# by256/icsg3d

Hardware: AMD Instinct MI355X
Metric: voxel-grids/s (fwd+bwd) for 32^3 U-Net+VAE at batch 32: value = U-Net train step (BASELINE configs[1]); DFC-VAE step (configs[2]) in secondary; both per batch in unet_plus_vae (higher is better)
Workload: dtype f32

## Files before the change

### icsg3d_amd/csrc/common.h

```cpp
#pragma once
#include <hip/hip_runtime.h>
#include <hip/hip_ext.h>
#include <atomic>
#include <cstdint>
#include <cstdio>
#include <string>
#include <vector>

#include "up8.h"
#include "up125.h"

namespace ics {

extern std::atomic<long long> g_kernel_launches;
struct LaunchTimer {
  virtual void next(hipEvent_t* start, hipEvent_t* stop) = 0;
  virtual ~LaunchTimer() = default;
};
extern thread_local LaunchTimer* tl_launch_timer;
template <typename... P, typename... A>
inline void ics_launch(void (*kernel)(P...), dim3 grid, dim3 block, size_t shmem, hipStream_t st, A&&... args) {
  static_assert(sizeof...(P) == sizeof...(A), "kernel argument count");
  if (tl_launch_timer != nullptr) {
    hipEvent_t e0 = nullptr, e1 = nullptr;
    tl_launch_timer->next(&e0, &e1);
    hipExtLaunchKernelGGL(kernel, grid, block, (std::uint32_t)shmem, st, e0, e1, 0u, static_cast<P>(args)...);
  } else {
    hipLaunchKernelGGL(kernel, grid, block, shmem, st, static_cast<P>(args)...);
  }
}
#define ICS_LAUNCH(...)                                      \
  do {                                                       \
    ::ics::g_kernel_launches.fetch_add(1, std::memory_order_relaxed); \
    ::ics::ics_launch(__VA_ARGS__);                          \
  } while (0)

void set_error(const std::string& msg);
#define ICS_HIP(expr)                                                                     \
  do {                                                                                    \
    hipError_t _e = (expr);                                                               \
    if (_e != hipSuccess) {                                                               \
      ::ics::set_error(std::string(#expr) + " -> " + hipGetErrorString(_e) + " @" +       \
                       __FILE__ + ":" + std::to_string(__LINE__));                        \
      return -1;                                                                          \
    }                                                                                     \
  } while (0)
#define ICS_CHECK(cond, msg)                                                              \
  do {                                                                                    \
    if (!(cond)) {                                                                        \
      ::ics::set_error(std::string(msg) + " (" #cond ") @" + __FILE__ + ":" +             \
                       std::to_string(__LINE__));                                         \
      return -1;                                                                          \
    }                                                                                     \
  } while (0)
#define ICS_TRY(expr)                                                                     \
  do {                                                                                    \
    if ((expr) != 0) return -1;                                                           \
  } while (0)

enum Act : int { ACT_NONE = 0, ACT_RELU = 1, ACT_LRELU = 2 };
constexpr float kLeaky = 0.3f;
constexpr float kBnEps = 1e-3f;
constexpr float kKEps = 1e-7f;
constexpr float kPoolTieTol = 1e-5f;

__device__ __forceinline__ float act_fwd(float v, int act) {
  if (act == ACT_RELU) return fmaxf(v, 0.f);
  if (act == ACT_LRELU) return v > 0.f ? v : kLeaky * v;
  return v;
}
__device__ __forceinline__ float act_grad(float v, int act) {
  if (act == ACT_RELU) return v > 0.f ? 1.f : 0.f;
  if (act == ACT_LRELU) return v > 0.f ? 1.f : kLeaky;
  return 1.f;
}

struct ConvSrc {
  const float* p;
  const float* scale;
  const float* shift;
  int C;
  int up;
  int act;
  int bcast;
};

enum ConvFlags : int {
  CF_NO_REUSE = 1,
  CF_NO_WGRAD3 = 2,
  CF_NO_WGRAD3S = 4,
  CF_NO_FWD_SPLITK = 8,
  CF_NO_THIN_N = 16,
  CF_NO_UPSPLIT = 32,
  CF_NO_THIN_C = 64,
  CF_NO_COND_FOLD = 128,
  CF_NO_WINO = 256,
  CF_NO_WINO_WGRAD = 512,
  CF_NO_WINO64 = 1024,
  CF_NO_UP3 = 2048,
  CF_NO_THIN1_2STAGE = 4096,
  CF_NO_FAST_BNBWD = 8192,
  CF_NO_FUSED_HEAD = 16384,
  CF_NO_BWD_FOLD = 32768,
  CF_UP3_BIG_ALWAYS = 65536,
  CF_NO_WINOG = 262144,
  CF_NO_HEAD_BNFUSE = 524288,
  CF_NO_UP3N = 1 << 21,
  CF_NO_DGRAD_BNFUSE = 1 << 22,
  CF_NO_POOL_PRESUM = 1 << 23,
  CF_NO_HEAD_LABELS = 1 << 24,
  CF_NO_UP8 = 1 << 25,
  CF_UP8 = 1 << 26,
  CF_NO_UP125 = 1 << 27,
  CF_FORCE_UP125 = 1 << 28,
  CF_POOL125_V1 = 1 << 29,
  CF_ZBATCH = 1 << 20,
};
int conv_flags_from_env();

struct ConvGeom {
  int B, S, lgS;
  int Cin, Cout;
  int taps;
  int Kpad, Npad;
  int flags = 0;
};

struct BwdStat {
  const float* s = nullptr;
  const float* mean = nullptr;
  const float* rstd = nullptr;
  const float* scale = nullptr;
  const float* shift = nullptr;
  float* partial = nullptr;
  int post_act = ACT_NONE;
  int ld = 0;
  const float* abc = nullptr;
  float* db_partial = nullptr;
  const float* pool_d = nullptr;
  int pool_ld = 0;
  const unsigned char* pool_mask = nullptr;
};

int launch_conv_fwd(hipStream_t st, const ConvGeom& g, const ConvSrc* src, int nsrc,
                    const float* wpacked, const float* bias, float* out, int ldo, int pre_act,
                    float* stat_partial, int* stat_rows_per_block, int accumulate = 0,
                    float* splitk_ws = nullptr, size_t splitk_ws_floats = 0, const BwdStat* bwd = nullptr,
                    int* bwd_blocks = nullptr);
size_t conv_fwd_workspace_floats(const ConvGeom& g, const ConvSrc* src, int nsrc);
bool conv_fwd_up8_tile_ok(const ConvGeom& g);
bool conv_thin_c_ok(const ConvGeom& g, const ConvSrc& s0, int nsrc, int cin_log);
size_t conv_thin_c_wgrad_workspace_floats(const ConvGeom& g);
int launch_conv_wgrad_thin_c(hipStream_t st, const ConvGeom& g, const ConvSrc& s0, const float* dy, int ldy, float* dw,
                             int ldw, int row_pitch, float* ws, size_t ws_floats, int phase);
int launch_conv_fwd_thin_c(hipStream_t st, const ConvGeom& g, const ConvSrc& s0, int cin_log, int wstride,
                           const float* wp, const float* bias, float* out, int ldo, int pre_act, float* stat_partial,
                           int* rows_per_block, const float* pos_bias = nullptr);
int launch_conv_fwd_par(hipStream_t st, const ConvGeom& g_lowres, const ConvSrc& src, const float* wpar, float* out,
                        int ldo, const float* bias = nullptr, int pre_act = ACT_NONE, float* stat_partial = nullptr,
                        int* stat_blocks = nullptr);
int launch_pack_par(hipStream_t st, const float* w, int Cin_total, int Cout, int c_off, int Cu, float* dst, int Kpad,
                    int Npad);
int launch_pack_fwd_sub(hipStream_t st, const float* w, int taps, int Cin_total, int Cout, int c_off, int Csub,
                        float* dst, int Kpad, int Npad);
int launch_conv_wgrad(hipStream_t st, const ConvGeom& g, const ConvSrc* src, int nsrc,
                      const float* dy, int ldy, float* dw, int ldw, float* workspace,
                      size_t workspace_floats, int sub_rows = 0, int row_pitch = 0, int row_off = 0,
                      int phase = 0);
const char* conv_last_kernel_id();
void conv_set_last_kernel_id(const char* id);
int launch_pack_sub(hipStream_t st, const float* w, int taps, int Cin_total, int Cout, int c_off, int Csub,
                    int flip, float* dst, int Kpad, int Npad);
size_t conv_wgrad_workspace_floats(const ConvGeom& g, const ConvSrc* src, int nsrc);
int conv_fwd_rows_per_block(const ConvGeom& g);
int launch_conv_wgrad_ablate(hipStream_t st, const ConvGeom& g, const ConvSrc* src, const float* dy, int ldy,
                             float* workspace, int ablate);
int launch_conv_fwd_ablate(hipStream_t st, const ConvGeom& g, const ConvSrc* src, int nsrc, const float* wp,
                           float* out, int ldo, int ablate);
int launch_pack_fwd(hipStream_t st, const float* w, int K, int N, float* dst, int Kpad, int Npad,
                    int k_off, int n_off, int zero_first, int cin_log = 0, int cin_phys = 0);
void* pack_table_record_begin();
int pack_table_record_end(void* handle, std::vector<unsigned char>* bytes, int* njobs, unsigned* nblocks);
int launch_pack_table(hipStream_t st, const void* d_jobs, int njobs, unsigned nblocks);
int launch_materialize_input(hipStream_t st, const ConvSrc* src, int nsrc, int Cin, int CinG, int B, int S,
                             float* out);
int launch_pack_bwd(hipStream_t st, const float* w, int taps, int Cin, int Cout, float* dst,
                    int Kpad, int Npad, int cout_total, int co_off, int zero_first);

bool conv_wino_ok(const ConvGeom& g, const ConvSrc* src, int nsrc);
size_t conv_wino_weight_floats(int Cin, int Cout);
int launch_conv_fwd_wino(hipStream_t st, const ConvGeom& g, const ConvSrc& s0, const float* wt, const float* bias,
                         float* out, int ldo, int pre_act, float* stat_partial, int* rows_per_block, int accumulate,
                         int layout, const BwdStat* bwd = nullptr, int* bwd_blocks = nullptr);
int launch_pack_wino(hipStream_t st, const float* w, int Cin_total, int Cout, int c_off, int Csub, int bwd, float* dst,
                     int layout = 0);
int conv_wino_layout(const ConvGeom& g);
bool conv_wino64_ok(const ConvGeom& g, const ConvSrc* src, int nsrc);
int launch_conv_fwd_wino64(hipStream_t st, const ConvGeom& g, const ConvSrc& s0, const float* wt, const float* bias,
                           float* out, int ldo, int pre_act, float* stat_partial, int* rows_per_block, int accumulate,
                           const BwdStat* bwd = nullptr, int* bwd_blocks = nullptr);
bool conv_wino_wgrad_ok(const ConvGeom& g, const ConvSrc* src, int nsrc);
size_t conv_wino_wgrad_workspace_floats(const ConvGeom& g);
int launch_conv_wgrad_wino(hipStream_t st, const ConvGeom& g, const ConvSrc& s0, const float* dy, int ldy, float* dw,
                           int ldw, float* ws, size_t ws_floats, int sub_rows, int row_pitch, int row_off, int phase);
bool conv_up3_ok(const ConvGeom& g, const ConvSrc& s0);
size_t conv_up3_weight_floats(int Cu, int Cout);
int launch_pack_up3(hipStream_t st, const float* w, int Cin_total, int Cout, int c_off, int Cu, float* dst);
int launch_conv_fwd_up3(hipStream_t st, const ConvGeom& g, const ConvSrc& s0, const float* wt, const float* bias,
                        float* out, int ldo, int pre_act, float* stat_partial, int* stat_blocks, int accumulate);
bool conv_winog_ok(const ConvGeom& g, const ConvSrc* src, int nsrc);
bool conv_winog_wgrad_ok(const ConvGeom& g, const ConvSrc* src, int nsrc);
size_t conv_winog_weight_floats(int Cin, int Cout);
void conv_winog_scratch_floats(const ConvGeom& g, size_t* v, size_t* m, size_t* z);
int launch_conv_fwd_winog(hipStream_t st, const ConvGeom& g, const ConvSrc& s0, const float* wg, const float* bias, float* out,
                          int ldo, int pre_act, float* stat_partial, int* rows_per_block, float* v_scratch, float* m_scratch,
                          float* vt_keep);
int launch_conv_wgrad_winog(hipStream_t st, const ConvGeom& g, const float* vt, const float* dy, int ldy, float* dw, int ldw,
                            int row_pitch, int row_off, float* z_scratch, float* m_scratch);
int launch_gemm_zbatch(hipStream_t st, int nz, int M, int K, int N, const float* A, const float* Wp, float* out, int flags);
int wgrad_zbatch_splits(int nz, int M, int K, int N);
int launch_wgrad_zbatch(hipStream_t st, int nz, int M, int K, int N, const float* x, const float* dy, float* ws, int ksplit);
int launch_pack_up125(hipStream_t st, const float* w, int Cin_total, int N, int c_off, int Cu, float* dst);
int launch_pack_up125_pieces(hipStream_t st, const float* w, int Cin_total, int N, int c_off, int Cu, float* dst);
bool conv_up3n_ok(const ConvGeom& g, const ConvSrc& s0);
size_t conv_up3n_weight_floats(int Cu, int Cout);
int launch_pack_up3n(hipStream_t st, const float* w, int Cin_total, int Cout, int c_off, int Cu, float* dst);
int launch_conv_fwd_up3n(hipStream_t st, const ConvGeom& g, const ConvSrc& s0, const float* wt, const float* bias, float* out,
                         int ldo, int pre_act, float* stat_partial, int* stat_blocks);
int launch_wgrad_reduce_splits(hipStream_t st, const float* ws, int nsplit, size_t n_elems, int N, float* dw, int ldw,
                               int sub_rows, int row_pitch, int row_off);

}
```

### icsg3d_amd/csrc/conv_igemm.hip

```cpp
#include "common.h"

#ifndef ICS_GEMM_DEEP_FWD_MIN
#define ICS_GEMM_DEEP_FWD_MIN 1
#endif
#ifndef ICS_GEMM_DEEP_MIN
#define ICS_GEMM_DEEP_MIN 3
#endif
#ifndef ICS_GEMM_DEEP
#define ICS_GEMM_DEEP 1
#endif

#include <algorithm>
#include <type_traits>
#include <cstdlib>
#include <cstring>
#include <vector>

namespace ics {

typedef float f32x16 __attribute__((ext_vector_type(16)));
typedef float v4f __attribute__((ext_vector_type(4)));

#ifndef ICS_KLDA
#define ICS_KLDA 36
#endif
constexpr int kLDA = ICS_KLDA;

__device__ __forceinline__ int xcd_swizzle(int bid, int nblk) {
  const int xcd = bid & 7, q = nblk >> 3, r = nblk & 7;
  return (xcd < r ? xcd * (q + 1) : r * (q + 1) + (xcd - r) * q) + (bid >> 3);
}

static thread_local const char* g_last_kernel_id = "";
const char* conv_last_kernel_id() { return g_last_kernel_id; }
void conv_set_last_kernel_id(const char* id) { g_last_kernel_id = id; }
static const char* tf(bool b) { return b ? "true" : "false"; }

int conv_flags_from_env() {
  int f = 0;
  if (getenv("ICSG3D_NO_REUSE")) f |= CF_NO_REUSE;
  if (getenv("ICSG3D_NO_WGRAD3")) f |= CF_NO_WGRAD3;
  if (getenv("ICSG3D_NO_WGRAD3S")) f |= CF_NO_WGRAD3S;
  if (getenv("ICSG3D_NO_FWD_SPLITK")) f |= CF_NO_FWD_SPLITK;
  if (getenv("ICSG3D_NO_THIN_N")) f |= CF_NO_THIN_N;
  if (getenv("ICSG3D_NO_UPSPLIT")) f |= CF_NO_UPSPLIT;
  if (getenv("ICSG3D_NO_THIN_C")) f |= CF_NO_THIN_C;
  if (getenv("ICSG3D_NO_COND_FOLD")) f |= CF_NO_COND_FOLD;
  if (getenv("ICSG3D_NO_WINO")) f |= CF_NO_WINO;
  if (getenv("ICSG3D_NO_WINO_WGRAD")) f |= CF_NO_WINO_WGRAD;
  if (getenv("ICSG3D_NO_WINO64")) f |= CF_NO_WINO64;
  if (getenv("ICSG3D_NO_UP3")) f |= CF_NO_UP3;
  if (getenv("ICSG3D_NO_THIN1_2STAGE")) f |= CF_NO_THIN1_2STAGE;
  if (getenv("ICSG3D_NO_FAST_BNBWD")) f |= CF_NO_FAST_BNBWD;
  if (getenv("ICSG3D_NO_FUSED_HEAD")) f |= CF_NO_FUSED_HEAD;
  if (getenv("ICSG3D_NO_BWD_FOLD")) f |= CF_NO_BWD_FOLD;
  if (getenv("ICSG3D_NO_WINOG")) f |= CF_NO_WINOG;
  if (getenv("ICSG3D_NO_HEAD_BNFUSE")) f |= CF_NO_HEAD_BNFUSE;
  if (getenv("ICSG3D_NO_UP3N")) f |= CF_NO_UP3N;
  if (getenv("ICSG3D_NO_DGRAD_BNFUSE")) f |= CF_NO_DGRAD_BNFUSE;
  if (getenv("ICSG3D_NO_POOL_PRESUM")) f |= CF_NO_POOL_PRESUM;
  if (getenv("ICSG3D_NO_HEAD_LABELS")) f |= CF_NO_HEAD_LABELS;
  if (getenv("ICSG3D_NO_UP8")) f |= CF_NO_UP8;
  if (getenv("ICSG3D_NO_UP125")) f |= CF_NO_UP125;
  if (getenv("ICSG3D_FORCE_UP125")) f |= CF_FORCE_UP125;
  if (getenv("ICSG3D_POOL125_V1")) f |= CF_POOL125_V1;
  { const char* e = getenv("ICSG3D_UP3_BIG_MIN_WG"); if (e && *e && strtoul(e, nullptr, 10) <= 1) f |= CF_UP3_BIG_ALWAYS; }
  return f;
}
struct DevOnce {
  bool done[64] = {false};
  bool need(int* dev) {
    int d = 0;
    if (hipGetDevice(&d) != hipSuccess || d < 0 || d >= 64) { *dev = -1; return true; }
    *dev = d;
    return !done[d];
  }
  void mark(int dev) { if (dev >= 0) done[dev] = true; }
};

static int identity_affine(const float** ones, const float** zeros) {
  constexpr int kN = 16384;
  static float* buf[64] = {nullptr};
  int dev = 0;
  ICS_HIP(hipGetDevice(&dev));
  ICS_CHECK(dev >= 0 && dev < 64, "device index out of range");
  if (!buf[dev]) {
    float* p = nullptr;
    ICS_HIP(hipMalloc(&p, 2 * kN * sizeof(float)));
    std::vector<float> h(2 * kN, 0.f);
    for (int i = 0; i < kN; ++i) h[i] = 1.f;
    ICS_HIP(hipMemcpy(p, h.data(), 2 * kN * sizeof(float), hipMemcpyHostToDevice));
    buf[dev] = p;
  }
  *ones = buf[dev];
  *zeros = buf[dev] + kN;
  return 0;
}
static int fix_src(ConvSrc& s) {
  if (s.scale == nullptr) {
    ICS_CHECK(s.C <= 16384, "source wider than the identity-affine buffer");
    ICS_TRY(identity_affine(&s.scale, &s.shift));
    s.act = ACT_NONE;
  }
  return 0;
}

struct RowPos {
  int b, z, y, x;
};
__device__ __forceinline__ RowPos decode_row(int m, int S, int lg) {
  RowPos r;
  r.x = m & (S - 1);
  r.y = (m >> lg) & (S - 1);
  r.z = (m >> (2 * lg)) & (S - 1);
  r.b = m >> (3 * lg);
  return r;
}

__device__ __forceinline__ size_t src_voxel(const ConvSrc& s, int b, int z, int y, int x, int S) {
  if (s.up) {
    const int Sh = S >> 1;
    return ((((size_t)b * Sh + (z >> 1)) * Sh + (y >> 1)) * Sh + (x >> 1)) * (size_t)s.C;
  }
  return ((((size_t)b * S + z) * S + y) * S + x) * (size_t)s.C;
}

__host__ __device__ __forceinline__ float act_slope_of(int act) {
  return act == ACT_RELU ? 0.f : (act == ACT_LRELU ? kLeaky : 1.f);
}
__device__ __forceinline__ float act_apply(float v, float slope) {
  return fmaxf(v, v * slope);
}
template <bool NOACT>
__device__ __forceinline__ v4f affine_only_or_act4(v4f v, v4f sc, v4f sh, float slope);
__device__ __forceinline__ v4f affine_act4(v4f v, v4f sc, v4f sh, float slope) {
  v4f r;
  r.x = act_apply(fmaf(v.x, sc.x, sh.x), slope); r.y = act_apply(fmaf(v.y, sc.y, sh.y), slope);
  r.z = act_apply(fmaf(v.z, sc.z, sh.z), slope); r.w = act_apply(fmaf(v.w, sc.w, sh.w), slope);
  return r;
}
template <bool NOACT>
__device__ __forceinline__ v4f affine_only_or_act4(v4f v, v4f sc, v4f sh, float slope) {
  if (!NOACT) return affine_act4(v, sc, sh, slope);
  v4f r;
  r.x = fmaf(v.x, sc.x, sh.x); r.y = fmaf(v.y, sc.y, sh.y); r.z = fmaf(v.z, sc.z, sh.z); r.w = fmaf(v.w, sc.w, sh.w);
  return r;
}
__device__ __forceinline__ unsigned voxel_off(int b, int z, int y, int x, int S, int u, int C) {
  const int Ss = S >> u;
  return ((((unsigned)b * Ss + (z >> u)) * Ss + (y >> u)) * Ss + (x >> u)) * (unsigned)C;
}
__device__ __forceinline__ int clampi(int v, int hi) { return min(max(v, 0), hi); }

__device__ __forceinline__ ConvSrc pick_src(const ConvSrc& s0, const ConvSrc& s1, bool first) {
  ConvSrc s;
  s.p = first ? s0.p : s1.p;
  s.scale = first ? s0.scale : s1.scale;
  s.shift = first ? s0.shift : s1.shift;
  s.C = first ? s0.C : s1.C;
  s.up = first ? s0.up : s1.up;
  s.act = first ? s0.act : s1.act;
  s.bcast = first ? s0.bcast : s1.bcast;
  return s;
}

__device__ __forceinline__ float gather_scalar(const ConvSrc& s0, const ConvSrc& s1, int ci, int b,
                                               int z, int y, int x, int S) {
  const bool first = ci < s0.C;
  const ConvSrc s = pick_src(s0, s1, first);
  const int cl = first ? ci : ci - s0.C;
  float v;
  if (s.bcast > 0) {
    v = s.p[(size_t)b * s.bcast + (cl % s.bcast)];
  } else {
    v = s.p[src_voxel(s, b, z, y, x, S) + cl];
  }
  if (s.scale) v = act_fwd(fmaf(v, s.scale[cl], s.shift[cl]), s.act);
  return v;
}

template <int WM, int WN, int TM, int TN, bool VEC, int ABL = 0, bool AFF = true, bool UP = true, bool THIN = false,
          bool REUSE = false, bool PAR = false, bool NOACT = false, bool FOLD = false, bool UP8 = false>
__global__ __launch_bounds__(256, FOLD ? 2 : ((REUSE && PAR) ? 3 : 1)) void conv_fwd_kernel(ConvGeom g, ConvSrc s0, ConvSrc s1,
                                                        const float* __restrict__ wp,
                                                        const float* __restrict__ bias,
                                                        float* __restrict__ out, int ldo, int pre_act,
                                                        float* __restrict__ stat_partial, int gridM,
                                                        int gridN, int accumulate, BwdStat bs, Up8Geom u8) {
  constexpr int BM = WM * TM * 32, BN = WN * TN * 32;
  constexpr int B_FLOATS = 32 * BN;
  constexpr int RA = BM / 32;
  constexpr int RS = BM / 8;
  constexpr int NB = BN / 32;
  extern __shared__ __attribute__((aligned(16))) float smem[];
  const int A_FLOATS = (REUSE ? BM + (BM >> g.lgS) + 1 : BM) * kLDA;
  float* As = smem;
  constexpr int NABUF = 1;
  float* Bs = smem + NABUF * A_FLOATS;

  const int t = threadIdx.x, lane = t & 63, wave = t >> 6;
  const int wm = wave / WN, wn = wave % WN;
  const int li = lane & 31, lh = lane >> 5;
  const int sw = xcd_swizzle(blockIdx.x, gridM * gridN);
  const int mb = sw / gridN, nb = sw % gridN;
  const int S = g.S, lg = g.lgS;
  const int M = g.B << (3 * lg);
  const int n0 = nb * BN;
  const int nchunks = g.Kpad >> 5;
  const int cpt = (VEC && !THIN) ? (g.Cin >> 5) : 1;
  const int cls = PAR ? (int)blockIdx.y : 0;
  const int pz = cls >> 2, py = (cls >> 1) & 1, px = cls & 1;
  if (PAR) wp += (size_t)cls * g.Kpad * g.Npad;
  const bool zbatch = (g.flags & CF_ZBATCH) != 0;
  if (zbatch) {
    s0.p += (size_t)blockIdx.z * (size_t)M * (size_t)s0.C;
    wp += (size_t)blockIdx.z * (size_t)g.Kpad * (size_t)g.Npad;
    out += (size_t)blockIdx.z * (size_t)M * (size_t)ldo;
  }
// ... 1524 lines not shown
      return launch_fwd_cfg<WM, WN, TM, TN, true, 0, true, true, false, true>(ICS_FWD_ARGS);    \
    }                                                                                           \
    if (variant == 0 && fold)                                                                   \
      return launch_fwd_cfg<WM, WN, TM, TN, true, 0, false, false, false, false, false, false, true>(ICS_FWD_ARGS); \
    if (variant == 0) return launch_fwd_cfg<WM, WN, TM, TN, true, 0, false, false>(ICS_FWD_ARGS); \
    if (variant == 1) return launch_fwd_cfg<WM, WN, TM, TN, true, 0, true, false>(ICS_FWD_ARGS);  \
    return launch_fwd_cfg<WM, WN, TM, TN, true, 0, true, true>(ICS_FWD_ARGS);                   \
  } while (0)
  if (bm == 64) { ICS_FWD(2, 2, 1, 1); }
  if (bn == 128) { ICS_FWD(2, 2, 2, 2); }
  if (bn == 96) { ICS_FWD(4, 1, 1, 3); }
  if (bn == 64) { ICS_FWD(2, 2, 2, 1); }
  ICS_FWD(4, 1, 1, 1);
#undef ICS_FWD_ARGS
#undef ICS_FWD
}

static void pick_par_tile(const ConvGeom& g, int* bm, int* bn) {
  pick_fwd_tile(g, bm, bn);
  if (*bm == 64 && g.Npad % 128 == 0 && (long)(((g.B << (3 * g.lgS)) + 127) / 128) * (g.Npad / 128) * 8 >= 384) {
    *bm = 128; *bn = 128;
  }
}
int launch_conv_fwd_par(hipStream_t st, const ConvGeom& g, const ConvSrc& src, const float* wp, float* out,
                        int ldo, const float* bias, int pre_act, float* stat_partial, int* stat_blocks) {
  ConvSrc s0 = src, s1 = src;
  s1.C = 0;
  ICS_CHECK(g.taps == 8 && g.Cin % 32 == 0 && s0.C == g.Cin && !s0.up && !s0.bcast && g.Kpad == 8 * g.Cin,
            "parity-class conv needs a direct 32k-channel source");
  ICS_TRY(fix_src(s0));
  ICS_TRY(fix_src(s1));
  int bm, bn;
  pick_par_tile(g, &bm, &bn);
  int rpb = 0;
#define ICS_PAR_ARGS st, g, s0, s1, wp, bias, out, ldo, pre_act, stat_partial, &rpb
  int rc;
  const bool no_reuse = (g.flags & CF_NO_REUSE) != 0;
  const bool reuse = !no_reuse && g.S >= 4 && g.S <= bm;
  const bool noact = src.scale != nullptr && src.act == ACT_NONE;
#define ICS_PAR(WM, WN, TM, TN)                                                                              \
  (reuse ? (noact ? launch_fwd_cfg<WM, WN, TM, TN, true, 0, true, false, false, true, true, true>(ICS_PAR_ARGS) \
                  : launch_fwd_cfg<WM, WN, TM, TN, true, 0, true, false, false, true, true>(ICS_PAR_ARGS))   \
         : launch_fwd_cfg<WM, WN, TM, TN, true, 0, true, false, false, false, true>(ICS_PAR_ARGS))
  if (bm == 64) rc = ICS_PAR(2, 2, 1, 1);
  else if (bn == 128) rc = ICS_PAR(2, 2, 2, 2);
  else if (bn == 96) rc = ICS_PAR(4, 1, 1, 3);
  else if (bn == 64) rc = ICS_PAR(2, 2, 2, 1);
  else rc = ICS_PAR(4, 1, 1, 1);
#undef ICS_PAR
#undef ICS_PAR_ARGS
  if (stat_blocks) *stat_blocks = 8 * (((g.B << (3 * g.lgS)) + rpb - 1) / rpb);
  return rc;
}

struct PackJob {
  int kind;
  const float* w;
  float* dst;
  int a[9];
  unsigned long long total;
  unsigned blk0;
};
static thread_local std::vector<PackJob>* g_pack_rec = nullptr;

__device__ __forceinline__ float pack_par_value(size_t i, const float* __restrict__ w, int Cin_total, int Cout, int c_off,
                                                int Cu, int Kpad, int Npad) {
  const size_t per = (size_t)Kpad * Npad;
  const int cls = (int)(i / per);
  const size_t j = i - (size_t)cls * per;
  const int tq = j & 3;
  const size_t rest = j >> 2;
  const int n = rest % Npad;
  const int k = (int)(rest / Npad) * 4 + tq;
  const int e = k / Cu, c = k - e * Cu;
  float v = 0.f;
  if (e < 8 && n < Cout) {
    const int p3[3] = {cls >> 2, (cls >> 1) & 1, cls & 1};
    const int e3[3] = {e >> 2, (e >> 1) & 1, e & 1};
    int lo[3], hi[3];
#pragma unroll
    for (int a = 0; a < 3; ++a) {
      if (p3[a] == 0) { lo[a] = e3[a] ? 1 : 0; hi[a] = e3[a] ? 2 : 0; }
      else { lo[a] = e3[a] ? 2 : 0; hi[a] = e3[a] ? 2 : 1; }
    }
    for (int dz = lo[0]; dz <= hi[0]; ++dz)
      for (int dy = lo[1]; dy <= hi[1]; ++dy)
        for (int dx = lo[2]; dx <= hi[2]; ++dx)
          v += w[((size_t)((dz * 3 + dy) * 3 + dx) * Cin_total + c_off + c) * Cout + n];
  }
  return v;
}
__global__ void pack_par_kernel(const float* __restrict__ w, int Cin_total, int Cout, int c_off, int Cu,
                                float* __restrict__ dst, int Kpad, int Npad) {
  const size_t i = (size_t)blockIdx.x * blockDim.x + threadIdx.x;
  if (i >= 8 * (size_t)Kpad * Npad) return;
  dst[i] = pack_par_value(i, w, Cin_total, Cout, c_off, Cu, Kpad, Npad);
}
int launch_pack_par(hipStream_t st, const float* w, int Cin_total, int Cout, int c_off, int Cu, float* dst,
                    int Kpad, int Npad) {
  if (g_pack_rec) { g_pack_rec->push_back(PackJob{4, w, dst, {Cin_total, Cout, c_off, Cu, Kpad, Npad, 0, 0, 0}, 8ull * Kpad * Npad, 0}); return 0; }
  const size_t total = (size_t)8 * Kpad * Npad;
  ICS_LAUNCH(pack_par_kernel, dim3((unsigned)((total + 255) / 256)), dim3(256), 0, st, w, Cin_total, Cout,
                     c_off, Cu, dst, Kpad, Npad);
  ICS_HIP(hipGetLastError());
  return 0;
}
__device__ __forceinline__ float pack_fwd_sub_value(size_t i, const float* __restrict__ w, int taps, int Cin_total,
                                                    int Cout, int c_off, int Csub, int Npad) {
  const int tq = i & 3;
  const size_t rest = i >> 2;
  const int n = rest % Npad;
  const int k = (int)(rest / Npad) * 4 + tq;
  const int tap = k / Csub, c = k - tap * Csub;
  return (tap < taps && n < Cout) ? w[((size_t)tap * Cin_total + c_off + c) * Cout + n] : 0.f;
}
__global__ void pack_fwd_sub_kernel(const float* __restrict__ w, int taps, int Cin_total, int Cout, int c_off,
                                    int Csub, float* __restrict__ dst, int Kpad, int Npad) {
  const size_t i = (size_t)blockIdx.x * blockDim.x + threadIdx.x;
  if (i >= (size_t)Kpad * Npad) return;
  dst[i] = pack_fwd_sub_value(i, w, taps, Cin_total, Cout, c_off, Csub, Npad);
}
int launch_pack_fwd_sub(hipStream_t st, const float* w, int taps, int Cin_total, int Cout, int c_off, int Csub,
                        float* dst, int Kpad, int Npad) {
  if (g_pack_rec) { g_pack_rec->push_back(PackJob{3, w, dst, {taps, Cin_total, Cout, c_off, Csub, Npad, 0, 0, 0}, (unsigned long long)Kpad * Npad, 0}); return 0; }
  const size_t total = (size_t)Kpad * Npad;
  ICS_LAUNCH(pack_fwd_sub_kernel, dim3((unsigned)((total + 255) / 256)), dim3(256), 0, st, w, taps,
                     Cin_total, Cout, c_off, Csub, dst, Kpad, Npad);
  ICS_HIP(hipGetLastError());
  return 0;
}

int launch_conv_fwd_ablate(hipStream_t st, const ConvGeom& g, const ConvSrc* src, int nsrc, const float* wp,
                           float* out, int ldo, int ablate) {
  ConvSrc s0 = src[0], s1 = src[nsrc > 1 ? 1 : 0];
  if (nsrc == 1) s1.C = 0;
  ICS_TRY(fix_src(s0));
  ICS_TRY(fix_src(s1));
  ICS_CHECK(fwd_is_vec(g, s0, s1) && g.Npad % 128 == 0, "ablation bench needs the vector 128x128 configuration");
#define ICS_ABL_ARGS st, g, s0, s1, wp, nullptr, out, ldo, 0, nullptr, nullptr
  if (ablate == 1) return launch_fwd_cfg<2, 2, 2, 2, true, 1, true, false>(ICS_ABL_ARGS);
  if (ablate == 2) return launch_fwd_cfg<2, 2, 2, 2, true, 2, true, false>(ICS_ABL_ARGS);
  if (ablate == 3) return launch_fwd_cfg<2, 2, 2, 2, true, 3, true, false>(ICS_ABL_ARGS);
  if (ablate == 4) return launch_fwd_cfg<2, 2, 2, 2, true, 4, true, false>(ICS_ABL_ARGS);
  if (ablate == 8) return launch_fwd_cfg<2, 2, 2, 2, true, 8, false, false>(ICS_ABL_ARGS);
  if (ablate == 9) return launch_fwd_cfg<2, 2, 2, 2, true, 9, false, false>(ICS_ABL_ARGS);
  if (ablate == 5) return launch_fwd_cfg<2, 2, 2, 2, true, 0, true, false>(ICS_ABL_ARGS);
  if (ablate == 6) return launch_fwd_cfg<2, 2, 2, 2, true, 0, true, true>(ICS_ABL_ARGS);
  return launch_fwd_cfg<2, 2, 2, 2, true, 0, false, false>(ICS_ABL_ARGS);
#undef ICS_ABL_ARGS
}


template <int WM, int WN, int TM, int TN, bool VEC, bool DYVEC, bool AFF = true, bool UP = true, bool THIN = false,
          int ABL = 0, bool UP8 = false, bool ZB = false>
__global__ __launch_bounds__(256) void conv_wgrad_kernel(ConvGeom g, ConvSrc s0, ConvSrc s1,
                                                          const float* __restrict__ dy, int ldy,
                                                          int n_load,
                                                          float* __restrict__ ws, int ktiles,
                                                          int ntiles, int rows_per_split, Up8Geom u8) {
  constexpr int KT = WM * TM * 32, NT = WN * TN * 32;
  constexpr int A_FLOATS = 32 * KT, D_FLOATS = 32 * NT;
  constexpr int AF4 = KT / 4, ATOT = 32 * AF4, APASS = ATOT / 256;
  constexpr int DF4 = NT / 4, DTOT = 32 * DF4, DPASS = DTOT / 256;
  static_assert(ATOT % 256 == 0 && DTOT % 256 == 0, "tile loads must divide evenly over 256 threads");
  extern __shared__ __attribute__((aligned(16))) float smem[];
  float* As = smem;
  float* Ds = smem + 2 * A_FLOATS;

  const int t = threadIdx.x, lane = t & 63, wave = t >> 6;
  const int wm = wave / WN, wn = wave % WN;
  const int li = lane & 31, lh = lane >> 5;
  const int S = g.S, lg = g.lgS;
  const int M = g.B << (3 * lg);
  const int K = g.taps * g.Cin;
  if (ZB) {
    s0.p += (size_t)blockIdx.y * (size_t)M * (size_t)s0.C;
    dy += (size_t)blockIdx.y * (size_t)M * (size_t)ldy;
    ws += (size_t)blockIdx.y * (size_t)(gridDim.x / (unsigned)(ktiles * ntiles)) * (size_t)K * (size_t)g.Cout;
  }

  int bid = blockIdx.x;
  const int nt_i = bid % ntiles; bid /= ntiles;
  const int kt_i = bid % ktiles; bid /= ktiles;
  const int split = bid;
  const int n0 = nt_i * NT;
  const int m_begin = split * rows_per_split;
  const int m_end = min(M, m_begin + rows_per_split);
  const int nchunks = (m_end - m_begin + 31) >> 5;

  const int k0 = kt_i * KT;
  int tdz = 0, tdy = 0, tdx = 0, sdelta = 0, xbad = -1, ybad = -1, zbad = -1;
  bool kvalid = false;
  const float* sp = s0.p;
  int sC = s0.C, su = 0, cl0 = 0;
  float slope = 1.f;
  v4f sc = v4f{1.f, 1.f, 1.f, 1.f}, sh = v4f{0.f, 0.f, 0.f, 0.f};
  if (VEC) {
    const int kf = k0 + (t % AF4) * 4;
    const int tap = kf / g.Cin, ci = kf - tap * g.Cin;
    kvalid = kf < K;
    if (g.taps == 27 && kvalid) { tdz = tap / 9 - 1; tdy = (tap / 3) % 3 - 1; tdx = tap % 3 - 1; }
    sdelta = (tdz * S + tdy) * S + tdx;
    xbad = tdx < 0 ? 0 : (tdx > 0 ? S - 1 : -1);
    ybad = tdy < 0 ? 0 : (tdy > 0 ? S - 1 : -1);
    zbad = tdz < 0 ? 0 : (tdz > 0 ? S - 1 : -1);
    const bool first = ci < s0.C;
    const ConvSrc sv = pick_src(s0, s1, first);
    sp = sv.p; sC = sv.C; su = sv.up;
    cl0 = kvalid ? (first ? ci : ci - s0.C) : 0;
    slope = act_slope_of(sv.act);
    if (AFF) {
      sc = *reinterpret_cast<const v4f*>(sv.scale + cl0);
      sh = *reinterpret_cast<const v4f*>(sv.shift + cl0);
    }
  }
  int s_tap = 0, s_ci = 0; bool s_kvalid = false; int sdz = 0, sdy = 0, sdx = 0;
  if (!VEC) {
    const int kf = k0 + (t & 31);
    s_tap = kf / g.Cin; s_ci = kf - s_tap * g.Cin; s_kvalid = kf < K;
    if (g.taps == 27) { sdz = s_tap / 9 - 1; sdy = (s_tap / 3) % 3 - 1; sdx = s_tap % 3 - 1; }
  }

  v4f ra[VEC ? APASS : 1];
  float ras[4];
  v4f rd[DPASS];

  auto load_chunk = [&](int c) {
    const int mbase = m_begin + (c << 5);
    if (VEC) {
      const int Sh = S >> 1;
#pragma unroll
      for (int p = 0; p < APASS; ++p) {
        const int m = mbase + (t + 256 * p) / AF4;
        const int x = m & (S - 1), y = (m >> lg) & (S - 1), z = (m >> (2 * lg)) & (S - 1);
        const bool inb = kvalid && m < m_end && x != xbad && y != ybad && z != zbad;
        int idx = m + sdelta;
        if (UP) {
          const int b = m >> (3 * lg);
          const int idx_up = ((b * Sh + ((z + tdz) >> 1)) * Sh + ((y + tdy) >> 1)) * Sh + ((x + tdx) >> 1);
          idx = su ? idx_up : idx;
        }
        const unsigned off = inb ? (unsigned)idx * (unsigned)sC + cl0 : (unsigned)cl0;
        v4f v = *reinterpret_cast<const v4f*>(sp + off);
        if (AFF) v = affine_act4(v, sc, sh, slope);
        ra[p] = inb ? v : v4f{0.f, 0.f, 0.f, 0.f};
      }
    } else {
#pragma unroll
      for (int p = 0; p < 4; ++p) {
        const int m = mbase + (t >> 5) + 8 * p;
        float v = 0.f;
        if (s_kvalid && m < m_end) {
          const RowPos r = decode_row(m, S, lg);
          const int zz = r.z + sdz, yy = r.y + sdy, xx = r.x + sdx;
          if ((unsigned)zz < (unsigned)S && (unsigned)yy < (unsigned)S && (unsigned)xx < (unsigned)S)
            v = gather_scalar(s0, s1, s_ci, r.b, zz, yy, xx, S);
        }
        ras[p] = v;
      }
    }
#pragma unroll
    for (int p = 0; p < DPASS; ++p) {
      const int idx = t + 256 * p;
      const int m = mbase + idx / DF4;
      const int n = n0 + (idx % DF4) * 4;
      const float* q = dy + (size_t)min(m, M - 1) * ldy;
      v4f v;
      if (DYVEC) {
        v = *reinterpret_cast<const v4f*>(q + min(n, n_load - 4));
        if (!(m < m_end && n < n_load)) v = v4f{0.f, 0.f, 0.f, 0.f};
      } else {
        v.x = q[min(n + 0, n_load - 1)]; v.y = q[min(n + 1, n_load - 1)];
        v.z = q[min(n + 2, n_load - 1)]; v.w = q[min(n + 3, n_load - 1)];
        const bool rowok = m < m_end;
        v.x = (rowok && n + 0 < n_load) ? v.x : 0.f; v.y = (rowok && n + 1 < n_load) ? v.y : 0.f;
        v.z = (rowok && n + 2 < n_load) ? v.z : 0.f; v.w = (rowok && n + 3 < n_load) ? v.w : 0.f;
      }
      rd[p] = v;
    }
  };
  const bool gemm = VEC && DYVEC && !UP && !THIN && ABL == 0 && g.taps == 1 && (M & 31) == 0 &&
                    (rows_per_split & 31) == 0 && (UP8 || n0 + NT <= n_load);
  const bool noact_g = slope == 1.f;
  unsigned aoffg[VEC ? APASS : 1], doffg[DPASS];
  if (VEC) {
#pragma unroll
    for (int p = 0; p < APASS; ++p) aoffg[p] = (unsigned)(((t + 256 * p) / AF4) * sC + cl0) * 4u;
  }
#pragma unroll
  for (int p = 0; p < DPASS; ++p) {
    const int idx = t + 256 * p;
    doffg[p] = UP8 ? (up8_prow((unsigned)(idx / DF4), u8.lgSh, u8.P) * (unsigned)u8.N +
                      up8_col_floats(min(n0 + (idx % DF4) * 4, n_load - 4), u8)) * 4u
                   : (unsigned)((idx / DF4) * ldy + n0 + (idx % DF4) * 4) * 4u;
  }
  auto load_chunk_gemm = [&](int c, auto noact_tag) {
    constexpr bool NA = decltype(noact_tag)::value;
    const int mbase = m_begin + (c << 5);
    const char* abase = reinterpret_cast<const char*>(sp) + (size_t)mbase * (size_t)sC * 4;
    const char* dbase = reinterpret_cast<const char*>(dy) +
                        (UP8 ? up8_chunk_base_floats((unsigned)mbase, u8) : (size_t)mbase * (size_t)ldy) * 4;
    if (VEC) {
#pragma unroll
      for (int p = 0; p < APASS; ++p) {
        v4f v = *reinterpret_cast<const v4f*>(abase + aoffg[p]);
        if (AFF) v = affine_only_or_act4<NA>(v, sc, sh, slope);
        ra[p] = v;
      }
    }
#pragma unroll
    for (int p = 0; p < DPASS; ++p) rd[p] = *reinterpret_cast<const v4f*>(dbase + doffg[p]);
  };
  auto store_chunk = [&](int buf) {
    float* A = As + buf * A_FLOATS;
    float* D = Ds + buf * D_FLOATS;
    if (VEC) {
#pragma unroll
      for (int p = 0; p < APASS; ++p) {
        const int idx = t + 256 * p;
        *reinterpret_cast<v4f*>(A + (idx / AF4) * KT + (idx % AF4) * 4) = ra[p];
      }
    } else {
#pragma unroll
      for (int p = 0; p < 4; ++p) A[((t >> 5) + 8 * p) * KT + (t & 31)] = ras[p];
    }
#pragma unroll
    for (int p = 0; p < DPASS; ++p) {
      const int idx = t + 256 * p;
      *reinterpret_cast<v4f*>(D + (idx / DF4) * NT + (idx % DF4) * 4) = rd[p];
    }
  };

  f32x16 acc[TM][TN];
#pragma unroll
  for (int i = 0; i < TM; ++i)
#pragma unroll
    for (int j = 0; j < TN; ++j)
// ... 458 lines not shown
  const bool first = c0 < s0.C;
  const char* sp = reinterpret_cast<const char*>(first ? s0.p : s1.p);
  const int sC = first ? s0.C : s1.C;
  const float slope = act_slope_of(first ? s0.act : s1.act);
  const int ac4 = t & 15;
  const int cl = (first ? c0 : c0 - s0.C) + ac4 * 4;
  if (AFF && t < 32) {
    const float* src = (t < 16) ? (first ? s0.scale : s1.scale) : (first ? s0.shift : s1.shift);
    *reinterpret_cast<v4f*>(Aff + t * 4) = *reinterpret_cast<const v4f*>(src + (first ? c0 : c0 - s0.C) + (t & 15) * 4);
  }
  const unsigned aoff = (unsigned)((t >> 4) * sC + cl) * 4u;
  const unsigned hoff = (unsigned)cl * 4u;
  unsigned doff[4];
#pragma unroll
  for (int p = 0; p < 4; ++p) doff[p] = (unsigned)(((t >> 5) + 8 * p) * ldy + n0 + (t & 31) * 4) * 4u;
  const int hside = (t >> 4) & 1;

  v4f ra[2], rd[4], rah = v4f{0.f, 0.f, 0.f, 0.f};
  auto load_chunk = [&](int c) {
    const int mbase = m_begin + (c << 5);
    v4f sc = v4f{1.f, 1.f, 1.f, 1.f}, sh = v4f{0.f, 0.f, 0.f, 0.f};
    if (AFF) { sc = *reinterpret_cast<const v4f*>(Aff + ac4 * 4); sh = *reinterpret_cast<const v4f*>(Aff + 64 + ac4 * 4); }
#pragma unroll
    for (int p = 0; p < 2; ++p) {
      const int row0 = mbase + 16 * p;
      const int y = (row0 >> lg) & (S - 1), z = (row0 >> (2 * lg)) & (S - 1);
      const bool inb = (y != ybad) & (z != zbad);
      const float msk = inb ? 1.f : 0.f;
      const char* base = sp + (inb ? (long)(row0 + sdelta) * sC * 4 : 0L);
      v4f v = *reinterpret_cast<const v4f*>(base + aoff);
      if (AFF) v = affine_only_or_act4<NOACT>(v, sc, sh, slope);
      ra[p] = v4f{v.x * msk, v.y * msk, v.z * msk, v.w * msk};
    }
    if (halo) {
      const int x0 = mbase & (S - 1);
      const int y = (mbase >> lg) & (S - 1), z = (mbase >> (2 * lg)) & (S - 1);
      const bool lineok = (y != ybad) & (z != zbad);
      const bool inl = lineok & (x0 != 0), inr = lineok & (x0 == 0);
      const char* bl = sp + (inl ? (long)(mbase - 1 + sdelta) * sC * 4 : 0L);
      const char* br = sp + (inr ? (long)(mbase + 32 + sdelta) * sC * 4 : 0L);
      const float msk = (hside ? inr : inl) ? 1.f : 0.f;
      v4f v = *reinterpret_cast<const v4f*>((hside ? br : bl) + hoff);
      if (AFF) v = affine_only_or_act4<NOACT>(v, sc, sh, slope);
      rah = v4f{v.x * msk, v.y * msk, v.z * msk, v.w * msk};
    }
    const char* dbase = reinterpret_cast<const char*>(dy) + (size_t)mbase * (size_t)ldy * 4;
#pragma unroll
    for (int p = 0; p < 4; ++p) rd[p] = *reinterpret_cast<const v4f*>(dbase + doff[p]);
  };
  float* a_st[2];
#pragma unroll
  for (int p = 0; p < 2; ++p) {
    const int r = (t >> 4) + 16 * p;
    a_st[p] = As + (r + (halo ? 0 : (r >> lg)) + 1) * CK + ac4 * 4;
  }
  auto store_chunk = [&](int buf) {
#pragma unroll
    for (int p = 0; p < 2; ++p) *reinterpret_cast<v4f*>(a_st[p] + buf * A_FLOATS) = ra[p];
    if (halo && t < 32) *reinterpret_cast<v4f*>(As + buf * A_FLOATS + (hside ? 33 : 0) * CK + ac4 * 4) = rah;
    float* D = Ds + buf * D_FLOATS;
#pragma unroll
    for (int p = 0; p < 4; ++p) *reinterpret_cast<v4f*>(D + ((t >> 5) + 8 * p) * NT + (t & 31) * 4) = rd[p];
  };

  f32x16 acc[3][2];
#pragma unroll
  for (int i = 0; i < 3; ++i)
#pragma unroll
    for (int j = 0; j < 2; ++j)
#pragma unroll
      for (int r = 0; r < 16; ++r) acc[i][j][r] = 0.f;

  if (!halo) {
    for (int i = t; i < 2 * (lines + 1) * CK; i += 256) {
      const int b = i / ((lines + 1) * CK), rem = i - b * (lines + 1) * CK;
      As[b * A_FLOATS + (rem / CK) * (S + 1) * CK + rem % CK] = 0.f;
    }
  }
  __syncthreads();
  if (nchunks > 0) {
    load_chunk(0);
    store_chunk(0);
  }
  __syncthreads();
  auto compute = [&](int buf) {
    const float* A = As + buf * A_FLOATS + 2 * li + lh * CK;
    const float* D = Ds + buf * D_FLOATS + 32 * wave + li + lh * NT;
#pragma unroll
    for (int s = 0; s < 16; ++s) {
      constexpr int dummy = 0; (void)dummy;
      const int prow = 2 * s + (halo ? 0 : ((2 * s) >> lg)) + 1;
      const float b = D[(2 * s) * NT];
      float2 a[3];
#pragma unroll
      for (int dxi = 0; dxi < 3; ++dxi) a[dxi] = *reinterpret_cast<const float2*>(A + (prow + dxi - 1) * CK);
#pragma unroll
      for (int dxi = 0; dxi < 3; ++dxi) {
        acc[dxi][0] = __builtin_amdgcn_mfma_f32_32x32x2f32(a[dxi].x, b, acc[dxi][0], 0, 0, 0);
        acc[dxi][1] = __builtin_amdgcn_mfma_f32_32x32x2f32(a[dxi].y, b, acc[dxi][1], 0, 0, 0);
      }
    }
  };
  for (int c = 0; c + 1 < nchunks; ++c) {
    load_chunk(c + 1);
    compute(c & 1);
    store_chunk((c + 1) & 1);
    __syncthreads();
  }
  if (nchunks > 0) compute((nchunks - 1) & 1);

  float* wsp = ws + (size_t)split * K * g.Cout;
  const int n = n0 + 32 * wave + li;
#pragma unroll
  for (int dxi = 0; dxi < 3; ++dxi)
#pragma unroll
    for (int j = 0; j < 2; ++j)
#pragma unroll
      for (int r = 0; r < 16; ++r) {
        const int row = (r & 3) + 8 * (r >> 2) + 4 * lh;
        const int k = (gzy * 3 + dxi) * g.Cin + c0 + 2 * row + j;
        wsp[(size_t)k * g.Cout + n] = acc[dxi][j][r];
      }
}

static bool wgrad3_ok(const ConvGeom& g, const ConvSrc& s0, int nsrc, const ConvSrc& s1) {
  if ((g.flags & CF_NO_WGRAD3) || g.taps != 27 || g.S > 64 || g.S < 2 || g.Cin % 64 != 0 || g.Cout % 128 != 0) return false;
  if (s0.bcast || (nsrc > 1 && s1.bcast)) return false;
  if (nsrc > 1 && (s0.C % 64 != 0)) return false;
  return true;
}
struct Wgrad3Plan { int cgroups, ntiles, ksplit, rows_per_split; };
static Wgrad3Plan plan_wgrad3(const ConvGeom& g) {
  Wgrad3Plan p;
  const long M = (long)g.B << (3 * g.lgS);
  p.cgroups = g.Cin / 64;
  p.ntiles = g.Cout / 128;
  const int want = pick_ksplit(9L * p.cgroups * p.ntiles, M, g.lgS > 5 ? 512 : 768, 2);
  p.rows_per_split = (int)(((M + want - 1) / want + 31) / 32 * 32);
  p.ksplit = (int)((M + p.rows_per_split - 1) / p.rows_per_split);
  return p;
}


size_t conv_wgrad_workspace_floats(const ConvGeom& g, const ConvSrc* src, int nsrc) {
  if (thin_n_ok(g, src[0], nsrc)) return (size_t)thin_n_wgrad_splits(g) * g.taps * g.Cin * g.Cout;
  ConvSrc s0 = src[0], s1 = src[nsrc > 1 ? 1 : 0];
  WgradPlan p = plan_wgrad(g, s0, nsrc, s1);
  int ks = p.ksplit;
  if (wgrad3_ok(g, s0, nsrc, s1)) ks = std::max(ks, plan_wgrad3(g).ksplit);
  return (size_t)ks * g.taps * g.Cin * g.Cout;
}

template <int WM, int WN, int TM, int TN, bool VEC, bool DYVEC, bool AFF = true, bool UP = true, bool THIN = false,
          int ABL = 0, bool UP8 = false, bool ZB = false>
static int launch_wgrad_cfg(hipStream_t st, const ConvGeom& g, const ConvSrc& s0, const ConvSrc& s1,
                            const float* dy, int ldy, int n_load, float* ws, const WgradPlan& p, int nz = 1) {
  constexpr int KT = WM * TM * 32, NT = WN * TN * 32;
  const size_t lds = (size_t)2 * 32 * (KT + NT) * sizeof(float);
  auto kern = conv_wgrad_kernel<WM, WN, TM, TN, VEC, DYVEC, AFF, UP, THIN, ABL, UP8, ZB>;
  static DevOnce attr;
  int dev;
  if (attr.need(&dev)) {
    ICS_HIP(hipFuncSetAttribute(reinterpret_cast<const void*>(kern),
                                hipFuncAttributeMaxDynamicSharedMemorySize, (int)lds));
    attr.mark(dev);
  }
  static const std::string id = std::string("conv_wgrad_kernel<") + std::to_string(WM) + ", " + std::to_string(WN) +
                                ", " + std::to_string(TM) + ", " + std::to_string(TN) + ", " + tf(VEC) + ", " +
                                tf(DYVEC) + ", " + tf(AFF) + ", " + tf(UP) + ", " + tf(THIN) + ", " +
                                std::to_string(ABL) + (UP8 ? ", UP8>" : (ZB ? ", ZB>" : ">"));
  g_last_kernel_id = id.c_str();
  Up8Geom u8;
  if (UP8) u8 = up8_geom(g.B, g.S, g.lgS, g.Cout / 27);
  ICS_LAUNCH(kern, dim3(p.ktiles * p.ntiles * p.ksplit, ZB ? nz : 1), dim3(256), lds, st, g, s0, s1, dy,
                     ldy, n_load, ws, p.ktiles, p.ntiles, p.rows_per_split, u8);
  ICS_HIP(hipGetLastError());
  return 0;
}

int launch_conv_wgrad_ablate(hipStream_t st, const ConvGeom& g, const ConvSrc* src, const float* dy, int ldy,
                             float* workspace, int ablate) {
  ConvSrc s0 = src[0], s1 = src[0];
  s1.C = 0;
  ICS_TRY(fix_src(s0));
  ICS_TRY(fix_src(s1));
  WgradPlan p = plan_wgrad(g, s0, 1, s1);
  ICS_CHECK(p.vec && p.kt == 128 && p.nt == 128, "ablation bench needs the vector 128x128 configuration");
  if (ablate == 1) return launch_wgrad_cfg<2, 2, 2, 2, true, true, false, false, false, 1>(st, g, s0, s1, dy, ldy, g.Cout, workspace, p);
  return launch_wgrad_cfg<2, 2, 2, 2, true, true, false, false, false, 2>(st, g, s0, s1, dy, ldy, g.Cout, workspace, p);
}

int launch_conv_wgrad(hipStream_t st, const ConvGeom& g, const ConvSrc* src, int nsrc,
                      const float* dy, int ldy, float* dw, int ldw, float* workspace,
                      size_t workspace_floats, int sub_rows, int row_pitch, int row_off, int phase) {
  if (thin_n_ok(g, src[0], nsrc)) {
    const int ns = thin_n_wgrad_splits(g);
    const size_t n_el = (size_t)g.taps * g.Cin * g.Cout;
    ICS_CHECK((size_t)ns * n_el <= workspace_floats, "wgrad workspace too small");
    const int M = g.B << (3 * g.lgS);
    const int rows = (M + ns - 1) / ns;
    const int K = 27 * g.Cin;
    const bool aff = src[0].scale != nullptr;
    if (thin1_wgrad_ok(g, src[0])) {
      const int nb = thin1_wgrad_blocks(g);
      if (phase != 2) {
#define ICS_T1W(CKV)                                                                                                 \
  do {                                                                                                               \
    if (aff) ICS_LAUNCH((thin1_wgrad_kernel<CKV, true>), dim3(nb), dim3(256), 0, st, g, src[0], dy, ldy, workspace); \
    else ICS_LAUNCH((thin1_wgrad_kernel<CKV, false>), dim3(nb), dim3(256), 0, st, g, src[0], dy, ldy, workspace);    \
  } while (0)
        switch (g.Cin / 16) { case 1: ICS_T1W(1); break; case 2: ICS_T1W(2); break; case 3: ICS_T1W(3); break; default: ICS_T1W(4); break; }
#undef ICS_T1W
        ICS_HIP(hipGetLastError());
        g_last_kernel_id = "thin1_wgrad_kernel";
      }
      if (phase != 1) ICS_TRY(launch_reduce_splits(st, workspace, 4 * nb, n_el, g.Cout, dw, ldw, sub_rows, row_pitch, row_off));
      return 0;
    }
    if (phase != 2) {
#define ICS_TNW(NOUT, AFFV, KPT, NAME)                                                                         \
  do {                                                                                                         \
    g_last_kernel_id = NAME;                                                                                   \
    ICS_LAUNCH((conv_thin_n_wgrad_kernel<NOUT, AFFV, KPT>), dim3((M + rows - 1) / rows), dim3(256), 0,  \
                       st, g, src[0], dy, ldy, workspace, rows);                                               \
  } while (0)
#define ICS_TNW_K(NOUT, AFFV, TAG)                                                                  \
  do {                                                                                              \
    if (K <= 512) ICS_TNW(NOUT, AFFV, 2, "conv_thin_n_wgrad_kernel<" TAG ", 2>");                   \
    else if (K <= 1024) ICS_TNW(NOUT, AFFV, 4, "conv_thin_n_wgrad_kernel<" TAG ", 4>");             \
    else ICS_TNW(NOUT, AFFV, 7, "conv_thin_n_wgrad_kernel<" TAG ", 7>");                            \
  } while (0)
      if (g.Cout == 1) { if (aff) ICS_TNW_K(1, true, "1, true"); else ICS_TNW_K(1, false, "1, false"); }
      else { if (aff) ICS_TNW_K(4, true, "4, true"); else ICS_TNW_K(4, false, "4, false"); }
#undef ICS_TNW_K
#undef ICS_TNW
      ICS_HIP(hipGetLastError());
    }
    if (phase != 1)
      ICS_TRY(launch_reduce_splits(st, workspace, (M + rows - 1) / rows, n_el, g.Cout, dw, ldw, sub_rows, row_pitch,
                                   row_off));
    return 0;
  }
  ConvSrc s0 = src[0], s1 = src[nsrc > 1 ? 1 : 0];
  if (nsrc == 1) s1.C = 0;
  ICS_TRY(fix_src(s0));
  ICS_TRY(fix_src(s1));
  WgradPlan p = plan_wgrad(g, s0, nsrc, s1);
  const size_t n_elems = (size_t)g.taps * g.Cin * g.Cout;
  const int n_load4 = (g.Cout + 3) / 4 * 4;
  const bool dy_vec = (ldy % 4 == 0) && ((reinterpret_cast<uintptr_t>(dy) & 15) == 0) && (n_load4 <= ldy);
  const int n_load = dy_vec ? n_load4 : g.Cout;
  if (!dy_vec) {
    p.nt = (p.kt == 128) ? 32 : (p.kt == 64) ? 64 : 128;
    p.ntiles = (g.Npad + p.nt - 1) / p.nt;
  }
  const bool aff = src[0].scale != nullptr || (nsrc > 1 && src[1].scale != nullptr);
  const bool up = src[0].up || (nsrc > 1 && src[1].up);
  if (dy_vec && wgrad3_ok(g, s0, nsrc, s1)) {
    const Wgrad3Plan q = plan_wgrad3(g);
    ICS_CHECK((size_t)q.ksplit * n_elems <= workspace_floats, "wgrad workspace too small");
    const int arows = 32 + std::max(32 >> g.lgS, 1) + 1;
    const size_t lds = (size_t)(2 * (arows * 64 + 32 * 128) + 128) * sizeof(float);
    const dim3 grid(9 * q.cgroups * q.ntiles * q.ksplit);
    const int M3 = g.B << (3 * g.lgS);
    const bool fast = !up && g.lgS >= 4 && g.lgS <= 6 && M3 % 32 == 0 && n_load == g.Cout &&
                      !(g.flags & CF_NO_WGRAD3S);
    if (phase != 2 && fast) {
      const bool noact = aff && (src[0].scale == nullptr || src[0].act == ACT_NONE) &&
                         (nsrc < 2 || src[1].scale == nullptr || src[1].act == ACT_NONE);
      const int ar = 32 + (g.lgS == 6 ? 1 : (32 >> g.lgS)) + 1;
      const size_t lds3 = (size_t)(2 * (ar * 64 + 32 * 128) + 128) * sizeof(float);
#define ICS_W3S(AFFV, NOACTV, LGV)                                                                              \
  do {                                                                                                          \
    g_last_kernel_id = "conv_wgrad3s_kernel<" #AFFV ", " #NOACTV ", " #LGV ">";                                 \
    ICS_LAUNCH((conv_wgrad3s_kernel<AFFV, NOACTV, LGV>), grid, dim3(256), lds3, st, g, s0, s1, dy, ldy,  \
                       workspace, q.cgroups, q.ntiles, q.rows_per_split);                                       \
  } while (0)
#define ICS_W3S_L(AFFV, NOACTV)                                                       \
  do {                                                                                \
    if (g.lgS == 4) ICS_W3S(AFFV, NOACTV, 4);                                         \
    else if (g.lgS == 5) ICS_W3S(AFFV, NOACTV, 5);                                    \
    else ICS_W3S(AFFV, NOACTV, 6);                                                    \
  } while (0)
      if (!aff) ICS_W3S_L(false, false);
      else if (noact) ICS_W3S_L(true, true);
      else ICS_W3S_L(true, false);
#undef ICS_W3S_L
#undef ICS_W3S
      ICS_HIP(hipGetLastError());
    } else if (phase != 2) {
#define ICS_W3(AFFV, UPV, HALOV)                                                                                 \
  do {                                                                                                           \
    g_last_kernel_id = "conv_wgrad3_kernel<" #AFFV ", " #UPV ", " #HALOV ">";                                    \
    ICS_LAUNCH((conv_wgrad3_kernel<AFFV, UPV, HALOV>), grid, dim3(256), lds, st, g, s0, s1, dy, ldy,      \
                       n_load, workspace, q.cgroups, q.ntiles, q.rows_per_split);                                \
  } while (0)
      if (g.lgS > 5) {
        if (up) ICS_W3(true, true, true); else if (aff) ICS_W3(true, false, true); else ICS_W3(false, false, true);
      } else {
        if (up) ICS_W3(true, true, false); else if (aff) ICS_W3(true, false, false); else ICS_W3(false, false, false);
      }
#undef ICS_W3
      ICS_HIP(hipGetLastError());
    }
    if (phase != 1) {
      ICS_TRY(launch_reduce_splits(st, workspace, q.ksplit, n_elems, g.Cout, dw, ldw, sub_rows, row_pitch, row_off));
    }
    return 0;
  }
  ICS_CHECK((size_t)p.ksplit * n_elems <= workspace_floats, "wgrad workspace too small");
  if (phase != 2) {
#define ICS_WG_ARGS st, g, s0, s1, dy, ldy, n_load, workspace, p
#define ICS_WG(WM, WN, TM, TN, DV)                                                                 \
  do {                                                                                             \
    if (p.thin) ICS_TRY((launch_wgrad_cfg<WM, WN, TM, TN, true, DV, true, true, true>(ICS_WG_ARGS)));  \
    else if (!p.vec) ICS_TRY((launch_wgrad_cfg<WM, WN, TM, TN, false, DV, true, true>(ICS_WG_ARGS)));   \
    else if (up) ICS_TRY((launch_wgrad_cfg<WM, WN, TM, TN, true, DV, true, true>(ICS_WG_ARGS)));   \
    else if (aff) ICS_TRY((launch_wgrad_cfg<WM, WN, TM, TN, true, DV, true, false>(ICS_WG_ARGS))); \
    else ICS_TRY((launch_wgrad_cfg<WM, WN, TM, TN, true, DV, false, false>(ICS_WG_ARGS)));         \
  } while (0)
  if (g.flags & CF_UP8) {
    const int M8 = g.B << (3 * g.lgS);
    ICS_CHECK(dy_vec && p.vec && !p.thin && !up && g.taps == 1 && g.Cout % 27 == 0 && n_load == g.Cout && M8 % 32 == 0 &&
                  p.rows_per_split % 32 == 0 && up8_shape_ok(2 * g.S, g.Cout / 27, (size_t)M8, g.B),
              "up8 backward-weight: shape outside the 8-volume layout");
#define ICS_WG8(WM, WN, TM, TN)                                                                                  \
  do {                                                                                                           \
    if (aff) ICS_TRY((launch_wgrad_cfg<WM, WN, TM, TN, true, true, true, false, false, 0, true>(ICS_WG_ARGS)));  \
    else ICS_TRY((launch_wgrad_cfg<WM, WN, TM, TN, true, true, false, false, false, 0, true>(ICS_WG_ARGS)));     \
  } while (0)
    ICS_CHECK(p.nt == 128 && p.kt >= 64, "up8 backward-weight: no UP8 instantiation of this tile");
    if (p.kt == 128) ICS_WG8(2, 2, 2, 2);
    else ICS_WG8(2, 2, 1, 2);
#undef ICS_WG8
  } else if (!dy_vec) {
    if (p.kt == 128) ICS_WG(4, 1, 1, 1, false);
    else if (p.kt == 64) ICS_WG(2, 2, 1, 1, false);
    else ICS_WG(1, 4, 1, 1, false);
  } else if (p.kt == 128) {
    if (p.nt == 128) ICS_WG(2, 2, 2, 2, true);
    else if (p.nt == 96) ICS_WG(4, 1, 1, 3, true);
    else if (p.nt == 64) ICS_WG(4, 1, 1, 2, true);
    else ICS_WG(4, 1, 1, 1, true);
  } else if (p.kt == 64) {
    if (p.nt == 128) ICS_WG(2, 2, 1, 2, true);
    else ICS_WG(2, 2, 1, 1, true);
  } else {
    ICS_WG(1, 4, 1, 1, true);
  }
#undef ICS_WG_ARGS
#undef ICS_WG
  }
  if (phase != 1) {
    ICS_TRY(launch_reduce_splits(st, workspace, p.ksplit, n_elems, g.Cout, dw, ldw, sub_rows, row_pitch, row_off));
  }
  return 0;
}

int wgrad_zbatch_splits(int nz, int M, int K, int N) {
  const long base = (long)((K + 127) / 128) * ((N + 127) / 128) * nz;
  const long ks_max = std::max<long>(1, M / 256);
  return (int)std::max<long>(1, std::min<long>(std::min<long>(512 / base, ks_max), 512));
}
int launch_wgrad_zbatch(hipStream_t st, int nz, int M, int K, int N, const float* x, const float* dy, float* ws, int ksplit) {
  ICS_CHECK(nz >= 1 && nz <= 65535 && M >= 1 && K % 32 == 0 && N % 4 == 0 && ksplit >= 1, "z-batched wgrad: K % 32, N % 4 required");
  ICS_CHECK((size_t)M * (size_t)std::max(K, N) < ((size_t)1 << 30), "z-batched wgrad: matrix too large for 32-bit offsets");
  const ConvGeom g{M, 1, 0, K, N, 1, K, (N + 31) / 32 * 32, 0};
  const ConvSrc s0{x, nullptr, nullptr, K, 0, ACT_NONE, 0};
  ConvSrc s1 = s0;
  s1.C = 0;
  WgradPlan p;
  p.vec = true; p.thin = false;
  p.kt = 128; p.nt = 128;
  p.ktiles = (K + 127) / 128; p.ntiles = (N + 127) / 128;
  p.rows_per_split = ((M + ksplit - 1) / ksplit + 31) / 32 * 32;
  p.ksplit = (M + p.rows_per_split - 1) / p.rows_per_split;
  ICS_CHECK(p.ksplit <= ksplit, "z-batched wgrad: split plan");
  p.ksplit = ksplit;
  return launch_wgrad_cfg<2, 2, 2, 2, true, true, false, false, false, 0, false, true>(st, g, s0, s1, dy, N, N, ws, p, nz);
}

__device__ __forceinline__ bool pack_fwd_value(size_t i, const float* __restrict__ w, int K, int N, int Npad, int k_off,
                                               int n_off, int cin_log, int cin_phys, float* v) {
  const int tq = i & 3;
  const size_t rest = i >> 2;
  const int n = rest % Npad;
  const int k = (int)(rest / Npad) * 4 + tq;
  int ks = k - k_off;
  const int ns = n - n_off;
  bool ok = ks >= 0 && ks < K && ns >= 0 && ns < N;
  if (ok && cin_phys > 0) {
    const int tap = ks / cin_phys, ci = ks - tap * cin_phys;
    ok = ci < cin_log;
    ks = tap * cin_log + ci;
  }
  *v = ok ? w[(size_t)ks * N + ns] : 0.f;
  return ok;
}
__global__ void pack_fwd_kernel(const float* __restrict__ w, int K, int N, float* __restrict__ dst,
                                int Kpad, int Npad, int k_off, int n_off, int zero_first, int cin_log,
                                int cin_phys) {
  const size_t i = (size_t)blockIdx.x * blockDim.x + threadIdx.x;
  const size_t total = (size_t)Kpad * Npad;
  if (i >= total) return;
  float v;
  if (pack_fwd_value(i, w, K, N, Npad, k_off, n_off, cin_log, cin_phys, &v) || zero_first) dst[i] = v;
}

__global__ void materialize_input_kernel(ConvSrc s0, ConvSrc s1, int Cin, int CinG, int S, int lg, size_t total,
                                         float* __restrict__ out) {
  const size_t i = (size_t)blockIdx.x * blockDim.x + threadIdx.x;
  if (i >= total) return;
  const int c = (int)(i % CinG);
  const RowPos r = decode_row((int)(i / CinG), S, lg);
  out[i] = c < Cin ? gather_scalar(s0, s1, c, r.b, r.z, r.y, r.x, S) : 0.f;
}
int launch_materialize_input(hipStream_t st, const ConvSrc* src, int nsrc, int Cin, int CinG, int B, int S,
                             float* out) {
  ConvSrc s0 = src[0], s1 = src[nsrc > 1 ? 1 : 0];
  if (nsrc == 1) s1.C = 0;
  int lg = 0;
  while ((1 << lg) < S) ++lg;
  const size_t total = (size_t)B * S * S * S * CinG;
  ICS_LAUNCH(materialize_input_kernel, dim3((unsigned)((total + 255) / 256)), dim3(256), 0, st, s0, s1, Cin,
                     CinG, S, lg, total, out);
  ICS_HIP(hipGetLastError());
  return 0;
}

__device__ __forceinline__ bool pack_bwd_value(size_t i, const float* __restrict__ w, int taps, int Cin, int Cout,
                                               int Npad, int cout_total, int co_off, float* v) {
  const int tq = i & 3;
  const size_t rest = i >> 2;
  const int n = rest % Npad;
  const int k = (int)(rest / Npad) * 4 + tq;
  const int tp = k / cout_total, co = k - tp * cout_total - co_off;
  const bool ok = tp < taps && co >= 0 && co < Cout && n < Cin;
  *v = ok ? w[((size_t)(taps - 1 - tp) * Cin + n) * Cout + co] : 0.f;
  return ok;
}
__global__ void pack_bwd_kernel(const float* __restrict__ w, int taps, int Cin, int Cout,
                                float* __restrict__ dst, int Kpad, int Npad, int cout_total,
                                int co_off, int zero_first) {
  const size_t i = (size_t)blockIdx.x * blockDim.x + threadIdx.x;
  const size_t total = (size_t)Kpad * Npad;
  if (i >= total) return;
  float v;
  if (pack_bwd_value(i, w, taps, Cin, Cout, Npad, cout_total, co_off, &v) || zero_first) dst[i] = v;
}

__device__ __forceinline__ float pack_sub_value(size_t i, const float* __restrict__ w, int taps, int Cin_total, int Cout,
                                                int c_off, int Csub, int flip, int Npad) {
  const int tq = i & 3;
  const size_t rest = i >> 2;
  const int n = rest % Npad;
  const int k = (int)(rest / Npad) * 4 + tq;
  const int tp = k / Cout, co = k - tp * Cout;
  float v = 0.f;
  if (tp < taps && n < Csub) v = w[((size_t)(flip ? taps - 1 - tp : tp) * Cin_total + c_off + n) * Cout + co];
  return v;
}
__global__ void pack_sub_kernel(const float* __restrict__ w, int taps, int Cin_total, int Cout, int c_off,
                                int Csub, int flip, float* __restrict__ dst, int Kpad, int Npad) {
  const size_t i = (size_t)blockIdx.x * blockDim.x + threadIdx.x;
  const size_t total = (size_t)Kpad * Npad;
  if (i >= total) return;
  dst[i] = pack_sub_value(i, w, taps, Cin_total, Cout, c_off, Csub, flip, Npad);
}
int launch_pack_sub(hipStream_t st, const float* w, int taps, int Cin_total, int Cout, int c_off, int Csub,
                    int flip, float* dst, int Kpad, int Npad) {
  if (g_pack_rec) { g_pack_rec->push_back(PackJob{2, w, dst, {taps, Cin_total, Cout, c_off, Csub, flip, Npad, 0, 0}, (unsigned long long)Kpad * Npad, 0}); return 0; }
  const size_t total = (size_t)Kpad * Npad;
  ICS_LAUNCH(pack_sub_kernel, dim3((unsigned)((total + 255) / 256)), dim3(256), 0, st, w, taps, Cin_total,
                     Cout, c_off, Csub, flip, dst, Kpad, Npad);
  ICS_HIP(hipGetLastError());
  return 0;
}

int launch_pack_fwd(hipStream_t st, const float* w, int K, int N, float* dst, int Kpad, int Npad,
                    int k_off, int n_off, int zero_first, int cin_log, int cin_phys) {
  if (g_pack_rec) { g_pack_rec->push_back(PackJob{0, w, dst, {K, N, Npad, k_off, n_off, cin_log, cin_phys, 0, 0}, (unsigned long long)Kpad * Npad, 0}); return 0; }
  const size_t total = (size_t)Kpad * Npad;
  ICS_LAUNCH(pack_fwd_kernel, dim3((unsigned)((total + 255) / 256)), dim3(256), 0, st, w, K, N,
                     dst, Kpad, Npad, k_off, n_off, zero_first, cin_log, cin_phys);
  ICS_HIP(hipGetLastError());
  return 0;
}
int launch_pack_bwd(hipStream_t st, const float* w, int taps, int Cin, int Cout, float* dst,
                    int Kpad, int Npad, int cout_total, int co_off, int zero_first) {
  if (g_pack_rec) { g_pack_rec->push_back(PackJob{1, w, dst, {taps, Cin, Cout, Npad, cout_total, co_off, 0, 0, 0}, (unsigned long long)Kpad * Npad, 0}); return 0; }
  const size_t total = (size_t)Kpad * Npad;
  ICS_LAUNCH(pack_bwd_kernel, dim3((unsigned)((total + 255) / 256)), dim3(256), 0, st, w, taps,
                     Cin, Cout, dst, Kpad, Npad, cout_total, co_off, zero_first);
  ICS_HIP(hipGetLastError());
  return 0;
}

__device__ __forceinline__ void pack_wino_pair(size_t t, const float* __restrict__ w, int Cin_total, int Cout, int c_off,
                                               int Csub, int bwd, float* __restrict__ dst, int layout) {
  const int K = bwd ? Cout : Csub;
  if (layout == 2) {
    const int Nn = bwd ? Csub : Cout;
    const int k2 = (int)(t / ((size_t)4 * Nn)) * 4 + (int)(t & 3), n2 = (int)((t >> 2) % (size_t)Nn);
    float g2[27];
#pragma unroll
    for (int tap = 0; tap < 27; ++tap)
      g2[tap] = bwd ? w[((size_t)(26 - tap) * Cin_total + c_off + n2) * Cout + k2]
                    : w[((size_t)tap * Cin_total + c_off + k2) * Cout + n2];
    const size_t fs2 = (size_t)K * Nn;
    float* d2 = dst + t;
#pragma unroll
    for (int fz = 0; fz < 4; ++fz)
#pragma unroll
      for (int fy = 0; fy < 4; ++fy)
#pragma unroll
        for (int fx = 0; fx < 4; ++fx) {
          float acc = 0.f;
#pragma unroll
          for (int a = 0; a < 3; ++a) {
            const float ga = fz == 0 ? (a == 0 ? 1.f : 0.f) : fz == 3 ? (a == 2 ? 1.f : 0.f) : (fz == 2 && a == 1 ? -0.5f : 0.5f);
            if (ga == 0.f) continue;
#pragma unroll
            for (int b = 0; b < 3; ++b) {
              const float gb = fy == 0 ? (b == 0 ? 1.f : 0.f) : fy == 3 ? (b == 2 ? 1.f : 0.f) : (fy == 2 && b == 1 ? -0.5f : 0.5f);
              if (gb == 0.f) continue;
#pragma unroll
              for (int c = 0; c < 3; ++c) {
                const float gc = fx == 0 ? (c == 0 ? 1.f : 0.f) : fx == 3 ? (c == 2 ? 1.f : 0.f) : (fx == 2 && c == 1 ? -0.5f : 0.5f);
                if (gc == 0.f) continue;
                acc += (ga * gb * gc) * g2[(a * 3 + b) * 3 + c];
              }
            }
// ... 224 lines not shown
```

### icsg3d_amd/csrc/elementwise.h

```cpp
#pragma once
#include "common.h"

#include <rccl/rccl.h>

namespace ics {

struct BnParams {
  const float* gamma;
  const float* beta;
  float* moving_mean;
  float* moving_var;
  float* mean;
  float* rstd;
  float* scale;
  float* shift;
  float* xs = nullptr;
};

struct BnSyncEmu {
  int rank, nranks;
  double* fwd;
  double* bwd;
  int cmax, cap;
  int call;
};
struct BnSync {
  ncclComm_t comm;
  int nranks;
  double* local;
  double* gathered;
  BnSyncEmu* emu = nullptr;
};
int bn_sync_exchange(hipStream_t st, const BnSync* sync, bool gather, size_t count, const char* what);

enum GradSrcKind : int { GS_NONE = 0, GS_DIRECT = 1, GS_UP = 2, GS_POOL = 3 };

struct GradSrc {
  const float* p;
  int ld, off;
  int kind;
  const float* pooled;
  const unsigned char* pool_idx;
};

struct LayerBwd {
  const float* s;
  const float* scale; const float* shift; const float* mean; const float* rstd;
  const float* dtap;
  const float* tap_ref;
  float tap_coef;
  double* tap_partial;
  GradSrc g0, g1;
  int B, S, lgS, C;
  int has_bn, pre_act, post_act;
  int pool_ties_all;
  int flags;
};

int launch_bn_finalize(hipStream_t st, const float* partial, int nblk, int Npad, const BnParams& bn,
                       int C, int update_moving, int unbias, const BnSync* sync = nullptr);
int launch_bn_eval_prepare(hipStream_t st, const BnParams& bn, int C);
int launch_pool_fwd(hipStream_t st, const float* s, const float* scale, const float* shift, int act,
                    int B, int S, int C, float* out, unsigned char* idx, unsigned char* tie_mask = nullptr,
                    float* tie_ssum = nullptr, int ties_all = 1);
struct BwdPre {
  const float* partial;
  int nblk, ld;
};
int launch_layer_bwd(hipStream_t st, const LayerBwd& L, float* dy, float* ws_partial, float* c1c2,
                     float* dgamma, float* dbeta, float* dbias, const BnSync* sync = nullptr,
                     const BwdPre* pre = nullptr, float* db_partial_own = nullptr, int* db_blocks = nullptr);
__host__ __device__ inline int colsum_blocks(int C) { return C % 4 == 0 ? C / 4 : C; }
struct ColsumJobs {
  const float* partial[24];
  float* out[24];
  int nblk[24], C[24], blk0[25];
  int n;
};
int launch_colsum_batch(hipStream_t st, const ColsumJobs& J);
size_t layer_bwd_workspace_floats(const LayerBwd& L);
int bn_bwd_num_blocks(const LayerBwd& L, int* rows_per_block);
struct PmSums {
  int n[4];
  double per[4];
  float w[4];
};
bool head_fused_ok(int ncls, int cin, size_t M, int act, int flags);
bool head_dgrad_ok(int ncls, int cin, size_t M, const BwdStat* bs, int flags);
int launch_head_dgrad(hipStream_t st, const float* dz, const float* wsoft_k, const float* wsig_k, float* dx, int ldo, size_t M,
                      const BwdStat* bs, int Npad, int* blocks, const float* c1c2 = nullptr, float* db_partial = nullptr);
int launch_xhat_affine(hipStream_t st, const float* mean, const float* rstd, int C, float* xs);
int launch_head_bnfuse(hipStream_t st, const float* Q, const float* dzsum, const float* wsoft, const float* wsig,
                       const float* gamma, const float* beta, double n, int ncls, float* dwsoft, float* dwsig, float* c1c2,
                       float* dgamma, float* dbeta, const BnSync* sync = nullptr);
bool conv_bnfuse_ok(int S, int Cin, int N);
size_t conv_bnfuse_partial_floats(int B, int S, int C);
int launch_conv_bnfuse(hipStream_t st, const float* dy, int B, int S, int Cin, int CinTot, int N, const float* db_partial,
                       int db_nblk, const float* W, float* G, const float* gamma, const float* beta, const float* mean,
                       const float* rstd, const float* scale, float* abc, float* c1c2, float* dgamma, float* dbeta,
                       float* ws_partial, size_t ws_partial_floats, double* ws_R, double* sums_out = nullptr);
bool pool_presum_ok(int C, int ldg);
int pool_presum_blocks(size_t pooled_rows);
int launch_pool_presum(hipStream_t st, const float* g, int ldg, const unsigned char* mask, const float* ssum, size_t pooled_rows,
                       int C, const float* mean, const float* rstd, float* pre, size_t pre_floats, int* blocks);
size_t pool_bnfuse_partial_doubles(size_t pooled_rows, int C);
int launch_pool_bnfuse(hipStream_t st, const float* g, int ldg, const unsigned char* mask, const float* ssum, size_t pooled_rows,
                       int C, double cnt, const double* sums_conv, const float* mean, const float* rstd, const float* scale,
                       float* abc, float* c1c2, float* dgamma, float* dbeta, double* ws_partial, size_t ws_partial_doubles);
int launch_head_fused(hipStream_t st, const float* x, int ldx, const float* scale, const float* shift, const float* wsoft_k,
                      const float* wsig_k, const float* bsoft, const float* bsig, float* z, const unsigned char* labels,
                      size_t M, int mode, int want_grad, float wsoft, double* partial, int partial_blocks, float* metrics,
                      int* nblk_out = nullptr, float* dz_colsum = nullptr, double* keep = nullptr,
                      float thresh = 0.f, unsigned char* species = nullptr, unsigned char* mask = nullptr,
                      const float* cw = nullptr);
int launch_head(hipStream_t st, float* z, int ldz, int ncls, const unsigned char* labels, size_t M,
                int mode, int want_grad, float wsoft, double* partial, int partial_blocks,
                float* metrics, int* nblk_out = nullptr, float* dz_colsum = nullptr, double* keep = nullptr,
                const float* cw = nullptr);
int launch_head_metrics(hipStream_t st, const double* partial, int nblk, double M, float* metrics, double* sums,
                        int phase, double* keep = nullptr);
int launch_adam(hipStream_t st, float* p, const float* g, float* m, float* v, size_t n, float lr_t,
                float gscale);
int launch_bn_apply(hipStream_t st, const float* s, const float* scale, const float* shift, int act,
                    size_t n, int C, float* out);
int launch_sqdiff(hipStream_t st, const float* a, const float* b, int B, size_t per_sample,
                  int blocks_per_sample, double* partial, float* grad, float coef, int accumulate);
int launch_sampling(hipStream_t st, const float* mulv, int ld, int latent, const float* eps,
                    const float* cond, int ncond, int B, float* z, float* zc);
int launch_vae_loss(hipStream_t st, const float* mulv, int ld, int latent, int B, const double* mse_partial,
                    int n_mse, double n_elems, const double* pm_partial, const PmSums& pmc, float alpha, float beta,
                    float* metrics, double* sums = nullptr, int phase = 0);
int launch_vae_dz(hipStream_t st, const float* mulv, int ld, int latent, int B, const float* eps,
                  const float* dzc, int ldzc, float beta, float* dmulv);
int launch_cond_bias_table(hipStream_t st, const float* w, const float* bias, const float* cond, int C, int ncond,
                           int Cin_tot, int Cout, int B, float* T);
size_t cond_wgrad_workspace_doubles(int B, int Cout);
int launch_cond_wgrad(hipStream_t st, const float* dy, int B, int S, int Cout, const float* cond, int C0, int nfold,
                      int ncond, int Cin_tot, float* dw, double* ws, size_t ws_doubles);
int launch_relu_bwd(hipStream_t st, const float* a, float* g, size_t n);
int launch_colsum_small(hipStream_t st, const float* a, int rows, int cols, int ld, float* out);
int launch_axpy(hipStream_t st, float* y, const float* x, size_t n, float a);
int launch_pool27(hipStream_t st, const float* dy, int B, int S, int N, float* out, int ldo);
int launch_pool8(hipStream_t st, const float* dy, int B, int S, int N, float* out, const Up8Geom& u);
int launch_pool125(hipStream_t st, const float* dy, int B, int S, int N, float* out, const Up125Geom& u, bool v1);
int launch_up125_xclass(hipStream_t st, const ConvSrc& s, float* out, const Up125Geom& u);
int launch_up125_combine(hipStream_t st, const float* cls, float* dxl, const Up125Geom& u);
struct Up125Splits { unsigned long long off[4]; int ks[4]; };
int launch_up125_contract(hipStream_t st, const float* ws, const Up125Splits& p, float* dw, const Up125Geom& u);
int launch_permute_up_dw(hipStream_t st, const float* tmp, int Cu, int N, int Cin, int c_off, float* dw);

}
```

### icsg3d_amd/csrc/engine.hip

```cpp
#include "common.h"
#include "elementwise.h"
#include "segment.h"
#include "scratch.h"
#include "voxelise.h"
#include "latent.h"
#include "tsne.h"
#include "render.h"
#include "monitor.h"
#include "feed.h"
#include "confusion.h"
#include "atomscore.h"
#include "../../include/icsg3d.h"

#include <rccl/rccl.h>
#include <roctracer/roctx.h>

#include <cmath>
#include <cstring>
#include <functional>
#include <map>
#include <memory>
#include <mutex>
#include <vector>

// ... 348 lines not shown
  int add_tensor(const std::string& name, std::vector<int64_t> dims, bool trainable) {
    Tensor t;
    t.name = name; t.dims = dims; t.trainable = trainable;
    t.count = 1;
    for (auto v : dims) t.count *= (size_t)v;
    if (trainable) { t.off = nparams; nparams += t.count; }
    tensors.push_back(t);
    tindex[name] = (int)tensors.size() - 1;
    return (int)tensors.size() - 1;
  }
  float* tp(int ti) const { return P + tensors[ti].off; }
  float* tg(int ti) const { return G + tensors[ti].off; }
  size_t rows(const ConvLayer& L, int B) const { return (size_t)B * L.S * L.S * L.S; }
};

static int padded_cin(int Cin) {
  if (Cin % 32 == 0 || Cin == 4 || Cin == 8 || Cin == 16) return Cin;
  return Cin < 4 ? 4 : (Cin < 8 ? 8 : (Cin < 16 ? 16 : round_up(Cin, 32)));
}

static ConvLayer* add_conv(Net& n, const std::string& name, int Cin, int Cout, int taps, int S, int pre_act,
                           int has_bn, int post_act, bool dense, bool register_params = true, bool pad_input = false) {
  auto L = std::make_unique<ConvLayer>();
  L->name = name; L->Cin = Cin; L->Cout = Cout; L->taps = taps; L->S = S;
  L->flags = n.flags;
  L->CinG = pad_input ? padded_cin(Cin) : Cin;
  L->pre_act = pre_act; L->has_bn = has_bn; L->post_act = post_act;
  L->Kpad = round_up(taps * L->CinG, 32); L->Npad = round_up(Cout, 32);
  L->Kpad_b = round_up(taps * Cout, 32); L->Npad_b = round_up(L->CinG, 32);
  if (register_params) {
    if (dense) L->t_w = n.add_tensor(name + "/kernel", {Cin, Cout}, true);
    else L->t_w = n.add_tensor(name + "/kernel", {taps == 27 ? 3 : 1, taps == 27 ? 3 : 1, taps == 27 ? 3 : 1, Cin, Cout}, true);
    L->t_b = n.add_tensor(name + "/bias", {Cout}, true);
    if (has_bn) {
      L->t_gamma = n.add_tensor(name + "/gamma", {Cout}, true);
      L->t_beta = n.add_tensor(name + "/beta", {Cout}, true);
    }
  }
  n.layers.push_back(std::move(L));
  return n.layers.back().get();
}

static int alloc_layer(Net& n, ConvLayer& L, bool need_bwd, bool pooled) {
  const size_t M = n.rows(L, n.maxB);
  ICS_TRY(n.alloc(&L.wp, (size_t)L.Kpad * L.Npad));
  ICS_TRY(n.alloc(&L.s, M * L.Cout));
  if (need_bwd) {
    ICS_TRY(n.alloc(&L.wf, (size_t)L.Kpad_b * L.Npad_b));
    ICS_TRY(n.alloc(&L.dy, M * L.Cout));
    ICS_TRY(n.alloc(&L.dA, M * L.CinG));
    ICS_TRY(n.alloc(&L.c1c2, (size_t)2 * L.Cout));
    if ((L.Cout & (L.Cout - 1)) == 0 || L.Cout % 4 == 0) {
      size_t rows = std::max((size_t)512, M / 128 + 1);
      for (int b = 1; b <= n.maxB; ++b) {
        LayerBwd lb{};
        lb.B = b; lb.S = L.S; lb.lgS = ilog2(L.S); lb.C = L.Cout;
        int rpb;
        rows = std::max(rows, (size_t)bn_bwd_num_blocks(lb, &rpb));
      }
      L.db_rows = rows;
      ICS_TRY(n.alloc(&L.db_partial, rows * L.Cout));
    }
    if (L.has_bn) { ICS_TRY(n.alloc(&L.xs, (size_t)2 * L.Cout)); ICS_TRY(n.alloc(&L.abc, (size_t)3 * L.Cout)); }
  }
  if (L.has_bn) {
    if (!n.bn_slab) {
      size_t tot = 0;
      for (auto& q : n.layers) if (q->has_bn) tot += 2 * (size_t)q->Cout;
      ICS_TRY(n.alloc(&n.bn_slab, tot));
      n.bn_slab_n = tot;
    }
    ICS_CHECK(n.bn_slab_used + 2 * (size_t)L.Cout <= n.bn_slab_n, "BN slab overflow");
    L.mm = n.bn_slab + n.bn_slab_used; L.mv = L.mm + L.Cout;
    n.bn_slab_used += 2 * (size_t)L.Cout;
    n.sync_cmax = std::max(n.sync_cmax, L.Cout);
    ICS_TRY(n.alloc(&L.mean, (size_t)L.Cout)); ICS_TRY(n.alloc(&L.rstd, (size_t)L.Cout));
    ICS_TRY(n.alloc(&L.scale, (size_t)L.Cout)); ICS_TRY(n.alloc(&L.shift, (size_t)L.Cout));
    int ti = n.add_tensor(L.name + "/moving_mean", {L.Cout}, false);
    n.tensors[ti].ptr = L.mm;
    ti = n.add_tensor(L.name + "/moving_var", {L.Cout}, false);
    n.tensors[ti].ptr = L.mv;
  }
  if (L.cond_fold) {
    ICS_TRY(n.alloc(&L.cond_T, (size_t)n.maxB * 27 * L.Cout));
  } else if (L.CinG != L.Cin) {
    ICS_TRY(n.alloc(&L.pad_in, M * L.CinG));
    if (need_bwd) ICS_TRY(n.alloc(&L.dw_phys, (size_t)L.taps * L.CinG * L.Cout));
  }
  if (pooled) {
    ICS_TRY(n.alloc(&L.pooled, M / 8 * L.Cout));
    ICS_TRY(n.alloc(&L.pool_idx, M / 8 * L.Cout));
    if (need_bwd && L.has_bn && L.Cout % 4 == 0) {
      ICS_TRY(n.alloc(&L.tie_mask, M / 8 * L.Cout));
      ICS_TRY(n.alloc(&L.tie_ssum, M / 8 * L.Cout));
      ICS_TRY(n.alloc(&L.bn_sums, (size_t)2 * L.Cout));
    }
  }
  return 0;
}

static ConvSrc src_plain(const float* p, int C) { return ConvSrc{p, nullptr, nullptr, C, 0, ACT_NONE, 0}; }
static ConvSrc src_layer(const ConvLayer& L, int up) {
  if (L.has_bn) return ConvSrc{L.s, L.scale, L.shift, L.Cout, up, L.post_act, 0};
  return ConvSrc{L.s, nullptr, nullptr, L.Cout, up, ACT_NONE, 0};
}

static ConvGeom geom_fwd(const ConvLayer& L, int B) {
  return ConvGeom{B, L.S, ilog2(L.S), L.CinG, L.Cout, L.taps, L.Kpad, L.Npad, L.flags};
}
static ConvGeom geom_bwd(const ConvLayer& L, int B) {
  return ConvGeom{B, L.S, ilog2(L.S), L.Cout, L.CinG, L.taps, L.Kpad_b, L.Npad_b, L.flags};
}

static ConvGeom geom_up_wgrad(const ConvLayer& L, int B) {
  return ConvGeom{B, L.S / 2, ilog2(L.S / 2), L.Cu, 27 * L.Cout, 1, round_up(L.Cu, 32), L.ldS, L.flags | (L.up8 ? CF_UP8 : 0)};
}
static ConvGeom geom_up_dgrad(const ConvLayer& L, int B) {
  return ConvGeom{B, L.S / 2, ilog2(L.S / 2), L.ldS, L.Cu, 1, L.ldS, round_up(L.Cu, 32), L.flags | (L.up8 ? CF_UP8 : 0)};
}
static ConvGeom geom_skip_wgrad(const ConvLayer& L, int B) {
  return ConvGeom{B, L.S, ilog2(L.S), L.Cs, L.Cout, L.taps, round_up(L.taps * L.Cs, 32), L.Npad, L.flags};
}
static ConvGeom geom_skip_dgrad(const ConvLayer& L, int B) {
  return ConvGeom{B, L.S, ilog2(L.S), L.Cout, L.Cs, L.taps, L.Kpad_b, round_up(L.Cs, 32), L.flags};
}
static ConvGeom geom_skip_fwd(const ConvLayer& L, int B) {
  return ConvGeom{B, L.S, ilog2(L.S), L.Cs, L.Cout, L.taps, round_up(L.taps * L.Cs, 32), L.Npad, L.flags};
}
static ConvGeom geom_par_fwd(const ConvLayer& L, int B) {
  return ConvGeom{B, L.S / 2, ilog2(L.S / 2), L.Cu, L.Cout, 8, 8 * L.Cu, L.Npad, L.flags};
}
static ConvSrc src_lowres(const ConvLayer& L) { ConvSrc u = L.src[L.nsrc - 1]; u.up = 0; return u; }

static bool up8_ok(const Net& n, const ConvLayer& L) {
  if (n.flags & CF_NO_UP8) return false;
  const size_t S3 = (size_t)(L.S / 2) * (L.S / 2) * (L.S / 2);
  if (L.Cout % 32 || L.Cu % 64 || !up8_shape_ok(L.S, L.Cout, (size_t)n.maxB * S3, n.maxB)) return false;
  for (int b = 1; b <= n.maxB; ++b)
    if (!conv_fwd_up8_tile_ok(geom_up_dgrad(L, b))) return false;
  return true;
}

constexpr size_t kUp125MinRows = 2048;
static bool up125_layer_ok(const Net& n, const ConvLayer& L) {
  if ((n.flags & CF_NO_UP125) || !L.up8 || n.side_on || n.sync() != nullptr) return false;
  if (!up125_shape_ok(L.S, L.Cout, L.Cu, n.maxB)) return false;
  if (n.flags & CF_FORCE_UP125) return true;
  return L.Cout % 128 == 0 && L.Cu % 128 == 0 && up125_geom(n.maxB, L.S, L.Cout, L.Cu).rows >= kUp125MinRows;
}
static bool up125_ok(const Net& n, const ConvLayer& L, int B) {
  if (!L.up125) return false;
  return (n.flags & CF_FORCE_UP125) || up125_geom(B, L.S, L.Cout, L.Cu).rows >= kUp125MinRows;
}
static size_t up125_splits(const ConvLayer& L, int B, Up125Splits* sp) {
  const int rows = (int)up125_geom(B, L.S, L.Cout, L.Cu).rows;
  size_t off = 0;
  for (int g = 0; g < 4; ++g) {
    const int nz = up125_group_classes(g), nb = 8 >> g;
    sp->off[g] = off;
    sp->ks[g] = wgrad_zbatch_splits(nz, rows, L.Cu, nb * L.Cout);
    off += (size_t)nz * sp->ks[g] * L.Cu * nb * L.Cout;
  }
  return off;
}

static int enable_split_up(Net& n, ConvLayer& L) {
  if (n.flags & CF_NO_UPSPLIT) return 0;
  const ConvSrc& up = L.src[L.nsrc - 1];
  const int Cs = L.nsrc == 2 ? L.src[0].C : 0;
  if (!up.up || (L.nsrc == 2 && L.src[0].up) || L.taps != 27 || L.S < 2 || L.CinG != L.Cin || Cs % 32 || up.C % 32 ||
      up.bcast || L.Cout % 4)
    return 0;
  L.split_up = true;
  L.Cs = Cs; L.Cu = up.C;
  L.ldS = round_up(27 * L.Cout, 32);
  const size_t M = n.rows(L, n.maxB);
  ICS_TRY(n.alloc(&L.w_up, (size_t)L.ldS * round_up(L.Cu, 32)));
  L.up8 = up8_ok(n, L);
  if (L.up8) {
    const size_t n8 = 8 * up8_volume_floats(n.maxB, L.S / 2, L.Cout);
    ICS_TRY(n.alloc(&L.dy8, n8));
    ICS_HIP(hipMemsetAsync(L.dy8, 0, n8 * sizeof(float), n.st));
  } else {
    ICS_TRY(n.alloc(&L.dyS, M / 8 * L.ldS));
    ICS_HIP(hipMemsetAsync(L.dyS, 0, M / 8 * L.ldS * sizeof(float), n.st));
  }
  L.up125 = up125_layer_ok(n, L);
  if (L.up125) {
    ICS_TRY(n.alloc(&L.w125, up125_weight_floats(L.Cout, L.Cu)));
    const size_t rows = up125_geom(n.maxB, L.S, L.Cout, L.Cu).rows;
    n.u125_P_n = std::max(n.u125_P_n, up125_pooled_floats(rows, L.Cout));
    n.u125_X_n = std::max(n.u125_X_n, up125_class_floats(rows, L.Cu));
    Up125Splits sp;
    for (int b = 1; b <= n.maxB; ++b)
      if (up125_ok(n, L, b)) n.u125_ws_n = std::max(n.u125_ws_n, up125_splits(L, b, &sp));
  }
  ICS_TRY(n.alloc(&L.dxl, M / 8 * L.Cu));
  ICS_TRY(n.alloc(&L.dw_up, (size_t)L.Cu * 27 * L.Cout));
  if (conv_up3_ok(geom_par_fwd(L, n.maxB), src_lowres(L)))
    ICS_TRY(n.alloc(&L.w_up3, conv_up3_weight_floats(L.Cu, L.Cout)));
  else if (L.Cs == 0 && conv_up3n_ok(geom_par_fwd(L, n.maxB), src_lowres(L)))
    ICS_TRY(n.alloc(&L.w_up3n, conv_up3n_weight_floats(L.Cu, L.Cout)));
  else
    ICS_TRY(n.alloc(&L.wp_par, (size_t)8 * 8 * L.Cu * L.Npad));
  if (L.Cs) {
    ICS_TRY(n.alloc(&L.wf_skip, (size_t)L.Kpad_b * round_up(L.Cs, 32)));
    ICS_TRY(n.alloc(&L.dA_skip, M * L.Cs));
    ICS_TRY(n.alloc(&L.wp_skip, (size_t)round_up(L.taps * L.Cs, 32) * L.Npad));
  }
  return 0;
}

static ConvGeom geom_wino_fwd(const ConvLayer& L, int B) { return L.split_up ? geom_skip_fwd(L, B) : geom_fwd(L, B); }
static ConvGeom geom_wino_bwd(const ConvLayer& L, int B) {
  if (L.split_up) return geom_skip_dgrad(L, B);
  ConvGeom g = geom_bwd(L, B);
  g.Cout = L.Cin;
  return g;
}
static int enable_wino(Net& n, ConvLayer& L, bool need_bwd) {
  if ((n.flags & CF_NO_WINO) || L.taps != 27 || L.pad_in || L.cond_fold || L.CinG != L.Cin) return 0;
  if (L.split_up ? L.Cs == 0 : L.nsrc != 1) return 0;
  const int K = L.split_up ? L.Cs : L.Cin;
  if (conv_wino_ok(geom_wino_fwd(L, n.maxB), L.src, 1)) {
    ICS_TRY(n.alloc(&L.ww, conv_wino_weight_floats(K, L.Cout)));
    L.ww_layout = conv_wino_layout(geom_wino_fwd(L, n.maxB));
  }
  const ConvSrc sdy = src_plain(nullptr, L.Cout);
  if (need_bwd && conv_wino_ok(geom_wino_bwd(L, n.maxB), &sdy, 1)) {
    ICS_TRY(n.alloc(&L.wwb, conv_wino_weight_floats(K, L.Cout)));
    L.wwb_layout = conv_wino_layout(geom_wino_bwd(L, n.maxB));
  }
  L.wino_w = need_bwd && conv_wino_wgrad_ok(L.split_up ? geom_skip_wgrad(L, n.maxB) : geom_fwd(L, n.maxB), L.src, 1);
  return 0;
}

static int enable_winog(Net& n, ConvLayer& L, bool need_bwd) {
  if (L.ww || L.taps != 27 || L.pad_in || L.cond_fold || L.CinG != L.Cin || L.split_up || L.nsrc != 1) return 0;
  const ConvGeom g = geom_fwd(L, n.maxB);
  if (!conv_winog_ok(g, L.src, 1)) return 0;
  size_t v, m, z;
  conv_winog_scratch_floats(g, &v, &m, &z);
  ICS_TRY(n.alloc(&L.wg, conv_winog_weight_floats(L.Cin, L.Cout)));
  ICS_TRY(n.alloc(&L.wg_v, v));
  ICS_TRY(n.alloc(&L.wg_m, m));
  if (need_bwd) {
    ConvGeom gb = geom_bwd(L, n.maxB);
    gb.Cout = L.Cin;
    const ConvSrc sdy = src_plain(nullptr, L.Cout);
    if (conv_winog_ok(gb, &sdy, 1)) ICS_TRY(n.alloc(&L.wgb, conv_winog_weight_floats(L.Cin, L.Cout)));
    L.wg_w = true;
    ICS_TRY(n.alloc(&L.wg_vt, (size_t)64 * n.maxB * 8 * L.Cin));
    ICS_TRY(n.alloc(&L.wg_z, z));
    ICS_TRY(n.alloc(&L.wg_du, (size_t)64 * L.Cin * L.Cout));
  }
  return 0;
}

static int alloc_workspaces(Net& n, bool need_bwd) {
  size_t stat = 0, bwd = 0, wg = 0, fw = 0;
  for (int b = 1; b <= n.maxB; ++b)
  for (auto& Lp : n.layers) {
    ConvLayer& L = *Lp;
    const size_t M = n.rows(L, b);
    const ConvGeom g = geom_fwd(L, b);
    const int rpb = std::min(conv_fwd_rows_per_block(g), 64);
    stat = std::max(stat, (M + rpb - 1) / rpb * 3 * (size_t)L.Npad);
    if (L.split_up) stat = std::max(stat, 8 * ((M / 8 + 63) / 64) * 3 * (size_t)L.Npad);
    fw = std::max(fw, conv_fwd_workspace_floats(g, L.src, L.nsrc));
    if (need_bwd) {
      const ConvSrc sdy = src_plain(L.dy, L.Cout);
      fw = std::max(fw, conv_fwd_workspace_floats(geom_bwd(L, b), &sdy, 1));
      if (L.split_up) {
        const ConvSrc sd = src_plain(L.up8 ? L.dy8 : L.dyS, L.ldS);
        fw = std::max(fw, conv_fwd_workspace_floats(geom_up_dgrad(L, b), &sd, 1));
        if (L.Cs) fw = std::max(fw, conv_fwd_workspace_floats(geom_skip_dgrad(L, b), &sdy, 1));
      }
      LayerBwd lb{};
      lb.B = b; lb.S = L.S; lb.lgS = ilog2(L.S); lb.C = L.Cout;
      if (&L != n.head) bwd = std::max(bwd, layer_bwd_workspace_floats(lb));
      wg = std::max(wg, conv_wgrad_workspace_floats(g, L.src, L.nsrc));
      if (L.wino_w)
        wg = std::max(wg, conv_wino_wgrad_workspace_floats(L.split_up ? geom_skip_wgrad(L, b) : g));
      if ((L.Cin == 1 || L.cond_fold) && (L.Cout == 16 || L.Cout == 32))
        wg = std::max(wg, conv_thin_c_wgrad_workspace_floats(g));
      if (L.split_up) {
        const ConvSrc lo = src_lowres(L);
        wg = std::max(wg, conv_wgrad_workspace_floats(geom_up_wgrad(L, b), &lo, 1));
        if (L.Cs) wg = std::max(wg, conv_wgrad_workspace_floats(geom_skip_wgrad(L, b), L.src, 1));
      }
    }
  }
  n.ws_stat_n = stat; n.ws_bwd_n = std::max(bwd, (size_t)4096 * 128); n.ws_wgrad_n = wg;
  ICS_TRY(n.alloc(&n.ws_stat, stat + 16));
  n.ws_fwd_n = std::max(fw, (size_t)768 * 64 * 64);
  ICS_TRY(n.alloc(&n.ws_fwd, n.ws_fwd_n + 16));
  if (need_bwd) {
    ICS_TRY(n.alloc(&n.ws_bwd, n.ws_bwd_n + 16));
    ICS_TRY(n.alloc(&n.ws_wgrad, wg + 16));
    if (n.u125_P_n && n.u125_P == nullptr) {
      ICS_TRY(n.alloc(&n.u125_P, n.u125_P_n));
      ICS_TRY(n.alloc(&n.u125_X, n.u125_X_n));
      ICS_TRY(n.alloc(&n.u125_O, n.u125_X_n));
      ICS_TRY(n.alloc(&n.u125_ws, n.u125_ws_n));
    }
    size_t b2 = 0;
    for (auto& Lp : n.layers)
      if (Lp->has_bn) b2 = std::max(b2, (size_t)2 * Lp->Npad * ((n.rows(*Lp, n.maxB) + 63) / 64));
    n.ws_bwd2_n = b2;
    ICS_TRY(n.alloc(&n.ws_bwd2, b2 + 16));
    size_t cls = 0; int cmax = 0;
    for (auto& Lp : n.layers)
      if (Lp->taps == 27 && Lp->S >= 3 && Lp->Cout % 4 == 0) {
        for (int b = 1; b <= n.maxB; ++b) cls = std::max(cls, conv_bnfuse_partial_floats(b, Lp->S, Lp->Cout));
        cmax = std::max(cmax, Lp->Cout);
      }
    n.ws_cls_n = cls;
    ICS_TRY(n.alloc(&n.ws_cls, cls + 16));
    ICS_TRY(n.alloc(&n.ws_R, (size_t)48 * cmax + 16));
    size_t pl = 0;
    for (auto& Lp : n.layers)
      if (Lp->tie_mask) pl = std::max(pl, pool_bnfuse_partial_doubles(n.rows(*Lp, n.maxB) / 8, Lp->Cout));
    n.ws_pool_n = pl;
    ICS_TRY(n.alloc(&n.ws_pool, pl + 16));
    if (const char* e = getenv("ICSG3D_DGRAD_BNFUSE_MIN")) n.bnfuse_min_bytes = (size_t)atoll(e);
  }
  n.ws_dbl_n = 1 << 16;
  for (auto& Lp : n.layers)
    if (Lp->cond_fold) n.ws_dbl_n = std::max(n.ws_dbl_n, cond_wgrad_workspace_doubles(n.maxB, Lp->Cout));
  ICS_TRY(n.alloc(&n.ws_dbl, n.ws_dbl_n));
  ICS_TRY(n.alloc(&n.d_metrics, (size_t)16));
  ICS_TRY(n.alloc(&n.d_red, (size_t)16));
  return 0;
}

static int alloc_params(Net& n) {
  ICS_TRY(n.alloc(&n.P, n.nparams)); ICS_TRY(n.alloc(&n.G, n.nparams));
  ICS_TRY(n.alloc(&n.Mo, n.nparams)); ICS_TRY(n.alloc(&n.Vo, n.nparams));
  for (auto& t : n.tensors)
    if (t.trainable) t.ptr = n.P + t.off;
  return 0;
}

__global__ void fill_kernel(float* p, size_t n, float v) {
  const size_t i = (size_t)blockIdx.x * blockDim.x + threadIdx.x;
  if (i < n) p[i] = v;
}
static int fill(Net& n, float* p, size_t cnt, float v) {
  ICS_LAUNCH(fill_kernel, dim3((unsigned)((cnt + 255) / 256)), dim3(256), 0, n.st, p, cnt, v);
  ICS_HIP(hipGetLastError());
  return 0;
}
static int init_bn_defaults(Net& n) {
  for (auto& Lp : n.layers)
    if (Lp->has_bn) {
      ICS_TRY(fill(n, n.tp(Lp->t_gamma), Lp->Cout, 1.f));
      ICS_TRY(fill(n, Lp->mv, Lp->Cout, 1.f));
    }
  return 0;
}

static int pack_layer(Net& n, ConvLayer& L, bool need_bwd) {
  const bool wino_f = L.ww != nullptr || L.wg != nullptr, wino_b = L.wwb != nullptr || L.wgb != nullptr;
  if (L.wg) ICS_TRY(launch_pack_wino(n.st, n.tp(L.t_w), L.Cin, L.Cout, 0, L.Cin, 0, L.wg, 2));
  if (need_bwd && L.wgb) ICS_TRY(launch_pack_wino(n.st, n.tp(L.t_w), L.Cin, L.Cout, 0, L.Cin, 1, L.wgb, 2));
  if (!wino_f && !L.split_up)
    ICS_TRY(launch_pack_fwd(n.st, n.tp(L.t_w), L.taps * L.CinG, L.Cout, L.wp, L.Kpad, L.Npad, 0, 0, 1,
                            L.CinG != L.Cin ? L.Cin : 0, L.CinG != L.Cin ? L.CinG : 0));
  if (need_bwd && L.wf && !wino_b && !L.split_up)
    ICS_TRY(launch_pack_bwd(n.st, n.tp(L.t_w), L.taps, L.Cin, L.Cout, L.wf, L.Kpad_b, L.Npad_b, L.Cout, 0, 1));
  if (L.split_up) {
    if (L.Cs && !wino_f)
      ICS_TRY(launch_pack_fwd_sub(n.st, n.tp(L.t_w), L.taps, L.Cin, L.Cout, 0, L.Cs, L.wp_skip,
                                  round_up(L.taps * L.Cs, 32), L.Npad));
    if (L.w_up3) ICS_TRY(launch_pack_up3(n.st, n.tp(L.t_w), L.Cin, L.Cout, L.Cs, L.Cu, L.w_up3));
    else if (L.w_up3n) ICS_TRY(launch_pack_up3n(n.st, n.tp(L.t_w), L.Cin, L.Cout, L.Cs, L.Cu, L.w_up3n));
    else ICS_TRY(launch_pack_par(n.st, n.tp(L.t_w), L.Cin, L.Cout, L.Cs, L.Cu, L.wp_par, 8 * L.Cu, L.Npad));
  }
  if (L.ww)
    ICS_TRY(launch_pack_wino(n.st, n.tp(L.t_w), L.Cin, L.Cout, 0, L.split_up ? L.Cs : L.Cin, 0, L.ww, L.ww_layout));
  if (need_bwd && L.wwb)
    ICS_TRY(launch_pack_wino(n.st, n.tp(L.t_w), L.Cin, L.Cout, 0, L.split_up ? L.Cs : L.Cin, 1, L.wwb, L.wwb_layout));
  if (need_bwd && L.split_up) {
    if (L.Cs && !wino_b)
      ICS_TRY(launch_pack_sub(n.st, n.tp(L.t_w), L.taps, L.Cin, L.Cout, 0, L.Cs, 1, L.wf_skip, L.Kpad_b,
                              round_up(L.Cs, 32)));
    ICS_TRY(launch_pack_sub(n.st, n.tp(L.t_w), L.taps, L.Cin, L.Cout, L.Cs, L.Cu, 0, L.w_up, L.ldS, round_up(L.Cu, 32)));
    if (L.up125) ICS_TRY(launch_pack_up125(n.st, n.tp(L.t_w), L.Cin, L.Cout, L.Cs, L.Cu, L.w125));
  }
  return 0;
}

static int conv_forward(Net& n, ConvLayer& L, int B, bool training, bool update_moving, const float* bias) {
  n.last_batch = B;
  const ConvGeom g = geom_fwd(L, B);
  const size_t M = n.rows(L, B);
  const bool stats = L.has_bn && training;
  int rpb = 128, par_blocks = 0;
  const bool thin1_all = L.pad_in && L.nvsrc == 1 && L.Cin == 1 && conv_thin_c_ok(g, L.vsrc[0], 1, 1) && L.Cout % 4 == 0;
  if (L.pad_in && !thin1_all) {
    n.prof.begin(n.st, "materialize_input", 0, 4.0 * M * (L.Cin + L.CinG));
    ICS_TRY(launch_materialize_input(n.st, L.vsrc, L.nvsrc, L.Cin, L.CinG, B, L.S, L.pad_in));
    n.prof.end(n.st);
  }
  if (L.split_up) {
    const ConvGeom gp = geom_par_fwd(L, B), gs = geom_skip_fwd(L, B);
    const ConvSrc lo = src_lowres(L);
    const bool only_up = L.Cs == 0;
    const bool p27 = L.w_up3 != nullptr || L.w_up3n != nullptr;
    n.prof.begin(n.st, "conv_fwd:" + L.name + ".up|", 2.0 * M / 8 * (p27 ? 27 : 64) * L.Cu * L.Cout,
                 4.0 * (M / 8 * L.Cu + M * L.Cout + (p27 ? 27.0 : 64.0) * L.Cu * L.Cout));
    if (L.w_up3n)
      ICS_TRY(launch_conv_fwd_up3n(n.st, gp, lo, L.w_up3n, bias, L.s, L.Cout, L.pre_act, stats ? n.ws_stat : nullptr,
                                   &par_blocks));
    else if (L.w_up3)
      ICS_TRY(launch_conv_fwd_up3(n.st, gp, lo, L.w_up3, only_up ? bias : nullptr, L.s, L.Cout,
                                  only_up ? L.pre_act : ACT_NONE, (only_up && stats) ? n.ws_stat : nullptr, &par_blocks, 0));
    else
      ICS_TRY(launch_conv_fwd_par(n.st, gp, lo, L.wp_par, L.s, L.Cout, only_up ? bias : nullptr,
                                  only_up ? L.pre_act : ACT_NONE, (only_up && stats) ? n.ws_stat : nullptr, &par_blocks));
    n.prof.end(n.st);
    if (!only_up) {
      n.prof.begin(n.st, "conv_fwd:" + L.name + ".skip|", 2.0 * M * 27 * L.Cs * L.Cout,
                   4.0 * (M * L.Cs + 2 * M * L.Cout + 27.0 * L.Cs * L.Cout));
      if (L.ww && conv_wino_ok(gs, L.src, 1))
        ICS_TRY(launch_conv_fwd_wino(n.st, gs, L.src[0], L.ww, bias, L.s, L.Cout, L.pre_act,
                                     stats ? n.ws_stat : nullptr, &rpb, 1, L.ww_layout));
      else
      ICS_TRY(launch_conv_fwd(n.st, gs, L.src, 1, L.wp_skip, bias, L.s, L.Cout, L.pre_act, stats ? n.ws_stat : nullptr,
                              &rpb, 1));
      n.prof.end(n.st);
      par_blocks = 0;
    }
  } else {
  n.prof.begin(n.st, "conv_fwd:" + L.name + "|", 2.0 * M * L.taps * L.Cin * L.Cout,
               4.0 * (M * L.Cin + M * L.Cout + (double)L.taps * L.Cin * L.Cout));
  if (L.cond_fold) {
    const ConvSrc& cs = L.vsrc[1];
    ICS_TRY(launch_cond_bias_table(n.st, n.tp(L.t_w), bias, cs.p, L.vsrc[0].C, cs.bcast, L.Cin, L.Cout, B, L.cond_T));
    ICS_TRY(launch_conv_fwd_thin_c(n.st, g, L.vsrc[0], L.vsrc[0].C, L.CinG, L.wp, nullptr, L.s, L.Cout, L.pre_act,
                                   stats ? n.ws_stat : nullptr, &rpb, L.cond_T));
    conv_set_last_kernel_id(L.Cout == 32 ? "cond_bias_table_kernel + conv_thin_c_fwd_kernel<1, 32>"
                                         : "cond_bias_table_kernel + conv_thin_c_fwd_kernel<1, 16>");
  } else if (L.pad_in && L.nvsrc == 1 && conv_thin_c_ok(g, L.vsrc[0], 1, L.Cin) && L.Cout % 4 == 0) {
    ICS_TRY(launch_conv_fwd_thin_c(n.st, g, L.vsrc[0], L.Cin, L.CinG, L.wp, bias, L.s, L.Cout, L.pre_act,
                                   stats ? n.ws_stat : nullptr, &rpb));
  } else if (L.ww && conv_wino_ok(g, L.src, L.nsrc)) {
    ICS_TRY(launch_conv_fwd_wino(n.st, g, L.src[0], L.ww, bias, L.s, L.Cout, L.pre_act, stats ? n.ws_stat : nullptr,
                                 &rpb, 0, L.ww_layout));
  } else if (L.wg && conv_winog_ok(g, L.src, L.nsrc)) {
    const bool keep = n.want_wgrad_inputs && L.wg_w && conv_winog_wgrad_ok(g, L.src, L.nsrc);
    ICS_TRY(launch_conv_fwd_winog(n.st, g, L.src[0], L.wg, bias, L.s, L.Cout, L.pre_act, stats ? n.ws_stat : nullptr, &rpb,
                                  L.wg_v, L.wg_m, keep ? L.wg_vt : nullptr));
    L.wg_vt_batch = keep ? B : 0;
  } else {
    ICS_TRY(launch_conv_fwd(n.st, g, L.src, L.nsrc, L.wp, bias, L.s, L.Cout, L.pre_act,
                            stats ? n.ws_stat : nullptr, &rpb, 0, n.fws(), n.ws_fwd_n));
  }
  n.prof.end(n.st);
  }
  if (L.has_bn) {
    BnParams bn{n.tp(L.t_gamma), n.tp(L.t_beta), L.mm, L.mv, L.mean, L.rstd, L.scale, L.shift};
    if (training && n.sync() == nullptr) bn.xs = L.xs;
    if (training) {
      const int nblk = par_blocks ? par_blocks : (int)((M + rpb - 1) / rpb);
      L.stat_rpb = par_blocks ? 0 : rpb; L.stat_nblk = nblk;
      ICS_TRY(launch_bn_finalize(n.st, n.ws_stat, nblk, L.Npad, bn, L.Cout, update_moving ? 1 : 0, n.bn_unbias, n.sync()));
    } else {
      ICS_TRY(launch_bn_eval_prepare(n.st, bn, L.Cout));
    }
  }
  if (L.pooled) {
    n.prof.begin(n.st, "pool_fwd", 0, 4.0 * M * L.Cout * 1.125);
    const bool ties = training && L.tie_mask != nullptr && (n.want_wgrad_inputs || n.want_tie_stats);
    L.tie_batch = ties ? B : 0;
    ICS_TRY(launch_pool_fwd(n.st, L.s, L.has_bn ? L.scale : nullptr, L.shift, L.has_bn ? L.post_act : ACT_NONE,
                            B, L.S, L.Cout, L.pooled, L.pool_idx, ties ? L.tie_mask : nullptr, ties ? L.tie_ssum : nullptr,
                            n.pool_ties_all));
    n.prof.end(n.st);
  }
  return 0;
}

__global__ void unpad_dw_kernel(const float* __restrict__ src, int Cin, int CinG, int N, size_t total,
                                float* __restrict__ dst) {
  const size_t i = (size_t)blockIdx.x * blockDim.x + threadIdx.x;
  if (i >= total) return;
  const size_t row = i / N, n = i - row * N;
  const size_t tap = row / Cin, ci = row - tap * Cin;
  dst[i] = src[(tap * CinG + ci) * N + n];
}
__global__ void axpy_strided_kernel(float* __restrict__ y, const float* __restrict__ x, size_t rows, int C, int ldx) {
  const size_t i = (size_t)blockIdx.x * blockDim.x + threadIdx.x;
  if (i >= rows * C) return;
  const size_t m = i / C, c = i - m * C;
  y[i] += x[m * ldx + c];
}
static void use_padded_input(ConvLayer& L) {
  if (L.CinG == L.Cin && !L.cond_fold) return;
  L.vsrc[0] = L.src[0]; L.vsrc[1] = L.src[1]; L.nvsrc = L.nsrc;
  L.src[0] = ConvSrc{L.pad_in, nullptr, nullptr, L.CinG, 0, ACT_NONE, 0};
  L.nsrc = 1;
}

static GradSrc gs_none() { return GradSrc{nullptr, 0, 0, GS_NONE, nullptr, nullptr}; }
static GradSrc gs_direct(const float* p, int ld, int off) { return GradSrc{p, ld, off, GS_DIRECT, nullptr, nullptr}; }
static GradSrc gs_up(const float* p, int ld, int off) { return GradSrc{p, ld, off, GS_UP, nullptr, nullptr}; }
static GradSrc gs_pool(const float* p, int ld, const ConvLayer& producer) {
  return GradSrc{p, ld, 0, GS_POOL, producer.pooled, producer.pool_idx};
}

static hipStream_t side_begin(Net& n) {
  if (!n.side_on || (n.prof.on && n.prof.filter.empty())) return n.st;
  (void)hipEventRecord(n.ev_fork, n.st);
  (void)hipStreamWaitEvent(n.st2, n.ev_fork, 0);
  n.side_dirty = true;
  return n.st2;
}
static int side_join(Net& n) {
  if (!n.side_dirty) return 0;
  ICS_HIP(hipEventRecord(n.ev_join, n.st2));
  ICS_HIP(hipStreamWaitEvent(n.st, n.ev_join, 0));
  n.side_dirty = false;
  return 0;
}

static BwdStat bwd_stat_for(Net& n, ConvLayer* next, int B) {
  BwdStat bs;
  if (next == nullptr || !next->has_bn || (n.flags & CF_NO_BWD_FOLD)) return bs;
  if ((size_t)2 * next->Npad * ((n.rows(*next, B) + 63) / 64) > n.ws_bwd2_n) return bs;
  bs.s = next->s; bs.mean = next->mean; bs.rstd = next->rstd; bs.scale = next->scale; bs.shift = next->shift;
  bs.partial = n.ws_bwd2; bs.post_act = next->post_act; bs.ld = next->Cout;
  return bs;
}
static void bwd_stat_done(ConvLayer* next, const BwdStat& bs, int blocks, int npad) {
  if (next == nullptr) return;
  next->bwd_pre_nblk = bs.partial ? blocks : 0;
  next->bwd_pre_ld = npad;
}

static bool skip_bnfuse_ok(const Net& n, const ConvLayer& L, int B) {
  const ConvLayer* P = L.skip_prod;
  if (P == nullptr || !L.split_up || L.Cs == 0 || (n.flags & CF_NO_DGRAD_BNFUSE) || n.sync() != nullptr || n.side_on) return false;
  if (!P->has_bn || P->pre_act != ACT_RELU || P->post_act != ACT_NONE || P->tie_mask == nullptr || P->xs == nullptr ||
      P->db_partial == nullptr || !P->pooled || P->Cout != L.Cs || L.src[0].p != P->s || L.src[0].scale == nullptr ||
      L.src[0].act != ACT_NONE || !n.want_wgrad_inputs || P->tie_batch != B)
    return false;
  if (!L.wino_w || !L.wwb || L.wwb_layout != 1) return false;
  if (n.rows(L, B) * (size_t)P->Cout * sizeof(float) < 2 * n.bnfuse_min_bytes) return false;
  const ConvGeom gw = geom_skip_wgrad(L, B), gd = geom_skip_dgrad(L, B);
  const ConvSrc sdy = src_plain(L.dy, L.Cout);
  return conv_bnfuse_ok(L.S, L.Cs, L.Cout) && conv_wino_wgrad_ok(gw, L.src, 1) && conv_wino_ok(gd, &sdy, 1) &&
         conv_bnfuse_partial_floats(B, L.S, L.Cout) <= n.ws_cls_n && L.Cs % 4 == 0 &&
         pool_bnfuse_partial_doubles(n.rows(L, B) / 8, P->Cout) <= n.ws_pool_n;
}
static int conv_grads_split_up(Net& n, ConvLayer& L, int B, ConvLayer* next) {
  const size_t M = n.rows(L, B);
  const double fl_skip = 2.0 * M * 27 * L.Cs * L.Cout, fl_up = 2.0 * (M / 8) * 27 * L.Cu * L.Cout;
  const bool skipfuse = skip_bnfuse_ok(n, L, B);
  ConvLayer* P = L.skip_prod;
  const float* dyp = L.up8 ? L.dy8 : L.dyS;
  const bool u125 = up125_ok(n, L, B);
  Up125Geom u5;
  Up125Splits sp5{};
  const double fl_up125 = 2.0 * (M / 64) * 125 * L.Cu * L.Cout;
  static thread_local std::string id125;
  auto mark125 = [&]() { id125 = std::string(conv_last_kernel_id()) + " UP125"; conv_set_last_kernel_id(id125.c_str()); };
  if (u125) {
    u5 = up125_geom(B, L.S, L.Cout, L.Cu);
    ICS_CHECK(up125_pooled_floats(u5.rows, L.Cout) <= n.u125_P_n && up125_class_floats(u5.rows, L.Cu) <= n.u125_X_n &&
                  up125_splits(L, B, &sp5) <= n.u125_ws_n, "up125 scratch smaller than the batch at hand");
    n.prof.begin(n.st, "pool125:" + L.name, 0, 4.0 * M * L.Cout * (1 + 125.0 / 64));
    ICS_TRY(launch_pool125(n.st, L.dy, B, L.S, L.Cout, n.u125_P, u5, (n.flags & CF_POOL125_V1) != 0));
  } else if (L.up8) {
    const double pr = (double)(L.S / 2 + 1) / (L.S / 2);
    n.prof.begin(n.st, "pool8:" + L.name, 0, 4.0 * M * L.Cout * (1 + pr * pr * pr));
    ICS_TRY(launch_pool8(n.st, L.dy, B, L.S, L.Cout, L.dy8, up8_geom(B, L.S / 2, ilog2(L.S / 2), L.Cout)));
  } else {
    n.prof.begin(n.st, "pool27:" + L.name, 0, 4.0 * M * L.Cout * (1 + 27.0 / 8));
    ICS_TRY(launch_pool27(n.st, L.dy, B, L.S, L.Cout, L.dyS, L.ldS));
  }
  n.prof.end(n.st);
  hipStream_t ws = side_begin(n);
  if (L.Cs) {
    const ConvGeom g = geom_skip_wgrad(L, B);
    n.prof.begin(ws, "conv_wgrad:" + L.name + ".skip|", fl_skip,
                 4.0 * (M * L.Cs + M * L.Cout + 27.0 * L.Cs * L.Cout));
    const bool wino = L.wino_w && conv_wino_wgrad_ok(g, L.src, 1);
    ConvSrc sx = L.src[0];
    if (skipfuse) { sx.scale = P->xs; sx.shift = P->xs + P->Cout; }
    if (wino)
      ICS_TRY(launch_conv_wgrad_wino(ws, g, sx, L.dy, L.Cout, n.tg(L.t_w), L.Cout, n.ws_wgrad, n.ws_wgrad_n,
                                     L.Cs, L.Cin, 0, 1));
    else
    ICS_TRY(launch_conv_wgrad(ws, g, L.src, 1, L.dy, L.Cout, n.tg(L.t_w), L.Cout, n.ws_wgrad, n.ws_wgrad_n, L.Cs,
                              L.Cin, 0, 1));
    n.prof.end(ws);
    n.prof.begin(ws, "wgrad_reduce_splits", 0, 0);
    if (wino)
      ICS_TRY(launch_conv_wgrad_wino(ws, g, sx, L.dy, L.Cout, n.tg(L.t_w), L.Cout, n.ws_wgrad, n.ws_wgrad_n,
                                     L.Cs, L.Cin, 0, 2));
    else
    ICS_TRY(launch_conv_wgrad(ws, g, L.src, 1, L.dy, L.Cout, n.tg(L.t_w), L.Cout, n.ws_wgrad, n.ws_wgrad_n, L.Cs,
                              L.Cin, 0, 2));
    n.prof.end(ws);
    if (skipfuse) {
      const bool pend = L.db_blocks > 0;
      n.prof.begin(ws, "bnfuse:" + L.name + ".skip", 0, 0);
      ICS_TRY(launch_conv_bnfuse(ws, L.dy, B, L.S, L.Cs, L.Cin, L.Cout, pend ? L.db_partial : n.tg(L.t_b), pend ? L.db_blocks : 1,
                                 n.tp(L.t_w), n.tg(L.t_w), n.tp(P->t_gamma), n.tp(P->t_beta), P->mean, P->rstd, P->scale,
                                 nullptr, nullptr, nullptr, nullptr, n.ws_cls, n.ws_cls_n, n.ws_R, P->bn_sums));
      n.prof.end(ws);
      P->deferred_skip = &L;
    }
  }
  if (u125) {
    const ConvSrc lo = src_lowres(L);
    const size_t rows = u5.rows;
    n.prof.begin(ws, "up125_xclass:" + L.name, 0, 4.0 * (M / 8 * L.Cu) * (1 + 27.0 / 8));
    ICS_TRY(launch_up125_xclass(ws, lo, n.u125_X, u5));
    n.prof.end(ws);
    n.prof.begin(ws, "conv_wgrad:" + L.name + ".up|", fl_up125, 4.0 * rows * (27.0 * L.Cu + 125.0 * L.Cout));
    for (int g = 0; g < 4; ++g)
      ICS_TRY(launch_wgrad_zbatch(ws, up125_group_classes(g), (int)rows, L.Cu, (8 >> g) * L.Cout,
                                  n.u125_X + (size_t)up125_group_slot0(g) * rows * L.Cu,
                                  n.u125_P + (size_t)up125_group_block0(g) * rows * L.Cout, n.u125_ws + sp5.off[g], sp5.ks[g]));
    mark125();
    n.prof.end(ws);
    n.prof.begin(ws, "wgrad_reduce_splits", 0, 0);
    ICS_TRY(launch_up125_contract(ws, n.u125_ws, sp5, L.dw_up, u5));
    ICS_TRY(launch_permute_up_dw(ws, L.dw_up, L.Cu, L.Cout, L.Cin, L.Cs, n.tg(L.t_w)));
    n.prof.end(ws);
  } else {
    const ConvGeom g = geom_up_wgrad(L, B);
    const ConvSrc lo = src_lowres(L);
    n.prof.begin(ws, "conv_wgrad:" + L.name + ".up|", fl_up,
                 4.0 * (M / 8 * L.Cu + M / 8 * 27.0 * L.Cout + 27.0 * L.Cu * L.Cout));
    ICS_TRY(launch_conv_wgrad(ws, g, &lo, 1, dyp, L.ldS, L.dw_up, 27 * L.Cout, n.ws_wgrad, n.ws_wgrad_n, 0, 0, 0, 1));
    n.prof.end(ws);
    n.prof.begin(ws, "wgrad_reduce_splits", 0, 0);
    ICS_TRY(launch_conv_wgrad(ws, g, &lo, 1, dyp, L.ldS, L.dw_up, 27 * L.Cout, n.ws_wgrad, n.ws_wgrad_n, 0, 0, 0, 2));
    ICS_TRY(launch_permute_up_dw(ws, L.dw_up, L.Cu, L.Cout, L.Cin, L.Cs, n.tg(L.t_w)));
    n.prof.end(ws);
  }
  if (L.Cs && !skipfuse) {
    const ConvGeom g = geom_skip_dgrad(L, B);
    ConvSrc sdy = src_plain(L.dy, L.Cout);
    n.prof.begin(n.st, "conv_dgrad:" + L.name + ".skip|", fl_skip,
                 4.0 * (M * L.Cs + M * L.Cout + 27.0 * L.Cs * L.Cout));
    if (L.wwb && conv_wino_ok(g, &sdy, 1))
      ICS_TRY(launch_conv_fwd_wino(n.st, g, sdy, L.wwb, nullptr, L.dA_skip, L.Cs, ACT_NONE, nullptr, nullptr, 0,
                                   L.wwb_layout));
    else
    ICS_TRY(launch_conv_fwd(n.st, g, &sdy, 1, L.wf_skip, nullptr, L.dA_skip, L.Cs, ACT_NONE, nullptr, nullptr, 0,
                            n.fws(), n.ws_fwd_n));
    n.prof.end(n.st);
  }
  if (u125) {
    const size_t rows = u5.rows;
    n.prof.begin(n.st, "conv_dgrad:" + L.name + ".up|", fl_up125, 4.0 * rows * (27.0 * L.Cu + 125.0 * L.Cout));
    for (int g = 0; g < 4; ++g)
      ICS_TRY(launch_gemm_zbatch(n.st, up125_group_classes(g), (int)rows, (8 >> g) * L.Cout, L.Cu,
                                 n.u125_P + (size_t)up125_group_block0(g) * rows * L.Cout,
                                 L.w125 + (size_t)up125_group_block0(g) * L.Cout * L.Cu,
                                 n.u125_O + (size_t)up125_group_slot0(g) * rows * L.Cu, L.flags));
    mark125();
    n.prof.end(n.st);
    n.prof.begin(n.st, "up125_combine:" + L.name, 0, 4.0 * (M / 8 * L.Cu) * (1 + 27.0 / 8));
    ICS_TRY(launch_up125_combine(n.st, n.u125_O, L.dxl, u5));
    n.prof.end(n.st);
    bwd_stat_done(next, BwdStat{}, 0, round_up(L.Cu, 32));
  } else {
    const ConvGeom g = geom_up_dgrad(L, B);
    ConvSrc sd = src_plain(dyp, L.ldS);
    n.prof.begin(n.st, "conv_dgrad:" + L.name + ".up|", fl_up,
                 4.0 * (M / 8 * L.Cu + M / 8 * 27.0 * L.Cout + 27.0 * L.Cu * L.Cout));
    const BwdStat bs = bwd_stat_for(n, next, B);
    int blocks = 0;
    ICS_TRY(launch_conv_fwd(n.st, g, &sd, 1, L.w_up, nullptr, L.dxl, L.Cu, ACT_NONE, nullptr, nullptr, 0, n.fws(),
                            n.ws_fwd_n, &bs, &blocks));
    bwd_stat_done(next, bs, blocks, g.Npad);
    n.prof.end(n.st);
  }
  return 0;
}

static int colsum_push(Net& n, const float* partial, int nblk, int C, float* out);
static bool dgrad_bnfuse_ok(const Net& n, const ConvLayer& L, const ConvLayer* next, int B, bool need_dA, bool param_grads) {
  if (next == nullptr || !need_dA || !param_grads || (n.flags & CF_NO_DGRAD_BNFUSE) || n.sync() != nullptr || n.side_on)
    return false;
  if (!next->has_bn || next->pre_act != ACT_RELU || next->post_act != ACT_NONE || next->xs == nullptr ||
      next->db_partial == nullptr || next->dy == nullptr)
    return false;
  if (L.split_up || L.nsrc != 1 || L.taps != 27 || !L.wino_w || !L.wwb || L.CinG != L.Cin ||
      L.Cin != next->Cout || L.src[0].p != next->s || L.src[0].scale == nullptr || L.src[0].act != ACT_NONE || L.dw_phys)
    return false;
  if (n.rows(L, B) * (size_t)next->Cout * sizeof(float) < n.bnfuse_min_bytes) return false;
  const ConvGeom g = geom_fwd(L, B);
  ConvGeom gb = geom_bwd(L, B);
  gb.Cout = L.Cin;
  const ConvSrc sdy = src_plain(L.dy, L.Cout);
  return conv_bnfuse_ok(L.S, L.Cin, L.Cout) && conv_wino_wgrad_ok(g, L.src, 1) && conv_wino_ok(gb, &sdy, 1) &&
         conv_bnfuse_partial_floats(B, L.S, L.Cout) <= n.ws_cls_n && L.Cin % 4 == 0;
}
static int conv_grads_from_dy(Net& n, ConvLayer& L, int B, bool need_dA, bool param_grads, ConvLayer* next) {
  if (L.split_up && need_dA && param_grads) return conv_grads_split_up(n, L, B, next);
  if (L.split_up) next = nullptr;
  const ConvGeom g = geom_fwd(L, B);
  const size_t M = n.rows(L, B);
  const bool bnfuse = dgrad_bnfuse_ok(n, L, next, B, need_dA, param_grads);
  if (param_grads) {
    hipStream_t ws = side_begin(n);
    n.prof.begin(ws, "conv_wgrad:" + L.name + "|", 2.0 * M * L.taps * L.Cin * L.Cout,
                 4.0 * (M * L.Cin + M * L.Cout + (double)L.taps * L.Cin * L.Cout));
    float* dw = L.dw_phys ? L.dw_phys : n.tg(L.t_w);
    const bool thin1 = L.pad_in && L.nvsrc == 1 && L.Cin == 1 && conv_thin_c_ok(g, L.vsrc[0], 1, 1) && L.Cout % 4 == 0;
    if (L.cond_fold) {
      const ConvSrc& cs = L.vsrc[1];
      const int C0 = L.vsrc[0].C;
      ICS_TRY(launch_conv_wgrad_thin_c(ws, g, L.vsrc[0], L.dy, L.Cout, n.tg(L.t_w), L.Cout, L.Cin, n.ws_wgrad,
                                       n.ws_wgrad_n, 0));
      ICS_TRY(launch_cond_wgrad(ws, L.dy, B, L.S, L.Cout, cs.p, C0, cs.C, cs.bcast, L.Cin, n.tg(L.t_w), n.ws_dbl,
                                n.ws_dbl_n));
      conv_set_last_kernel_id(L.Cout == 32 ? "conv_thin_c_wgrad_kernel<32> + cond_wgrad_kernel"
                                           : "conv_thin_c_wgrad_kernel<16> + cond_wgrad_kernel");
      n.prof.end(ws);
    } else if (thin1) {
      ICS_TRY(launch_conv_wgrad_thin_c(ws, g, L.vsrc[0], L.dy, L.Cout, n.tg(L.t_w), L.Cout, L.Cin, n.ws_wgrad,
                                       n.ws_wgrad_n, 1));
      n.prof.end(ws);
      n.prof.begin(ws, "wgrad_reduce_splits", 0, 0);
      ICS_TRY(launch_conv_wgrad_thin_c(ws, g, L.vsrc[0], L.dy, L.Cout, n.tg(L.t_w), L.Cout, L.Cin, n.ws_wgrad,
                                       n.ws_wgrad_n, 2));
      n.prof.end(ws);
    } else if (L.wg_w && L.wg_vt_batch == B && conv_winog_wgrad_ok(g, L.src, L.nsrc)) {
      ICS_TRY(launch_conv_wgrad_winog(ws, g, L.wg_vt, L.dy, L.Cout, dw, L.Cout, 0, 0, L.wg_z, L.wg_du));
      n.prof.end(ws);
    } else if (L.wino_w && !L.split_up && conv_wino_wgrad_ok(g, L.src, L.nsrc)) {
      ConvSrc sx = L.src[0];
      if (bnfuse) {
        sx.scale = next->xs; sx.shift = next->xs + next->Cout;
      }
      ICS_TRY(launch_conv_wgrad_wino(ws, g, sx, L.dy, L.Cout, dw, L.Cout, n.ws_wgrad, n.ws_wgrad_n, 0, 0, 0, 1));
      n.prof.end(ws);
      n.prof.begin(ws, "wgrad_reduce_splits", 0, 0);
      ICS_TRY(launch_conv_wgrad_wino(ws, g, sx, L.dy, L.Cout, dw, L.Cout, n.ws_wgrad, n.ws_wgrad_n, 0, 0, 0, 2));
      n.prof.end(ws);
      if (bnfuse) {
        const bool pend = L.db_blocks > 0;
        n.prof.begin(ws, "bnfuse:" + L.name, 0, 0);
        ICS_TRY(launch_conv_bnfuse(ws, L.dy, B, L.S, L.Cin, L.Cin, L.Cout, pend ? L.db_partial : n.tg(L.t_b), pend ? L.db_blocks : 1,
                                   n.tp(L.t_w), dw, n.tp(next->t_gamma), n.tp(next->t_beta), next->mean, next->rstd,
                                   next->scale, next->abc, next->c1c2, n.tg(next->t_gamma), n.tg(next->t_beta), n.ws_cls,
                                   n.ws_cls_n, n.ws_R));
        n.prof.end(ws);
      }
    } else {
    ICS_TRY(launch_conv_wgrad(ws, g, L.src, L.nsrc, L.dy, L.Cout, dw, L.Cout, n.ws_wgrad, n.ws_wgrad_n, 0, 0, 0, 1));
    n.prof.end(ws);
    n.prof.begin(ws, "wgrad_reduce_splits", 0, 0);
    ICS_TRY(launch_conv_wgrad(ws, g, L.src, L.nsrc, L.dy, L.Cout, dw, L.Cout, n.ws_wgrad, n.ws_wgrad_n, 0, 0, 0, 2));
    if (L.dw_phys) {
      const size_t cnt = (size_t)L.taps * L.Cin * L.Cout;
      ICS_LAUNCH(unpad_dw_kernel, dim3((unsigned)((cnt + 255) / 256)), dim3(256), 0, ws, L.dw_phys, L.Cin,
                         L.CinG, L.Cout, cnt, n.tg(L.t_w));
      ICS_HIP(hipGetLastError());
    }
    n.prof.end(ws);
    }
  }
  if (need_dA) {
    ConvGeom gb = geom_bwd(L, B);
    gb.Cout = L.Cin;
    ConvSrc sdy = src_plain(L.dy, L.Cout);
    n.prof.begin(n.st, "conv_dgrad:" + L.name + "|", 2.0 * M * L.taps * L.Cin * L.Cout,
                 4.0 * (M * L.Cin + M * L.Cout + (double)L.taps * L.Cin * L.Cout));
    int blocks = 0;
    if (bnfuse) {
      BwdStat ba{};
      ba.s = next->s; ba.ld = next->Cout; ba.abc = next->abc; ba.db_partial = next->db_partial;
      ICS_TRY(launch_conv_fwd_wino(n.st, gb, sdy, L.wwb, nullptr, next->dy, next->Cout, ACT_NONE, nullptr, nullptr, 0,
                                   L.wwb_layout, &ba, &blocks));
      n.prof.end(n.st);
      ICS_CHECK(blocks > 0, "fused BatchNorm-backward apply: the backward-data launch did not take it");
      ICS_CHECK((size_t)blocks <= next->db_rows, "bias-gradient partial buffer too small for this batch");
      next->dy_ready = true;
      next->db_blocks = 0;
      ICS_TRY(colsum_push(n, next->db_partial, blocks, next->Cout, n.tg(next->t_b)));
      next->db_blocks = blocks;
      return 0;
    }
    const BwdStat bs = bwd_stat_for(n, next, B);
    if (L.wwb && !L.split_up && conv_wino_ok(gb, &sdy, 1))
      ICS_TRY(launch_conv_fwd_wino(n.st, gb, sdy, L.wwb, nullptr, L.dA, L.CinG, ACT_NONE, nullptr, nullptr, 0,
                                   L.wwb_layout, &bs, &blocks));
    else if (L.wgb && conv_winog_ok(gb, &sdy, 1))
      ICS_TRY(launch_conv_fwd_winog(n.st, gb, sdy, L.wgb, nullptr, L.dA, L.CinG, ACT_NONE, nullptr, nullptr, L.wg_v, L.wg_m,
                                    nullptr));
    else {
      if (L.split_up && L.wf_stale) {
        ICS_TRY(launch_pack_bwd(n.st, n.tp(L.t_w), L.taps, L.Cin, L.Cout, L.wf, L.Kpad_b, L.Npad_b, L.Cout, 0, 1));
        L.wf_stale = false;
      }
      ICS_TRY(launch_conv_fwd(n.st, gb, &sdy, 1, L.wf, nullptr, L.dA, L.CinG, ACT_NONE, nullptr, nullptr, 0, n.fws(),
                              n.ws_fwd_n, &bs, &blocks));
    }
    bwd_stat_done(next, bs, blocks, gb.Npad);
    n.prof.end(n.st);
  }
  return 0;
}

static int colsum_push(Net& n, const float* partial, int nblk, int C, float* out) {
  ColsumJobs& J = n.colsum;
  if (J.n == 24) { ICS_TRY(launch_colsum_batch(n.st, J)); J.n = 0; }
  if (J.n == 0) J.blk0[0] = 0;
  J.partial[J.n] = partial; J.out[J.n] = out; J.nblk[J.n] = nblk; J.C[J.n] = C;
  J.blk0[J.n + 1] = J.blk0[J.n] + colsum_blocks(C);
  J.n += 1;
  return 0;
}
static int colsum_flush(Net& n) {
  ICS_TRY(launch_colsum_batch(n.st, n.colsum));
  n.colsum.n = 0;
// ... 2947 lines not shown
```

### icsg3d_amd/csrc/up125.h

```cpp
#pragma once
#include <stddef.h>

#if defined(__HIPCC__) || defined(__CUDACC__)
#define ICS_UP125_HD __host__ __device__ constexpr inline
#define ICS_UP125_F __host__ __device__ inline
#else
#define ICS_UP125_HD constexpr inline
#define ICS_UP125_F inline
#endif

enum { UP125_D1 = 0, UP125_R0 = 1, UP125_Q1 = 2, UP125_D2 = 3, UP125_R1 = 4 };

ICS_UP125_HD int up125_cls(int t) { return t < 2 ? 0 : (t == 2 ? 1 : 2); }
ICS_UP125_HD int up125_e(int t) { return t < 2 ? t : (t == 2 ? 0 : t - 3); }
ICS_UP125_HD int up125_n(int c) { return c == 1 ? 1 : 2; }
ICS_UP125_HD int up125_type(int c, int e) { return c == 0 ? e : (c == 1 ? UP125_Q1 : 3 + e); }
ICS_UP125_HD int up125_coef(int t, int f) {
  return t == UP125_D1 ? (f < 2 ? 1 : (f < 4 ? -1 : 0))
       : t == UP125_R0 ? (f == 1 || f == 2)
       : t == UP125_Q1 ? (f == 2 || f == 3)
       : t == UP125_D2 ? ((f == 2 || f == 3) ? 1 : (f >= 4 ? -1 : 0))
                       : (f == 3 || f == 4);
}
ICS_UP125_HD int up125_wcoef(int t, int i) {
  return t == UP125_D1 ? (i == 2) : t == UP125_Q1 ? (i != 1) : t == UP125_D2 ? -(i == 0) : (i == 1);
}

ICS_UP125_HD int up125_nB(int q) { return (q / 9 == 1) + ((q / 3) % 3 == 1) + (q % 3 == 1); }
ICS_UP125_HD int up125_nb(int q) { return 8 >> up125_nB(q); }
ICS_UP125_HD int up125_group_slot0(int g) { return g == 0 ? 0 : (g == 1 ? 8 : (g == 2 ? 20 : 26)); }
ICS_UP125_HD int up125_group_block0(int g) { return g == 0 ? 0 : (g == 1 ? 64 : (g == 2 ? 112 : 124)); }
ICS_UP125_HD int up125_group_classes(int g) { return g == 0 ? 8 : (g == 1 ? 12 : (g == 2 ? 6 : 1)); }
ICS_UP125_HD int up125_slot(int q) {
  const int g = up125_nB(q);
  int r = 0;
  for (int p = 0; p < q; ++p) r += up125_nB(p) == g;
  return up125_group_slot0(g) + r;
}
ICS_UP125_HD int up125_class_of_slot(int s) {
  for (int q = 0; q < 27; ++q)
    if (up125_slot(q) == s) return q;
  return -1;
}
ICS_UP125_HD int up125_bbase(int q) {
  const int g = up125_nB(q);
  return up125_group_block0(g) + (up125_slot(q) - up125_group_slot0(g)) * (8 >> g);
}
ICS_UP125_HD int up125_block(int q, int tz, int ty, int tx) {
  return (up125_e(tz) * up125_n((q / 3) % 3) + up125_e(ty)) * up125_n(q % 3) + up125_e(tx);
}

struct Up125Geom {
  int T = 0, lgT = 0;
  int N = 0, Cu = 0;
  unsigned rows = 0;
  unsigned char slot[27] = {};
  unsigned char bbase[27] = {};
};

inline Up125Geom up125_geom(int B, int S, int N, int Cu) {
  Up125Geom u;
  u.T = S / 4;
  while ((1 << u.lgT) < u.T) ++u.lgT;
  u.N = N; u.Cu = Cu;
  u.rows = (unsigned)B * (unsigned)u.T * (unsigned)u.T * (unsigned)u.T;
  for (int q = 0; q < 27; ++q) { u.slot[q] = (unsigned char)up125_slot(q); u.bbase[q] = (unsigned char)up125_bbase(q); }
  return u;
}

ICS_UP125_HD size_t up125_pooled_floats(size_t rows, int N) { return 125 * rows * (size_t)N; }
ICS_UP125_HD size_t up125_class_floats(size_t rows, int Cu) { return 27 * rows * (size_t)Cu; }
ICS_UP125_HD size_t up125_weight_floats(int N, int Cu) { return (size_t)125 * N * Cu; }

ICS_UP125_F size_t up125_pooled_off(const Up125Geom& u, int q, size_t row, int b, int n) {
  return ((size_t)u.bbase[q] * u.rows + row * (size_t)up125_nb(q) + (size_t)b) * (size_t)u.N + (size_t)n;
}
ICS_UP125_F size_t up125_class_off(const Up125Geom& u, int q, size_t row, int c) {
  return ((size_t)u.slot[q] * u.rows + row) * (size_t)u.Cu + (size_t)c;
}

ICS_UP125_HD bool up125_shape_ok(int S, int N, int Cu, int B) {
  if (S < 8 || (S & (S - 1)) != 0 || N < 32 || (N & (N - 1)) != 0 || Cu < 64 || Cu % 64 != 0 || B < 1) return false;
  const size_t rows = (size_t)B * (S / 4) * (S / 4) * (S / 4);
  const size_t w = (size_t)(8 * N > Cu ? 8 * N : Cu);
  return rows * w < ((size_t)1 << 30);
}

enum { UP125_POOL_WAVES = 6, UP125_POOL_ROUNDS = 5, UP125_XCH_ELEMS = 6 * 5 * 64 };
ICS_UP125_F void up125_pool_lane(int lgc, unsigned bx, unsigned by, int lane, unsigned* tile, int* n) {
  *n = (int)(((by << lgc) + ((unsigned)lane & ((1u << lgc) - 1u))) * 4u);
  *tile = bx * (64u >> lgc) + ((unsigned)lane >> lgc);
}
ICS_UP125_HD int up125_xch_off(int fz, int tx, int lane) { return (fz * 5 + tx) * 64 + lane; }
template <class V>
ICS_UP125_F void up125_xline(const V* v, V* xr) {
  const V q0 = v[0] + v[1], q1 = v[2] + v[3], q2 = v[4] + v[5];
  xr[UP125_D1] = q0 - q1; xr[UP125_R0] = v[1] + v[2]; xr[UP125_Q1] = q1; xr[UP125_D2] = q1 - q2; xr[UP125_R1] = v[3] + v[4];
}
template <class V>
ICS_UP125_F void up125_yacc(int fy, const V* xr, V* S) {
#pragma unroll
  for (int ty = 0; ty < 5; ++ty) {
    const int s = up125_coef(ty, fy);
    if (s == 0) continue;
#pragma unroll
    for (int tx = 0; tx < 5; ++tx) {
      if (s > 0) S[ty * 5 + tx] += xr[tx]; else S[ty * 5 + tx] -= xr[tx];
    }
  }
}
template <class V>
ICS_UP125_F V up125_zcomb(int tz, const V* s) {
  return tz == UP125_D1 ? (s[0] + s[1]) - (s[2] + s[3])
       : tz == UP125_R0 ? s[1] + s[2]
       : tz == UP125_Q1 ? s[2] + s[3]
       : tz == UP125_D2 ? (s[2] + s[3]) - (s[4] + s[5])
                        : s[3] + s[4];
}

ICS_UP125_HD size_t up125_pack_pieces(int N, int Cu) { return (size_t)25 * (N / 4) * Cu; }
ICS_UP125_F void up125_pack_piece(size_t i, const float* w, int Cin_total, int N, int c_off, int Cu, float* dst) {
  const int c = (int)(i % (size_t)Cu);
  size_t r = i / (size_t)Cu;
  const int n = (int)(r % (size_t)(N / 4)) * 4;
  r /= (size_t)(N / 4);
  const int ty = (int)(r % 5), tz = (int)(r / 5);
  float sx[3][4] = {};
  for (int iz = 0; iz < 3; ++iz)
    for (int iy = 0; iy < 3; ++iy) {
      const int s = up125_wcoef(tz, iz) * up125_wcoef(ty, iy);
      if (s == 0) continue;
      for (int ix = 0; ix < 3; ++ix) {
        const float* p = w + ((size_t)((iz * 3 + iy) * 3 + ix) * Cin_total + c_off + c) * N + n;
        for (int k = 0; k < 4; ++k) sx[ix][k] += (float)s * p[k];
      }
    }
  for (int tx = 0; tx < 5; ++tx) {
    const int q = up125_cls(tz) * 9 + up125_cls(ty) * 3 + up125_cls(tx);
    const int k0 = up125_block(q, tz, ty, tx) * N + n;
    float* d = (float*)__builtin_assume_aligned(dst + (size_t)up125_bbase(q) * N * Cu + ((size_t)(k0 / 4) * Cu + c) * 4, 16);
    for (int k = 0; k < 4; ++k) {
      float v = 0.f;
      for (int ix = 0; ix < 3; ++ix) {
        const int s = up125_wcoef(tx, ix);
        if (s != 0) v += (float)s * sx[ix][k];
      }
      d[k] = v;
    }
  }
}

ICS_UP125_F float up125_weight_value(size_t i, const float* w, int Cin_total, int N, int c_off, int Cu, int q) {
  const int tq = (int)(i & 3);
  const size_t rest = i >> 2;
  const int c = (int)(rest % (size_t)Cu);
  const int k = (int)(rest / (size_t)Cu) * 4 + tq;
  int b = k / N;
  const int n = k - b * N;
  const int cz = q / 9, cy = (q / 3) % 3, cx = q % 3;
  const int ex = b % up125_n(cx); b /= up125_n(cx);
  const int ey = b % up125_n(cy); b /= up125_n(cy);
  const int tz = up125_type(cz, b), ty = up125_type(cy, ey), tx = up125_type(cx, ex);
  float v = 0.f;
  for (int iz = 0; iz < 3; ++iz)
    for (int iy = 0; iy < 3; ++iy)
      for (int ix = 0; ix < 3; ++ix) {
        const int s = up125_wcoef(tz, iz) * up125_wcoef(ty, iy) * up125_wcoef(tx, ix);
        if (s != 0) v += (float)s * w[((size_t)((iz * 3 + iy) * 3 + ix) * Cin_total + c_off + c) * N + n];
      }
  return v;
}
```

### icsg3d_amd/csrc/up125.hip

```cpp
#include "common.h"
#include "elementwise.h"
#include "up125.h"
#include "scratch.h"
#include "icsg3d.h"

#include <algorithm>
#include <string>

namespace ics {

typedef float qf4 __attribute__((ext_vector_type(4)));

template <int TZ>
__device__ __forceinline__ void pool125_body(const float* __restrict__ dy, int S, int N, int b, int jz, int jy, int jx,
                                             unsigned tile, int n, float* __restrict__ out, const Up125Geom& u) {
  qf4 acc[5][5];
#pragma unroll
  for (int k = 0; k < 25; ++k) acc[k / 5][k % 5] = qf4{0.f, 0.f, 0.f, 0.f};
#pragma unroll
  for (int fz = 0; fz < 6; ++fz) {
    const int cz = up125_coef(TZ, fz);
    if (cz == 0) continue;
    const int z = 4 * jz - 1 + fz;
    if ((unsigned)z >= (unsigned)S) continue;
// ... 21 lines not shown
          if (s > 0) acc[ty][tx] += xr[tx]; else acc[ty][tx] -= xr[tx];
        }
      }
    }
  }
#pragma unroll
  for (int ty = 0; ty < 5; ++ty)
#pragma unroll
    for (int tx = 0; tx < 5; ++tx) {
      const int q = up125_cls(TZ) * 9 + up125_cls(ty) * 3 + up125_cls(tx);
      *reinterpret_cast<qf4*>(out + up125_pooled_off(u, q, tile, up125_block(q, TZ, ty, tx), n)) = acc[ty][tx];
    }
}
__global__ __launch_bounds__(320) void pool125_kernel(const float* __restrict__ dy, int S, int lgc,
                                                      float* __restrict__ out, Up125Geom u) {
  const int tz = threadIdx.x >> 6, lane = threadIdx.x & 63;
  const int n = (((int)blockIdx.y << lgc) + (lane & ((1 << lgc) - 1))) * 4;
  const unsigned tile = blockIdx.x * (64u >> lgc) + (unsigned)(lane >> lgc);
  if (tile >= u.rows) return;
  const int T = u.T, lg = u.lgT;
  const int jx = tile & (T - 1), jy = (tile >> lg) & (T - 1), jz = (tile >> (2 * lg)) & (T - 1), b = tile >> (3 * lg);
  switch (tz) {
    case 0: pool125_body<0>(dy, S, u.N, b, jz, jy, jx, tile, n, out, u); break;
    case 1: pool125_body<1>(dy, S, u.N, b, jz, jy, jx, tile, n, out, u); break;
    case 2: pool125_body<2>(dy, S, u.N, b, jz, jy, jx, tile, n, out, u); break;
    case 3: pool125_body<3>(dy, S, u.N, b, jz, jy, jx, tile, n, out, u); break;
    default: pool125_body<4>(dy, S, u.N, b, jz, jy, jx, tile, n, out, u); break;
  }
}
template <int TZ>
__device__ __forceinline__ void pool125_zstore(const qf4* __restrict__ buf, int lane, int ty, bool live, unsigned tile, int n,
                                               float* __restrict__ out, const Up125Geom& u) {
#pragma unroll
  for (int tx = 0; tx < 5; ++tx) {
    qf4 s[6];
#pragma unroll
    for (int fz = 0; fz < 6; ++fz)
      s[fz] = up125_coef(TZ, fz) != 0 ? buf[up125_xch_off(fz, tx, lane)] : qf4{0.f, 0.f, 0.f, 0.f};
    const qf4 v = up125_zcomb(TZ, s);
    const int q = up125_cls(TZ) * 9 + up125_cls(ty) * 3 + up125_cls(tx);
    if (live) *reinterpret_cast<qf4*>(out + up125_pooled_off(u, q, tile, up125_block(q, TZ, ty, tx), n)) = v;
  }
}
__global__ __launch_bounds__(64 * UP125_POOL_WAVES) void pool125_planes_kernel(const float* __restrict__ dy, int S, int lgc,
                                                                               float* __restrict__ out, Up125Geom u) {
  __shared__ qf4 xch[2][UP125_XCH_ELEMS];
  const int fz = threadIdx.x >> 6, lane = threadIdx.x & 63;
  unsigned tile;
  int n;
  up125_pool_lane(lgc, blockIdx.x, blockIdx.y, lane, &tile, &n);
  const bool live = tile < u.rows;
  const int T = u.T, lg = u.lgT, N = u.N;
  const int jx = tile & (T - 1), jy = (tile >> lg) & (T - 1), jz = (tile >> (2 * lg)) & (T - 1), b = tile >> (3 * lg);
  qf4 Sa[25];
#pragma unroll
  for (int k = 0; k < 25; ++k) Sa[k] = qf4{0.f, 0.f, 0.f, 0.f};
  const int z = 4 * jz - 1 + fz;
  const bool zok = live && (unsigned)z < (unsigned)S;
#pragma unroll
  for (int fy = 0; fy < 6; ++fy) {
    const int y = 4 * jy - 1 + fy;
    const bool yok = zok && (unsigned)y < (unsigned)S;
    const float* line = dy + (yok ? ((((size_t)b * S + z) * S + y) * S) * (size_t)N + n : (size_t)0);
    qf4 v[6];
#pragma unroll
    for (int fx = 0; fx < 6; ++fx) {
      const int x = 4 * jx - 1 + fx;
      const bool ok = yok && (unsigned)x < (unsigned)S;
      v[fx] = ok ? *reinterpret_cast<const qf4*>(line + (size_t)(ok ? x : 0) * N) : qf4{0.f, 0.f, 0.f, 0.f};
    }
    qf4 xr[5];
    up125_xline(v, xr);
    up125_yacc(fy, xr, Sa);
  }
#pragma unroll
  for (int ty = 0; ty < UP125_POOL_ROUNDS; ++ty) {
    qf4* buf = xch[ty & 1];
#pragma unroll
    for (int tx = 0; tx < 5; ++tx) buf[up125_xch_off(fz, tx, lane)] = Sa[ty * 5 + tx];
    __syncthreads();
    switch (fz) {
      case 0: pool125_zstore<0>(buf, lane, ty, live, tile, n, out, u); break;
      case 1: pool125_zstore<1>(buf, lane, ty, live, tile, n, out, u); break;
      case 2: pool125_zstore<2>(buf, lane, ty, live, tile, n, out, u); break;
      case 3: pool125_zstore<3>(buf, lane, ty, live, tile, n, out, u); break;
      case 4: pool125_zstore<4>(buf, lane, ty, live, tile, n, out, u); break;
      default: break;
    }
  }
}
int launch_pool125(hipStream_t st, const float* dy, int B, int S, int N, float* out, const Up125Geom& u, bool v1) {
  ICS_CHECK(up125_shape_ok(S, N, u.Cu, B) && u.T == S / 4 && u.N == N && (1 << u.lgT) == u.T &&
                u.rows == (unsigned)B * (unsigned)(u.T * u.T * u.T),
            "pool125: layout does not match the shape");
  int lgc = 0;
  while ((1 << lgc) < std::min(N / 4, 64)) ++lgc;
  const unsigned tpw = 64u >> lgc;
  const dim3 grid((u.rows + tpw - 1) / tpw, (unsigned)((N / 4) >> lgc));
  if (v1) ICS_LAUNCH(pool125_kernel, grid, dim3(320), 0, st, dy, S, lgc, out, u);
  else ICS_LAUNCH(pool125_planes_kernel, grid, dim3(64 * UP125_POOL_WAVES), 0, st, dy, S, lgc, out, u);
  ICS_HIP(hipGetLastError());
  return 0;
}

__global__ __launch_bounds__(256) void up125_xclass_kernel(ConvSrc s, size_t total, float* __restrict__ out, Up125Geom u) {
  const size_t i = (size_t)blockIdx.x * blockDim.x + threadIdx.x;
  if (i >= total) return;
  const int C4 = u.Cu >> 2, T = u.T, lg = u.lgT, Sh = 2 * T;
  const int c = (int)(i % C4) * 4;
  const unsigned tile = (unsigned)(i / C4);
  const int jx = tile & (T - 1), jy = (tile >> lg) & (T - 1), jz = (tile >> (2 * lg)) & (T - 1), b = tile >> (3 * lg);
  const bool aff = s.scale != nullptr;
  qf4 sc = qf4{1.f, 1.f, 1.f, 1.f}, sh = qf4{0.f, 0.f, 0.f, 0.f};
  if (aff) { sc = *reinterpret_cast<const qf4*>(s.scale + c); sh = *reinterpret_cast<const qf4*>(s.shift + c); }
  const float slope = aff ? (s.act == ACT_RELU ? 0.f : (s.act == ACT_LRELU ? kLeaky : 1.f)) : 1.f;
  qf4 X[3][3][3];
#pragma unroll
  for (int ez = 0; ez < 2; ++ez)
#pragma unroll
    for (int ey = 0; ey < 2; ++ey) {
      qf4 p[2];
#pragma unroll
      for (int ex = 0; ex < 2; ++ex) {
        const size_t vox = (((size_t)b * Sh + 2 * jz + ez) * Sh + 2 * jy + ey) * Sh + 2 * jx + ex;
        qf4 v = *reinterpret_cast<const qf4*>(s.p + vox * (size_t)s.C + c);
        if (aff) {
          v.x = fmaf(v.x, sc.x, sh.x); v.y = fmaf(v.y, sc.y, sh.y); v.z = fmaf(v.z, sc.z, sh.z); v.w = fmaf(v.w, sc.w, sh.w);
          v.x = fmaxf(v.x, v.x * slope); v.y = fmaxf(v.y, v.y * slope); v.z = fmaxf(v.z, v.z * slope); v.w = fmaxf(v.w, v.w * slope);
        }
        p[ex] = v;
      }
      X[2 * ez][2 * ey][0] = p[0]; X[2 * ez][2 * ey][1] = p[0] + p[1]; X[2 * ez][2 * ey][2] = p[1];
    }
#pragma unroll
  for (int ez = 0; ez < 2; ++ez)
#pragma unroll
    for (int cx = 0; cx < 3; ++cx) X[2 * ez][1][cx] = X[2 * ez][0][cx] + X[2 * ez][2][cx];
#pragma unroll
  for (int cy = 0; cy < 3; ++cy)
#pragma unroll
    for (int cx = 0; cx < 3; ++cx) X[1][cy][cx] = X[0][cy][cx] + X[2][cy][cx];
#pragma unroll
  for (int q = 0; q < 27; ++q)
    *reinterpret_cast<qf4*>(out + up125_class_off(u, q, tile, c)) = X[q / 9][(q / 3) % 3][q % 3];
}
int launch_up125_xclass(hipStream_t st, const ConvSrc& s, float* out, const Up125Geom& u) {
  ICS_CHECK(s.C == u.Cu && u.Cu % 4 == 0 && !s.up && !s.bcast && u.rows > 0, "up125 x classes: plain low-res source required");
  const size_t total = (size_t)u.rows * (u.Cu / 4);
  ICS_LAUNCH(up125_xclass_kernel, dim3((unsigned)((total + 255) / 256)), dim3(256), 0, st, s, total, out, u);
  ICS_HIP(hipGetLastError());
  return 0;
}

__global__ __launch_bounds__(256) void up125_combine_kernel(const float* __restrict__ cls, size_t total,
                                                            float* __restrict__ dxl, Up125Geom u) {
  const size_t i = (size_t)blockIdx.x * blockDim.x + threadIdx.x;
  if (i >= total) return;
  const int C4 = u.Cu >> 2, T = u.T, lg = u.lgT, Sh = 2 * T;
  const int c = (int)(i % C4) * 4;
  const unsigned tile = (unsigned)(i / C4);
  const int jx = tile & (T - 1), jy = (tile >> lg) & (T - 1), jz = (tile >> (2 * lg)) & (T - 1), b = tile >> (3 * lg);
  qf4 O[3][3][3];
#pragma unroll
  for (int q = 0; q < 27; ++q) O[q / 9][(q / 3) % 3][q % 3] = *reinterpret_cast<const qf4*>(cls + up125_class_off(u, q, tile, c));
#pragma unroll
  for (int ez = 0; ez < 2; ++ez)
#pragma unroll
    for (int ey = 0; ey < 2; ++ey)
#pragma unroll
      for (int ex = 0; ex < 2; ++ex) {
        qf4 v = qf4{0.f, 0.f, 0.f, 0.f};
#pragma unroll
        for (int k = 0; k < 8; ++k) v += O[ez + (k >> 2)][ey + ((k >> 1) & 1)][ex + (k & 1)];
        const size_t vox = (((size_t)b * Sh + 2 * jz + ez) * Sh + 2 * jy + ey) * Sh + 2 * jx + ex;
        *reinterpret_cast<qf4*>(dxl + vox * (size_t)u.Cu + c) = v;
      }
}
int launch_up125_combine(hipStream_t st, const float* cls, float* dxl, const Up125Geom& u) {
  ICS_CHECK(u.Cu % 4 == 0 && u.rows > 0, "up125 combine: channels must be a multiple of 4");
  const size_t total = (size_t)u.rows * (u.Cu / 4);
  ICS_LAUNCH(up125_combine_kernel, dim3((unsigned)((total + 255) / 256)), dim3(256), 0, st, cls, total, dxl, u);
  ICS_HIP(hipGetLastError());
  return 0;
}

__global__ __launch_bounds__(256) void up125_contract_kernel(const float* __restrict__ ws, Up125Splits p, size_t total,
                                                             float* __restrict__ dw, Up125Geom u) {
  const size_t i = (size_t)blockIdx.x * blockDim.x + threadIdx.x;
  if (i >= total) return;
  const int N4 = u.N >> 2;
  const int n = (int)(i % N4) * 4;
  const int tap = (int)((i / N4) % 27);
  const int cu = (int)(i / ((size_t)N4 * 27));
  const int iz = tap / 9, iy = (tap / 3) % 3, ix = tap % 3;
  qf4 v = qf4{0.f, 0.f, 0.f, 0.f};
  for (int tz = 0; tz < 5; ++tz) {
    const int sz = up125_wcoef(tz, iz);
    if (sz == 0) continue;
    for (int ty = 0; ty < 5; ++ty) {
      const int sy = sz * up125_wcoef(ty, iy);
      if (sy == 0) continue;
      for (int tx = 0; tx < 5; ++tx) {
        const int s = sy * up125_wcoef(tx, ix);
        if (s == 0) continue;
        const int q = up125_cls(tz) * 9 + up125_cls(ty) * 3 + up125_cls(tx);
        const int g = up125_nB(q), nb = 8 >> g, ks = p.ks[g];
        const size_t ld = (size_t)nb * u.N;
        const float* base = ws + p.off[g] + ((size_t)(u.slot[q] - up125_group_slot0(g)) * ks * u.Cu + cu) * ld +
                            (size_t)up125_block(q, tz, ty, tx) * u.N + n;
        const size_t st = (size_t)u.Cu * ld;
        qf4 a0 = qf4{0.f, 0.f, 0.f, 0.f}, a1 = a0, a2 = a0, a3 = a0;
        int k = 0;
        for (; k + 4 <= ks; k += 4) {
          a0 += *reinterpret_cast<const qf4*>(base + (size_t)k * st);
          a1 += *reinterpret_cast<const qf4*>(base + (size_t)(k + 1) * st);
          a2 += *reinterpret_cast<const qf4*>(base + (size_t)(k + 2) * st);
          a3 += *reinterpret_cast<const qf4*>(base + (size_t)(k + 3) * st);
        }
        for (; k < ks; ++k) a0 += *reinterpret_cast<const qf4*>(base + (size_t)k * st);
        const qf4 a = (a0 + a1) + (a2 + a3);
        if (s > 0) v += a; else v -= a;
      }
    }
  }
  *reinterpret_cast<qf4*>(dw + ((size_t)cu * 27 + tap) * u.N + n) = v;
}
int launch_up125_contract(hipStream_t st, const float* ws, const Up125Splits& p, float* dw, const Up125Geom& u) {
  ICS_CHECK(u.N % 4 == 0, "up125 contraction: channels must be a multiple of 4");
  const size_t total = (size_t)u.Cu * 27 * (u.N / 4);
  ICS_LAUNCH(up125_contract_kernel, dim3((unsigned)((total + 255) / 256)), dim3(256), 0, st, ws, p, total, dw, u);
  ICS_HIP(hipGetLastError());
  return 0;
}

__global__ void pack_up125_kernel(const float* __restrict__ w, int Cin_total, int N, int c_off, int Cu, size_t total,
                                  float* __restrict__ dst) {
  const size_t i = (size_t)blockIdx.x * blockDim.x + threadIdx.x;
  if (i < total) up125_pack_piece(i, w, Cin_total, N, c_off, Cu, dst);
}
int launch_pack_up125_pieces(hipStream_t st, const float* w, int Cin_total, int N, int c_off, int Cu, float* dst) {
  const size_t total = up125_pack_pieces(N, Cu);
  ICS_LAUNCH(pack_up125_kernel, dim3((unsigned)((total + 255) / 256)), dim3(256), 0, st, w, Cin_total, N, c_off, Cu, total, dst);
  ICS_HIP(hipGetLastError());
  return 0;
}

}

using namespace ics;

extern "C" {

int ics_op_up125_pool(const float* dy, int B, int S, int N, int variant, float* out) {
  const std::string op = "ics_op_up125_pool: ";
  ICS_CHECK(dy && out, op + "dy and out are required");
  ICS_CHECK(variant == 0 || variant == 1, op + "variant is 0 (one wave per z type) or 1 (one wave per fine plane)");
  ICS_CHECK(up125_shape_ok(S, N, 64, B), op + "need S a power of two >= 8, N = 32 * 2^k and B (S/4)^3 * 8 N < 2^30");
  const Up125Geom u = up125_geom(B, S, N, 64);
  const size_t cnt = (size_t)B * S * S * S * N, pooled = up125_pooled_floats(u.rows, N);
  hipStream_t st;
  ICS_TRY(op_stream(&st));
  Layout L;
  const auto s_dy = L.add<float>(cnt);
  const auto s_out = L.add<float>(pooled);
  float *d_dy, *d_out;
  ICS_TRY(L.reserve(s_dy, &d_dy, s_out, &d_out));
  ICS_TRY(L.upload(s_dy, dy, cnt, st));
  ICS_TRY(launch_pool125(st, d_dy, B, S, N, d_out, u, variant == 0));
  ICS_TRY(L.download(out, s_out, pooled, st));
  ICS_HIP(hipStreamSynchronize(st));
  return 0;
}

}
```

Before: 1189.

## Group up125 wgrad into one launch and fold BN-backward stats into combine

Replaces the four per-group z-batched weight-gradient launches for the 125-tap upsample conv with a single grouped launch. A block-index decoder maps each workgroup to a class, column tile, row tile and split, and the split count is sized to fill a fixed resident-workgroup target. The up125 combine kernel can also compute the next layer's BN-backward partial sums (dy·act' and dy·x̂) while it writes dxl, which saves a separate reduction pass over that tensor. The cost is more complex index math, extra shared memory and a barrier in combine, and a different split plan and workspace layout.

```diff
diff --git a/icsg3d_amd/csrc/common.h b/icsg3d_amd/csrc/common.h
--- a/icsg3d_amd/csrc/common.h
+++ b/icsg3d_amd/csrc/common.h
@@ -114,6 +114,7 @@
   CF_NO_UP125 = 1 << 27,
   CF_FORCE_UP125 = 1 << 28,
   CF_POOL125_V1 = 1 << 29,
+  CF_UP125_UNGROUPED = 1 << 30,
   CF_ZBATCH = 1 << 20,
 };
 int conv_flags_from_env();
@@ -219,6 +220,7 @@
                             int row_pitch, int row_off, float* z_scratch, float* m_scratch);
 int launch_gemm_zbatch(hipStream_t st, int nz, int M, int K, int N, const float* A, const float* Wp, float* out, int flags);
 int wgrad_zbatch_splits(int nz, int M, int K, int N);
+int launch_wgrad_up125(hipStream_t st, int M, int Cu, int N, const float* x, const float* dy, float* ws);
 int launch_wgrad_zbatch(hipStream_t st, int nz, int M, int K, int N, const float* x, const float* dy, float* ws, int ksplit);
 int launch_pack_up125(hipStream_t st, const float* w, int Cin_total, int N, int c_off, int Cu, float* dst);
 int launch_pack_up125_pieces(hipStream_t st, const float* w, int Cin_total, int N, int c_off, int Cu, float* dst);
diff --git a/icsg3d_amd/csrc/conv_igemm.hip b/icsg3d_amd/csrc/conv_igemm.hip
--- a/icsg3d_amd/csrc/conv_igemm.hip
+++ b/icsg3d_amd/csrc/conv_igemm.hip
@@ -1,4 +1,5 @@
 #include "common.h"
+#include "up125.h"
 
 #ifndef ICS_GEMM_DEEP_FWD_MIN
 #define ICS_GEMM_DEEP_FWD_MIN 1
@@ -64,6 +65,7 @@
   if (getenv("ICSG3D_NO_UP125")) f |= CF_NO_UP125;
   if (getenv("ICSG3D_FORCE_UP125")) f |= CF_FORCE_UP125;
   if (getenv("ICSG3D_POOL125_V1")) f |= CF_POOL125_V1;
+  if (getenv("ICSG3D_UP125_UNGROUPED")) f |= CF_UP125_UNGROUPED;
   { const char* e = getenv("ICSG3D_UP3_BIG_MIN_WG"); if (e && *e && strtoul(e, nullptr, 10) <= 1) f |= CF_UP3_BIG_ALWAYS; }
   return f;
 }
@@ -1894,7 +1896,7 @@
 
 
 template <int WM, int WN, int TM, int TN, bool VEC, bool DYVEC, bool AFF = true, bool UP = true, bool THIN = false,
-          int ABL = 0, bool UP8 = false, bool ZB = false>
+          int ABL = 0, bool UP8 = false, int ZB = 0>
 __global__ __launch_bounds__(256) void conv_wgrad_kernel(ConvGeom g, ConvSrc s0, ConvSrc s1,
                                                           const float* __restrict__ dy, int ldy,
                                                           int n_load,
@@ -1915,16 +1917,28 @@
   const int S = g.S, lg = g.lgS;
   const int M = g.B << (3 * lg);
   const int K = g.taps * g.Cin;
-  if (ZB) {
+  if (ZB == 1) {
     s0.p += (size_t)blockIdx.y * (size_t)M * (size_t)s0.C;
     dy += (size_t)blockIdx.y * (size_t)M * (size_t)ldy;
     ws += (size_t)blockIdx.y * (size_t)(gridDim.x / (unsigned)(ktiles * ntiles)) * (size_t)K * (size_t)g.Cout;
   }
 
   int bid = blockIdx.x;
-  const int nt_i = bid % ntiles; bid /= ntiles;
-  const int kt_i = bid % ktiles; bid /= ktiles;
-  const int split = bid;
+  int nt_i, kt_i, split;
+  if (ZB == 2) {
+    const int Nb = n_load;
+    const Up125WgradBlock wb = up125_wgrad_block(blockIdx.x, ntiles, ktiles, Nb);
+    const int Nc = (8 >> wb.g) * Nb;
+    s0.p += (size_t)wb.slot * (size_t)M * (size_t)s0.C;
+    dy += (size_t)wb.bbase * (size_t)M * (size_t)Nb;
+    ws += (size_t)wb.bbase * (size_t)(gridDim.x / (unsigned)(ktiles * ntiles)) * (size_t)K * (size_t)Nb;
+    ldy = Nc; n_load = Nc; g.Cout = Nc;
+    nt_i = wb.nt; kt_i = wb.kt; split = wb.split;
+  } else {
+    nt_i = bid % ntiles; bid /= ntiles;
+    kt_i = bid % ktiles; bid /= ktiles;
+    split = bid;
+  }
   const int n0 = nt_i * NT;
   const int m_begin = split * rows_per_split;
   const int m_end = min(M, m_begin + rows_per_split);
@@ -2689,7 +2703,7 @@
 }
 
 template <int WM, int WN, int TM, int TN, bool VEC, bool DYVEC, bool AFF = true, bool UP = true, bool THIN = false,
-          int ABL = 0, bool UP8 = false, bool ZB = false>
+          int ABL = 0, bool UP8 = false, int ZB = 0>
 static int launch_wgrad_cfg(hipStream_t st, const ConvGeom& g, const ConvSrc& s0, const ConvSrc& s1,
                             const float* dy, int ldy, int n_load, float* ws, const WgradPlan& p, int nz = 1) {
   constexpr int KT = WM * TM * 32, NT = WN * TN * 32;
@@ -2705,11 +2719,11 @@
   static const std::string id = std::string("conv_wgrad_kernel<") + std::to_string(WM) + ", " + std::to_string(WN) +
                                 ", " + std::to_string(TM) + ", " + std::to_string(TN) + ", " + tf(VEC) + ", " +
                                 tf(DYVEC) + ", " + tf(AFF) + ", " + tf(UP) + ", " + tf(THIN) + ", " +
-                                std::to_string(ABL) + (UP8 ? ", UP8>" : (ZB ? ", ZB>" : ">"));
+                                std::to_string(ABL) + (UP8 ? ", UP8>" : (ZB == 2 ? ", GZB>" : (ZB ? ", ZB>" : ">")));
   g_last_kernel_id = id.c_str();
   Up8Geom u8;
   if (UP8) u8 = up8_geom(g.B, g.S, g.lgS, g.Cout / 27);
-  ICS_LAUNCH(kern, dim3(p.ktiles * p.ntiles * p.ksplit, ZB ? nz : 1), dim3(256), lds, st, g, s0, s1, dy,
+  ICS_LAUNCH(kern, dim3(p.ktiles * p.ntiles * p.ksplit, ZB == 1 ? nz : 1), dim3(256), lds, st, g, s0, s1, dy,
                      ldy, n_load, ws, p.ktiles, p.ntiles, p.rows_per_split, u8);
   ICS_HIP(hipGetLastError());
   return 0;
@@ -2914,7 +2928,24 @@
   p.ksplit = (M + p.rows_per_split - 1) / p.rows_per_split;
   ICS_CHECK(p.ksplit <= ksplit, "z-batched wgrad: split plan");
   p.ksplit = ksplit;
-  return launch_wgrad_cfg<2, 2, 2, 2, true, true, false, false, false, 0, false, true>(st, g, s0, s1, dy, N, N, ws, p, nz);
+  return launch_wgrad_cfg<2, 2, 2, 2, true, true, false, false, false, 0, false, 1>(st, g, s0, s1, dy, N, N, ws, p, nz);
+}
+int launch_wgrad_up125(hipStream_t st, int M, int Cu, int N, const float* x, const float* dy, float* ws) {
+  ICS_CHECK(M >= 1 && Cu % 32 == 0 && N % 32 == 0, "grouped up125 wgrad: Cu % 32, N % 32 required");
+  ICS_CHECK((size_t)M * (size_t)std::max(Cu, 8 * N) < ((size_t)1 << 30), "grouped up125 wgrad: matrix too large for 32-bit offsets");
+  const Up125WgradPlan u = up125_wgrad_plan((unsigned)M, N, Cu);
+  ICS_CHECK((size_t)u.ktiles * u.ctiles * u.ks < ((size_t)1 << 31), "grouped up125 wgrad: grid");
+  const ConvGeom g{M, 1, 0, Cu, N, 1, Cu, (N + 31) / 32 * 32, 0};
+  const ConvSrc s0{x, nullptr, nullptr, Cu, 0, ACT_NONE, 0};
+  ConvSrc s1 = s0;
+  s1.C = 0;
+  WgradPlan p;
+  p.vec = true; p.thin = false;
+  p.kt = 128; p.nt = 128;
+  p.ktiles = u.ktiles; p.ntiles = u.ctiles;
+  p.rows_per_split = u.rows_per_split;
+  p.ksplit = u.ks;
+  return launch_wgrad_cfg<2, 2, 2, 2, true, true, false, false, false, 0, false, 2>(st, g, s0, s1, dy, N, N, ws, p);
 }
 
 __device__ __forceinline__ bool pack_fwd_value(size_t i, const float* __restrict__ w, int K, int N, int Npad, int k_off,
diff --git a/icsg3d_amd/csrc/elementwise.h b/icsg3d_amd/csrc/elementwise.h
--- a/icsg3d_amd/csrc/elementwise.h
+++ b/icsg3d_amd/csrc/elementwise.h
@@ -144,7 +144,7 @@
 int launch_pool8(hipStream_t st, const float* dy, int B, int S, int N, float* out, const Up8Geom& u);
 int launch_pool125(hipStream_t st, const float* dy, int B, int S, int N, float* out, const Up125Geom& u, bool v1);
 int launch_up125_xclass(hipStream_t st, const ConvSrc& s, float* out, const Up125Geom& u);
-int launch_up125_combine(hipStream_t st, const float* cls, float* dxl, const Up125Geom& u);
+int launch_up125_combine(hipStream_t st, const float* cls, float* dxl, const Up125Geom& u, const BwdStat* bs = nullptr);
 struct Up125Splits { unsigned long long off[4]; int ks[4]; };
 int launch_up125_contract(hipStream_t st, const float* ws, const Up125Splits& p, float* dw, const Up125Geom& u);
 int launch_permute_up_dw(hipStream_t st, const float* tmp, int Cu, int N, int Cin, int c_off, float* dw);
diff --git a/icsg3d_amd/csrc/engine.hip b/icsg3d_amd/csrc/engine.hip
--- a/icsg3d_amd/csrc/engine.hip
+++ b/icsg3d_amd/csrc/engine.hip
@@ -524,8 +524,16 @@
   if (!L.up125) return false;
   return (n.flags & CF_FORCE_UP125) || up125_geom(B, L.S, L.Cout, L.Cu).rows >= kUp125MinRows;
 }
-static size_t up125_splits(const ConvLayer& L, int B, Up125Splits* sp) {
+static size_t up125_splits(const Net& n, const ConvLayer& L, int B, Up125Splits* sp) {
   const int rows = (int)up125_geom(B, L.S, L.Cout, L.Cu).rows;
+  if (!(n.flags & CF_UP125_UNGROUPED)) {
+    const int ks = up125_wgrad_plan((unsigned)rows, L.Cout, L.Cu).ks;
+    for (int g = 0; g < 4; ++g) {
+      sp->off[g] = up125_wgrad_group_off(g, ks, L.Cout, L.Cu);
+      sp->ks[g] = ks;
+    }
+    return up125_wgrad_ws_floats(ks, L.Cout, L.Cu);
+  }
   size_t off = 0;
   for (int g = 0; g < 4; ++g) {
     const int nz = up125_group_classes(g), nb = 8 >> g;
@@ -565,7 +573,7 @@
     n.u125_X_n = std::max(n.u125_X_n, up125_class_floats(rows, L.Cu));
     Up125Splits sp;
     for (int b = 1; b <= n.maxB; ++b)
-      if (up125_ok(n, L, b)) n.u125_ws_n = std::max(n.u125_ws_n, up125_splits(L, b, &sp));
+      if (up125_ok(n, L, b)) n.u125_ws_n = std::max(n.u125_ws_n, up125_splits(n, L, b, &sp));
   }
   ICS_TRY(n.alloc(&L.dxl, M / 8 * L.Cu));
   ICS_TRY(n.alloc(&L.dw_up, (size_t)L.Cu * 27 * L.Cout));
@@ -679,6 +687,8 @@
     size_t b2 = 0;
     for (auto& Lp : n.layers)
       if (Lp->has_bn) b2 = std::max(b2, (size_t)2 * Lp->Npad * ((n.rows(*Lp, n.maxB) + 63) / 64));
+    for (auto& Lp : n.layers)
+      if (Lp->up125) b2 = std::max(b2, (size_t)2 * Lp->Cu * up125_combine_blocks(up125_geom(n.maxB, Lp->S, Lp->Cout, Lp->Cu)));
     n.ws_bwd2_n = b2;
     ICS_TRY(n.alloc(&n.ws_bwd2, b2 + 16));
     size_t cls = 0; int cmax = 0;
@@ -941,7 +951,7 @@
   if (u125) {
     u5 = up125_geom(B, L.S, L.Cout, L.Cu);
     ICS_CHECK(up125_pooled_floats(u5.rows, L.Cout) <= n.u125_P_n && up125_class_floats(u5.rows, L.Cu) <= n.u125_X_n &&
-                  up125_splits(L, B, &sp5) <= n.u125_ws_n, "up125 scratch smaller than the batch at hand");
+                  up125_splits(n, L, B, &sp5) <= n.u125_ws_n, "up125 scratch smaller than the batch at hand");
     n.prof.begin(n.st, "pool125:" + L.name, 0, 4.0 * M * L.Cout * (1 + 125.0 / 64));
     ICS_TRY(launch_pool125(n.st, L.dy, B, L.S, L.Cout, n.u125_P, u5, (n.flags & CF_POOL125_V1) != 0));
   } else if (L.up8) {
@@ -993,6 +1003,9 @@
     ICS_TRY(launch_up125_xclass(ws, lo, n.u125_X, u5));
     n.prof.end(ws);
     n.prof.begin(ws, "conv_wgrad:" + L.name + ".up|", fl_up125, 4.0 * rows * (27.0 * L.Cu + 125.0 * L.Cout));
+    if (!(n.flags & CF_UP125_UNGROUPED))
+      ICS_TRY(launch_wgrad_up125(ws, (int)rows, L.Cu, L.Cout, n.u125_X, n.u125_P, n.u125_ws));
+    else
     for (int g = 0; g < 4; ++g)
       ICS_TRY(launch_wgrad_zbatch(ws, up125_group_classes(g), (int)rows, L.Cu, (8 >> g) * L.Cout,
                                   n.u125_X + (size_t)up125_group_slot0(g) * rows * L.Cu,
@@ -1038,10 +1051,14 @@
                                  n.u125_O + (size_t)up125_group_slot0(g) * rows * L.Cu, L.flags));
     mark125();
     n.prof.end(n.st);
-    n.prof.begin(n.st, "up125_combine:" + L.name, 0, 4.0 * (M / 8 * L.Cu) * (1 + 27.0 / 8));
-    ICS_TRY(launch_up125_combine(n.st, n.u125_O, L.dxl, u5));
+    n.prof.begin(n.st, "up125_combine:" + L.name + "|", 0, 4.0 * (M / 8 * L.Cu) * (1 + 27.0 / 8));
+    BwdStat bs{};
+    if (!(n.flags & CF_UP125_UNGROUPED) && next != nullptr && next->Cout == L.Cu && up125_combine_fold_ok(u5) &&
+        (size_t)2 * L.Cu * up125_combine_blocks(u5) <= n.ws_bwd2_n)
+      bs = bwd_stat_for(n, next, B);
+    ICS_TRY(launch_up125_combine(n.st, n.u125_O, L.dxl, u5, bs.partial ? &bs : nullptr));
     n.prof.end(n.st);
-    bwd_stat_done(next, BwdStat{}, 0, round_up(L.Cu, 32));
+    bwd_stat_done(next, bs, bs.partial ? up125_combine_blocks(u5) : 0, L.Cu);
   } else {
     const ConvGeom g = geom_up_dgrad(L, B);
     ConvSrc sd = src_plain(dyp, L.ldS);
diff --git a/icsg3d_amd/csrc/hoststub/up125_group_check.cpp b/icsg3d_amd/csrc/hoststub/up125_group_check.cpp
--- /dev/null
+++ b/icsg3d_amd/csrc/hoststub/up125_group_check.cpp
@@ -0,0 +1,139 @@
+#include "../up125.h"
+
+#include <cstdint>
+#include <cstdio>
+#include <vector>
+
+static int g_fail = 0;
+#define CHECK(cond, ...)                                \
+  do {                                                  \
+    if (!(cond)) {                                      \
+      if (g_fail < 20) {                                \
+        fprintf(stderr, "up125_group_check FAILED: ");  \
+        fprintf(stderr, __VA_ARGS__);                   \
+        fprintf(stderr, "\n");                          \
+      }                                                 \
+      ++g_fail;                                         \
+    }                                                   \
+  } while (0)
+
+static void check_wgrad(int B, int S, int N, int Cu) {
+  CHECK(up125_shape_ok(S, N, Cu, B), "shape (B %d, S %d, N %d, Cu %d) refused", B, S, N, Cu);
+  const Up125Geom u = up125_geom(B, S, N, Cu);
+  const long rows = u.rows;
+  const Up125WgradPlan p = up125_wgrad_plan(u.rows, N, Cu);
+  const size_t allocX = up125_class_floats(rows, Cu), allocP = up125_pooled_floats(rows, N);
+  const size_t allocW = up125_wgrad_ws_floats(p.ks, N, Cu);
+  CHECK(p.ks >= 1 && p.rows_per_split % 32 == 0 && (long)p.ks * p.rows_per_split >= rows &&
+            (long)(p.ks - 1) * p.rows_per_split < rows, "splits %d x %d rows do not cut %ld rows", p.ks, p.rows_per_split, rows);
+  CHECK(p.ks == 1 || rows / p.ks >= UP125_WG_MIN_ROWS, "split of %ld rows by %d", rows, p.ks);
+  CHECK(p.ktiles * UP125_WG_TILE >= Cu && (p.ktiles - 1) * UP125_WG_TILE < Cu, "row tiles of Cu");
+  int want = 0;
+  for (int g = 0; g < 4; ++g) {
+    CHECK(up125_wg_tile0(g, N) == want, "first column tile of group %d", g);
+    want += up125_group_classes(g) * up125_wg_ctiles(g, N);
+  }
+  CHECK(p.ctiles == want && up125_wg_tile0(4, N) == want, "column tiles");
+  const size_t grid = (size_t)p.ctiles * p.ktiles * p.ks;
+  const int max_ct = up125_wg_ctiles(0, N);
+  std::vector<unsigned char> taken((size_t)27 * max_ct * p.ktiles * p.ks, 0), hitW(allocW, 0);
+  for (size_t bid = 0; bid < grid; ++bid) {
+    const Up125WgradBlock b = up125_wgrad_block((unsigned)bid, p.ctiles, p.ktiles, N);
+    const bool ok = b.g >= 0 && b.g < 4 && b.slot >= up125_group_slot0(b.g) && b.slot < up125_group_slot0(b.g) + up125_group_classes(b.g) &&
+                    b.nt >= 0 && b.nt < up125_wg_ctiles(b.g, N) && b.kt >= 0 && b.kt < p.ktiles && b.split >= 0 && b.split < p.ks;
+    CHECK(ok, "workgroup %zu maps to (group %d, slot %d, tile %d, row tile %d, split %d)", bid, b.g, b.slot, b.nt, b.kt, b.split);
+    if (!ok) continue;
+    const int q = up125_class_of_slot(b.slot);
+    CHECK(q >= 0 && up125_nB(q) == b.g && up125_bbase(q) == b.bbase, "workgroup %zu: class of slot %d", bid, b.slot);
+    const size_t id = (((size_t)b.slot * max_ct + b.nt) * p.ktiles + b.kt) * p.ks + b.split;
+    CHECK(!taken[id], "(slot %d, tile %d, row tile %d, split %d) taken twice", b.slot, b.nt, b.kt, b.split);
+    taken[id] = 1;
+    const int nb = 8 >> b.g, Nc = nb * N;
+    const long m_begin = (long)b.split * p.rows_per_split, m_end = m_begin + p.rows_per_split < rows ? m_begin + p.rows_per_split : rows;
+    CHECK(m_begin < m_end, "workgroup %zu: empty split", bid);
+    const int k0 = b.kt * UP125_WG_TILE, k1 = k0 + UP125_WG_TILE < Cu ? k0 + UP125_WG_TILE : Cu;
+    const int n0 = b.nt * UP125_WG_TILE, n1 = n0 + UP125_WG_TILE < Nc ? n0 + UP125_WG_TILE : Nc;
+    CHECK(k0 < k1 && n0 < n1, "workgroup %zu: empty tile", bid);
+    const size_t x0 = (size_t)b.slot * rows * Cu, xa = x0 + (size_t)m_begin * Cu + k0, xb = x0 + (size_t)(m_end - 1) * Cu + k1;
+    CHECK(xa >= up125_class_off(u, q, 0, 0) && xb <= up125_class_off(u, q, 0, 0) + (size_t)rows * Cu && xb <= allocX, "X of workgroup %zu", bid);
+    const size_t p0 = (size_t)b.bbase * rows * N, pa = p0 + (size_t)m_begin * Nc + n0, pb = p0 + (size_t)(m_end - 1) * Nc + n1;
+    CHECK(pa >= up125_pooled_off(u, q, 0, 0, 0) && pb <= up125_pooled_off(u, q, 0, 0, 0) + (size_t)rows * Nc && pb <= allocP, "P of workgroup %zu", bid);
+    const size_t w0 = (size_t)b.bbase * p.ks * Cu * N + (size_t)b.split * Cu * Nc;
+    for (int k = k0; k < k1; ++k)
+      for (int n = n0; n < n1; ++n) {
+        const size_t off = w0 + (size_t)k * Nc + n;
+        CHECK(off < allocW, "partial offset %zu outside %zu", off, allocW);
+        if (off < allocW) { CHECK(!hitW[off], "partial %zu written twice", off); hitW[off] = 1; }
+      }
+  }
+  size_t n_taken = 0, n_want = 0;
+  for (unsigned char t : taken) n_taken += t;
+  for (int g = 0; g < 4; ++g) n_want += (size_t)up125_group_classes(g) * up125_wg_ctiles(g, N) * p.ktiles * p.ks;
+  CHECK(n_taken == n_want && n_want == grid, "%zu of %zu (class, tile, row tile, split) taken by %zu workgroups", n_taken, n_want, grid);
+  for (size_t i = 0; i < allocW; ++i)
+    if (!hitW[i]) { CHECK(false, "partial %zu never written", i); break; }
+  std::vector<unsigned char> readW(allocW, 0);
+  for (int cu = 0; cu < Cu; ++cu)
+    for (int tap = 0; tap < 27; ++tap) {
+      const int iz = tap / 9, iy = (tap / 3) % 3, ix = tap % 3;
+      for (int tz = 0; tz < 5; ++tz)
+        for (int ty = 0; ty < 5; ++ty)
+          for (int tx = 0; tx < 5; ++tx) {
+            if (up125_wcoef(tz, iz) * up125_wcoef(ty, iy) * up125_wcoef(tx, ix) == 0) continue;
+            const int q = up125_cls(tz) * 9 + up125_cls(ty) * 3 + up125_cls(tx);
+            const int g = up125_nB(q), nb = 8 >> g;
+            const size_t ld = (size_t)nb * N;
+            const size_t base = up125_wgrad_group_off(g, p.ks, N, Cu) + ((size_t)(u.slot[q] - up125_group_slot0(g)) * p.ks * Cu + cu) * ld +
+                                (size_t)up125_block(q, tz, ty, tx) * N;
+            for (int k = 0; k < p.ks; ++k)
+              for (int n = 0; n < N; ++n) {
+                const size_t off = base + (size_t)k * Cu * ld + n;
+                CHECK(off < allocW && hitW[off], "the contraction reads partial %zu, which no workgroup wrote", off);
+                if (off < allocW) readW[off] = 1;
+              }
+          }
+    }
+  for (size_t i = 0; i < allocW; ++i)
+    if (!readW[i]) { CHECK(false, "partial %zu written and never read", i); break; }
+}
+
+static void check_combine(int B, int S, int N, int Cu) {
+  const Up125Geom u = up125_geom(B, S, N, Cu);
+  const int C4 = Cu / 4, nblk = up125_combine_blocks(u);
+  const size_t total = (size_t)u.rows * C4;
+  CHECK((size_t)nblk * 256 >= total && (size_t)(nblk - 1) * 256 < total, "combine workgroups");
+  if (!up125_combine_fold_ok(u)) { CHECK(256 % C4 != 0 || C4 > 256, "fold refused at Cu %d", Cu); return; }
+  std::vector<unsigned char> hit((size_t)2 * Cu * nblk, 0);
+  for (int blk = 0; blk < nblk; ++blk) {
+    CHECK(((size_t)blk * 256) % C4 == 0, "workgroup %d does not start on channel quad 0", blk);
+    for (int h = 0; h < 2; ++h)
+      for (int col = 0; col < Cu; ++col) {
+        const size_t off = ((size_t)h * Cu + col) * nblk + blk;
+        CHECK(off < hit.size() && !hit[off], "combine partial %zu", off);
+        if (off < hit.size()) hit[off] = 1;
+      }
+  }
+  for (unsigned char h : hit) if (!h) { CHECK(false, "combine partials not dense"); break; }
+}
+
+int main() {
+  int cases = 0;
+  for (int B : {1, 2, 3, 5})
+    for (int S : {8, 16, 32})
+      for (int N : {64, 128, 256})
+        for (int Cu : {64, 128, 256}) {
+          check_wgrad(B, S, N, Cu);
+          check_combine(B, S, N, Cu);
+          ++cases;
+        }
+  check_combine(2, 8, 64, 192);
+  const Up125WgradPlan c17 = up125_wgrad_plan(16384, 128, 128), c15 = up125_wgrad_plan(2048, 256, 256);
+  CHECK(c17.ctiles == 125 && c17.ktiles == 1 && c17.ks == 4 && c17.rows_per_split == 4096, "c17 plan");
+  CHECK(c15.ctiles == 250 && c15.ktiles == 2 && c15.ks == 1 && c15.rows_per_split == 2048, "c15 plan");
+  if (g_fail) {
+    fprintf(stderr, "up125_group_check: %d failures\n", g_fail);
+    return 1;
+  }
+  printf("up125_group_check: %d shapes OK\n", cases);
+  return 0;
+}
diff --git a/icsg3d_amd/csrc/up125.h b/icsg3d_amd/csrc/up125.h
--- a/icsg3d_amd/csrc/up125.h
+++ b/icsg3d_amd/csrc/up125.h
@@ -85,6 +85,46 @@
   const size_t w = (size_t)(8 * N > Cu ? 8 * N : Cu);
   return rows * w < ((size_t)1 << 30);
 }
+
+enum { UP125_WG_TILE = 128, UP125_WG_RESIDENT = 512, UP125_WG_MIN_ROWS = 256 };
+ICS_UP125_HD int up125_wg_ctiles(int g, int N) { return ((8 >> g) * N + UP125_WG_TILE - 1) / UP125_WG_TILE; }
+ICS_UP125_HD int up125_wg_tile0(int g, int N) {
+  int t = 0;
+  for (int h = 0; h < g; ++h) t += up125_group_classes(h) * up125_wg_ctiles(h, N);
+  return t;
+}
+struct Up125WgradPlan { int ktiles = 0, ctiles = 0, ks = 0, rows_per_split = 0; };
+inline Up125WgradPlan up125_wgrad_plan(unsigned rows, int N, int Cu) {
+  Up125WgradPlan p;
+  p.ktiles = (Cu + UP125_WG_TILE - 1) / UP125_WG_TILE;
+  p.ctiles = up125_wg_tile0(4, N);
+  const long base = (long)p.ktiles * p.ctiles, ks_max = rows / UP125_WG_MIN_ROWS > 0 ? rows / UP125_WG_MIN_ROWS : 1;
+  long ks = UP125_WG_RESIDENT / base;
+  ks = ks < 1 ? 1 : (ks > ks_max ? ks_max : ks);
+  p.rows_per_split = (int)((((long)rows + ks - 1) / ks + 31) / 32 * 32);
+  p.ks = (int)(((long)rows + p.rows_per_split - 1) / p.rows_per_split);
+  return p;
+}
+struct Up125WgradBlock { int g, slot, bbase, nt, kt, split; };
+ICS_UP125_F Up125WgradBlock up125_wgrad_block(unsigned bid, int ctiles, int ktiles, int N) {
+  Up125WgradBlock b;
+  const int ct = (int)(bid % (unsigned)ctiles);
+  bid /= (unsigned)ctiles;
+  b.kt = (int)(bid % (unsigned)ktiles);
+  b.split = (int)(bid / (unsigned)ktiles);
+  b.g = 0;
+  while (b.g < 3 && ct >= up125_wg_tile0(b.g + 1, N)) ++b.g;
+  const int per = up125_wg_ctiles(b.g, N), r = ct - up125_wg_tile0(b.g, N), cls = r / per;
+  b.nt = r - cls * per;
+  b.slot = up125_group_slot0(b.g) + cls;
+  b.bbase = up125_group_block0(b.g) + cls * (8 >> b.g);
+  return b;
+}
+ICS_UP125_HD size_t up125_wgrad_ws_floats(int ks, int N, int Cu) { return (size_t)125 * ks * Cu * N; }
+ICS_UP125_HD size_t up125_wgrad_group_off(int g, int ks, int N, int Cu) { return (size_t)up125_group_block0(g) * ks * Cu * N; }
+
+inline int up125_combine_blocks(const Up125Geom& u) { return (int)(((size_t)u.rows * (u.Cu / 4) + 255) / 256); }
+inline bool up125_combine_fold_ok(const Up125Geom& u) { return u.Cu % 4 == 0 && u.Cu / 4 <= 256 && 256 % (u.Cu / 4) == 0; }
 
 enum { UP125_POOL_WAVES = 6, UP125_POOL_ROUNDS = 5, UP125_XCH_ELEMS = 6 * 5 * 64 };
 ICS_UP125_F void up125_pool_lane(int lgc, unsigned bx, unsigned by, int lane, unsigned* tile, int* n) {
diff --git a/icsg3d_amd/csrc/up125.hip b/icsg3d_amd/csrc/up125.hip
--- a/icsg3d_amd/csrc/up125.hip
+++ b/icsg3d_amd/csrc/up125.hip
@@ -197,17 +197,27 @@
   return 0;
 }
 
+template <bool FOLD>
 __global__ __launch_bounds__(256) void up125_combine_kernel(const float* __restrict__ cls, size_t total,
-                                                            float* __restrict__ dxl, Up125Geom u) {
+                                                            float* __restrict__ dxl, Up125Geom u, BwdStat bs) {
+  __shared__ float sh1[FOLD ? 1024 : 1], sh2[FOLD ? 1024 : 1];
   const size_t i = (size_t)blockIdx.x * blockDim.x + threadIdx.x;
-  if (i >= total) return;
+  const bool live = i < total;
+  if (!FOLD && !live) return;
   const int C4 = u.Cu >> 2, T = u.T, lg = u.lgT, Sh = 2 * T;
   const int c = (int)(i % C4) * 4;
+  qf4 a1 = qf4{0.f, 0.f, 0.f, 0.f}, a2 = a1;
+  if (live) {
   const unsigned tile = (unsigned)(i / C4);
   const int jx = tile & (T - 1), jy = (tile >> lg) & (T - 1), jz = (tile >> (2 * lg)) & (T - 1), b = tile >> (3 * lg);
   qf4 O[3][3][3];
 #pragma unroll
   for (int q = 0; q < 27; ++q) O[q / 9][(q / 3) % 3][q % 3] = *reinterpret_cast<const qf4*>(cls + up125_class_off(u, q, tile, c));
+  qf4 mu = a1, rs = a1, sc = qf4{1.f, 1.f, 1.f, 1.f}, sf = a1;
+  if (FOLD) {
+    mu = *reinterpret_cast<const qf4*>(bs.mean + c); rs = *reinterpret_cast<const qf4*>(bs.rstd + c);
+    if (bs.post_act != ACT_NONE) { sc = *reinterpret_cast<const qf4*>(bs.scale + c); sf = *reinterpret_cast<const qf4*>(bs.shift + c); }
+  }
 #pragma unroll
   for (int ez = 0; ez < 2; ++ez)
 #pragma unroll
@@ -219,12 +229,45 @@
         for (int k = 0; k < 8; ++k) v += O[ez + (k >> 2)][ey + ((k >> 1) & 1)][ex + (k & 1)];
         const size_t vox = (((size_t)b * Sh + 2 * jz + ez) * Sh + 2 * jy + ey) * Sh + 2 * jx + ex;
         *reinterpret_cast<qf4*>(dxl + vox * (size_t)u.Cu + c) = v;
-      }
-}
-int launch_up125_combine(hipStream_t st, const float* cls, float* dxl, const Up125Geom& u) {
+        if (FOLD) {
+          const qf4 s = *reinterpret_cast<const qf4*>(bs.s + vox * (size_t)bs.ld + c);
+          qf4 d;
+          d.x = v.x * act_grad(fmaf(s.x, sc.x, sf.x), bs.post_act); d.y = v.y * act_grad(fmaf(s.y, sc.y, sf.y), bs.post_act);
+          d.z = v.z * act_grad(fmaf(s.z, sc.z, sf.z), bs.post_act); d.w = v.w * act_grad(fmaf(s.w, sc.w, sf.w), bs.post_act);
+          a1 += d;
+          a2.x = fmaf(d.x, (s.x - mu.x) * rs.x, a2.x); a2.y = fmaf(d.y, (s.y - mu.y) * rs.y, a2.y);
+          a2.z = fmaf(d.z, (s.z - mu.z) * rs.z, a2.z); a2.w = fmaf(d.w, (s.w - mu.w) * rs.w, a2.w);
+        }
+      }
+  }
+  if (FOLD) {
+    const int t = threadIdx.x;
+    *reinterpret_cast<qf4*>(sh1 + 4 * t) = a1;
+    *reinterpret_cast<qf4*>(sh2 + 4 * t) = a2;
+    __syncthreads();
+    const int RPP = 256 / C4;
+    for (int col = t; col < u.Cu; col += 256) {
+      float s1 = 0.f, s2 = 0.f;
+      for (int r = 0; r < RPP; ++r) { s1 += sh1[(r * C4) * 4 + col]; s2 += sh2[(r * C4) * 4 + col]; }
+      bs.partial[((size_t)0 * u.Cu + col) * gridDim.x + blockIdx.x] = s1;
+      bs.partial[((size_t)1 * u.Cu + col) * gridDim.x + blockIdx.x] = s2;
+    }
+  }
+}
+int launch_up125_combine(hipStream_t st, const float* cls, float* dxl, const Up125Geom& u, const BwdStat* bs) {
   ICS_CHECK(u.Cu % 4 == 0 && u.rows > 0, "up125 combine: channels must be a multiple of 4");
   const size_t total = (size_t)u.rows * (u.Cu / 4);
-  ICS_LAUNCH(up125_combine_kernel, dim3((unsigned)((total + 255) / 256)), dim3(256), 0, st, cls, total, dxl, u);
+  const dim3 grid((unsigned)up125_combine_blocks(u));
+  if (bs != nullptr) {
+    ICS_CHECK(up125_combine_fold_ok(u) && bs->partial && bs->s && bs->mean && bs->rstd && bs->ld >= u.Cu && bs->ld % 4 == 0 &&
+                  (bs->post_act == ACT_NONE || (bs->scale && bs->shift)),
+              "up125 combine: the fold needs 256 % (Cu / 4) == 0 and the producer's statistics");
+    ICS_LAUNCH(up125_combine_kernel<true>, grid, dim3(256), 0, st, cls, total, dxl, u, *bs);
+    conv_set_last_kernel_id("up125_combine_kernel<true>");
+  } else {
+    ICS_LAUNCH(up125_combine_kernel<false>, grid, dim3(256), 0, st, cls, total, dxl, u, BwdStat{});
+    conv_set_last_kernel_id("up125_combine_kernel<false>");
+  }
   ICS_HIP(hipGetLastError());
   return 0;
 }
```

After: 1197, median of 6. Within noise of the previous version (+0.6%).
